# v0lta/PyTorch-Wavelet-Toolbox

Measured on AMD Instinct MI355X. Metric: Msamples/s, higher is better.
Workload: dtype f32; 1 GPU; wavedec2_db4_L3_64x1024x1024_f32; api=ptwt_amd.wavedec2(x, 'db4', mode='reflect', level=3), parallelism=batch-sharded x1, no data-path collective

## Files before the change

### __graft_entry__.py

```python
from __future__ import annotations

import os
import subprocess
import sys
import time
from concurrent.futures import ThreadPoolExecutor

ROOT = os.path.dirname(os.path.abspath(__file__))
PKG = os.path.join(ROOT, "pytorch-wavelet-toolbox_amd")
CSRC = os.path.join(PKG, "csrc")
LIB = os.path.join(PKG, "libmifwt.so")
ARCH = "gfx950"

if ROOT not in sys.path:
    sys.path.insert(0, ROOT)


def _hipcc() -> str:
    for cand in (os.environ.get("HIPCC"), "/opt/rocm/bin/hipcc", "hipcc"):
        if cand and (os.path.isabs(cand) and os.path.exists(cand) or not os.path.isabs(cand)):
            return cand
    return "hipcc"


def _sources():
    return sorted(os.path.join(CSRC, f) for f in os.listdir(CSRC) if f.endswith(".hip"))


STAMP = os.path.join(PKG, "build", "flags.stamp")


def _flag_string() -> str:
    return f"arch={ARCH} cflags={os.environ.get('MIFWT_CFLAGS', '')}"


def _needs_rebuild() -> bool:
    if not os.path.exists(LIB):
        return True
    if os.path.exists(STAMP):
        with open(STAMP) as f:
            if f.read() != _flag_string():
                return True
    elif os.environ.get("MIFWT_CFLAGS"):
        return True
    t = os.path.getmtime(LIB)
    deps = _sources() + [os.path.join(CSRC, f) for f in os.listdir(CSRC) if f.endswith(".h")]
    deps.append(os.path.join(ROOT, "include", "mifwt.h"))
    return any(os.path.getmtime(d) > t for d in deps)


def build_variant(tag: str, cflags: str) -> str:
    objdir = os.path.join(PKG, "build_" + tag)
    os.makedirs(objdir, exist_ok=True)
    lib = os.path.join(PKG, f"libmifwt_{tag}.so")
    flags = [f"--offload-arch={ARCH}", "-O3", "-std=c++17", "-fPIC", "-I" + os.path.join(ROOT, "include"), "-I" + CSRC, *cflags.split()]

    def compile_one(src: str) -> str:
        obj = os.path.join(objdir, os.path.basename(src)[:-4] + ".o")
        subprocess.run([_hipcc(), *flags, "-c", src, "-o", obj], check=True)
        return obj

    with ThreadPoolExecutor(max_workers=8) as pool:
        objs = list(pool.map(compile_one, _sources()))
    subprocess.run([_hipcc(), f"--offload-arch={ARCH}", "-shared", "-fPIC", *objs, "-o", lib], check=True)
    return lib


def build(force: bool = False, verbose: bool = True) -> None:
    if force or _needs_rebuild():
        t0 = time.time()
        objdir = os.path.join(PKG, "build")
        os.makedirs(objdir, exist_ok=True)
        flags = [f"--offload-arch={ARCH}", "-O3", "-std=c++17", "-fPIC", "-I" + os.path.join(ROOT, "include"), "-I" + CSRC]
        flags += os.environ.get("MIFWT_CFLAGS", "").split()

        import re

        def deps_mtime(path: str, seen=None) -> float:
            seen = set() if seen is None else seen
            if path in seen or not os.path.exists(path):
                return 0.0
            seen.add(path)
            t = os.path.getmtime(path)
            with open(path) as f:
                for inc in re.findall(r'^\s*#\s*include\s+"([^"]+)"', f.read(), flags=re.M):
                    for base in (CSRC, os.path.join(ROOT, "include")):
                        t = max(t, deps_mtime(os.path.join(base, inc), seen))
            return t

        stale_flags = not os.path.exists(STAMP) or open(STAMP).read() != _flag_string()

        def compile_one(src: str) -> str:
            obj = os.path.join(objdir, os.path.basename(src)[:-4] + ".o")
            if force or stale_flags or not os.path.exists(obj) or os.path.getmtime(obj) < deps_mtime(src):
                subprocess.run([_hipcc(), *flags, "-c", src, "-o", obj], check=True)
            return obj

        with ThreadPoolExecutor(max_workers=8) as pool:
            objs = list(pool.map(compile_one, _sources()))
        subprocess.run([_hipcc(), f"--offload-arch={ARCH}", "-shared", "-fPIC", *objs, "-o", LIB], check=True)
        with open(STAMP, "w") as f:
            f.write(_flag_string())
        if verbose:
            print(f"[build] libmifwt.so built for {ARCH} in {time.time() - t0:.1f}s ({len(objs)} translation units)")
    import ptwt_amd
    from ptwt_amd import _engine

    lib = _engine.load_library()
    for sym in ("mifwt_dwt_fwd", "mifwt_dwt_inv", "mifwt_dwt_fwd_adjoint", "mifwt_dwt_inv_adjoint", "mifwt_swt_fwd", "mifwt_swt_inv", "mifwt_tap_correlate", "mifwt_tap_correlate_dilated", "mifwt_dwt2_fwd_pair", "mifwt_dwt2_fwd_pair_supported", "mifwt_dwt2_inv_pair", "mifwt_dwt2_inv_pair_supported", "mifwt_dwt2_fwd_pyramid", "mifwt_dwt2_fwd_pyramid_supported", "mifwt_dwt2_fwd_pyramid_schedule", "mifwt_dwt3_fwd_slab_plan", "mifwt_dwt_fwd_dtaps", "mifwt_dwt_inv_dtaps", "mifwt_dwt_fwd_adjoint_dtaps", "mifwt_dwt_inv_adjoint_dtaps", "mifwt_workspace_bytes_dtaps", "mifwt_kernel_id_dtaps", "mifwt_dwt2_inv_pyramid", "mifwt_dwt2_inv_pyramid_supported", "mifwt_dwt1_fwd_long", "mifwt_dwt1_fwd_long_levels", "mifwt_dwt1_inv_long", "mifwt_dwt1_inv_long_supported", "mifwt_dwt1_long_plan", "mifwt_dwt1_fwd_tail", "mifwt_dwt1_fwd_tail_max_n", "mifwt_dwt1_inv_tail", "mifwt_workspace_bytes", "mifwt_kernel_id", "mifwt_set_option",
                "mifwt_launch_count", "mifwt_strerror", "mifwt_abi_version", "mifwt_bwt_fwd", "mifwt_bwt_inv", "mifwt_bwt_supported", "mifwt_bwt_kernel_id",
                "mifwt_bwt_axis_fwd", "mifwt_bwt_axis_inv", "mifwt_bwt3_fwd", "mifwt_bwt3_inv", "mifwt_bwt3_supported", "mifwt_bwt3_kernel_id",
                "mifwt_bwt_tree_levels", "mifwt_bwt_tree_fwd", "mifwt_bwt_tree_inv"):
        getattr(lib, sym)
    if verbose:
        print(f"[build] ptwt_amd imports, libmifwt ABI v{lib.mifwt_abi_version()} exports all symbols of include/mifwt.h")


def smoke() -> None:
    import numpy as np
    import torch

    build(verbose=False)
    import ptwt_amd
    from oracle import fwt_oracle as O

    assert torch.cuda.is_available(), "smoke() needs a GPU"
    dev = torch.device("cuda:0")
    g = torch.Generator().manual_seed(0)
    x = torch.randn(3, 70, 530, generator=g, dtype=torch.float32)
    coeffs = ptwt_amd.wavedec2(x.to(dev), "db4", level=3)
    want = O.wavedec2(x.numpy().astype(np.float64), "db4", level=3)

    def rel(a, b):
        return float(np.linalg.norm(a.cpu().double().numpy() - b) / np.linalg.norm(b))

    errs = [rel(coeffs[0], want[0])]
    for got_t, want_t in zip(coeffs[1:], want[1:]):
        errs += [rel(g_, w_) for g_, w_ in zip(got_t, want_t)]
    rec = ptwt_amd.waverec2(coeffs, "db4")
    rt = float((rec[..., :70, :530].cpu() - x).abs().max())
    torch.cuda.synchronize()
    assert max(errs) < 1e-6, f"HIP wavedec2 deviates from the oracle: {max(errs):.3e}"
    assert rt < 5e-6, f"round trip error {rt:.3e}"
    print(f"[smoke] wavedec2 db4 L3 on {torch.cuda.get_device_name(0)}: max sub-band rel-err vs oracle "
          f"{max(errs):.2e}, round-trip max-abs {rt:.2e}  OK")


if __name__ == "__main__":
    build(force="--force" in sys.argv)
    if "--smoke" in sys.argv:
        smoke()
```

### include/mifwt.h

```cpp
#ifndef MIFWT_H
#define MIFWT_H

#include <stddef.h>
#include <stdint.h>

#ifdef __cplusplus
extern "C" {
#endif

#define MIFWT_ABI_VERSION 3
#define MIFWT_MAX_NDIM 3
#define MIFWT_MAX_FILT 128

enum mifwt_dtype { MIFWT_F32 = 0, MIFWT_F64 = 1, MIFWT_F16 = 2  };

enum mifwt_mode {
  MIFWT_MODE_ZERO = 0,
  MIFWT_MODE_CONSTANT = 1,
  MIFWT_MODE_REFLECT = 2,
  MIFWT_MODE_PERIODIC = 3,
  MIFWT_MODE_SYMMETRIC = 4
};

enum mifwt_status {
  MIFWT_OK = 0,
  MIFWT_ERR_BADARG = -1,
  MIFWT_ERR_UNSUPPORTED = -2,
  MIFWT_ERR_WORKSPACE = -3,
  MIFWT_ERR_LAUNCH = -4
};

typedef struct mifwt_level_desc {
  int32_t ndim;
  int32_t dtype;
  int32_t mode;
  int32_t filt_len;
  int64_t batch;
  int64_t sig_extent[MIFWT_MAX_NDIM];
  int64_t sig_stride[1 + MIFWT_MAX_NDIM];
  int64_t coef_extent[MIFWT_MAX_NDIM];
  int64_t approx_stride[1 + MIFWT_MAX_NDIM];
  int64_t detail_stride[1 + MIFWT_MAX_NDIM];
} mifwt_level_desc;

int mifwt_dwt_fwd(const mifwt_level_desc* desc, const void* x, void* approx, void* const* details,
                  const double* dec_lo, const double* dec_hi, void* workspace, size_t workspace_bytes,
                  void* stream);

int mifwt_dwt_inv(const mifwt_level_desc* desc, const void* approx, const void* const* details, void* y,
                  const double* rec_lo, const double* rec_hi, void* workspace, size_t workspace_bytes,
                  void* stream);

int mifwt_kernel_id_dtaps(const mifwt_level_desc* desc, int direction);
size_t mifwt_workspace_bytes_dtaps(const mifwt_level_desc* desc, int direction);
int mifwt_dwt_fwd_dtaps(const mifwt_level_desc* desc, const void* x, void* approx, void* const* details, const double* d_dec_lo,
                        const double* d_dec_hi, void* workspace, size_t workspace_bytes, void* stream);
int mifwt_dwt_inv_dtaps(const mifwt_level_desc* desc, const void* approx, const void* const* details, void* y, const double* d_rec_lo,
                        const double* d_rec_hi, void* workspace, size_t workspace_bytes, void* stream);
int mifwt_dwt_fwd_adjoint_dtaps(const mifwt_level_desc* desc, const void* g_approx, const void* const* g_details, void* g_x,
                                const double* d_dec_lo, const double* d_dec_hi, void* workspace, size_t workspace_bytes, void* stream);
int mifwt_dwt_inv_adjoint_dtaps(const mifwt_level_desc* desc, const void* g_y, void* g_approx, void* const* g_details,
                                const double* d_rec_lo, const double* d_rec_hi, void* workspace, size_t workspace_bytes, void* stream);

int mifwt_dwt1_fwd_outer(int dtype, int64_t batch, int64_t n, int64_t inner, const void* x, int64_t x_batch_stride, int64_t x_axis_stride, void* lo_out,
                         void* hi_out, int64_t out_batch_stride, int64_t out_axis_stride, int mode, int filt_len, const double* dec_lo,
                         const double* dec_hi, const double* d_dec_lo, const double* d_dec_hi, void* stream);
int mifwt_dwt1_inv_outer(int dtype, int64_t batch, int64_t m, int64_t n_out, int64_t inner, const void* lo_in, int64_t lo_batch_stride,
                         int64_t lo_axis_stride, const void* hi_in, int64_t hi_batch_stride, int64_t hi_axis_stride, void* y, int64_t y_batch_stride,
                         int64_t y_axis_stride, int filt_len, const double* rec_lo, const double* rec_hi, const double* d_rec_lo,
                         const double* d_rec_hi, void* stream);
int mifwt_tap_correlate_planes(int dtype, int along, int64_t batch, int64_t a_rows, int64_t a_cols, int64_t b_rows, int64_t b_cols, const void* a,
                               int64_t a_batch_stride, int64_t a_row_stride, const void* b, int64_t b_batch_stride, int64_t b_row_stride,
                               int filt_len, int c0, int sgn, int mode, double* out, void* stream);

int mifwt_dwt2_fwd_pair_supported(const mifwt_level_desc* d1, const mifwt_level_desc* d2);
int mifwt_dwt2_fwd_pair(const mifwt_level_desc* d1, const mifwt_level_desc* d2, const void* x, void* const* details1,
                        void* approx2, void* const* details2, const double* dec_lo, const double* dec_hi, void* stream);

int mifwt_dwt2_fwd_pyramid_supported(int nlevels, const mifwt_level_desc* const* descs);
int mifwt_dwt2_fwd_pyramid(int nlevels, const mifwt_level_desc* const* descs, const void* x, void* const* const* details, void* approx,
                           const double* dec_lo, const double* dec_hi, void* stream);
int mifwt_dwt2_fwd_pyramid_schedule(int nlevels, const mifwt_level_desc* const* descs, unsigned int* wg_start, int capacity);

int mifwt_dwt3_fwd_slab_plan(const mifwt_level_desc* desc, int* out, int capacity);

int mifwt_dwt2_inv_pyramid_supported(int nlevels, const mifwt_level_desc* const* descs);
int mifwt_dwt2_inv_pyramid(int nlevels, const mifwt_level_desc* const* descs, const void* approx, const void* const* const* details, void* y,
                           const double* rec_lo, const double* rec_hi, void* stream);

int mifwt_dwt2_inv_pair_supported(const mifwt_level_desc* d2, const mifwt_level_desc* d1);
int mifwt_dwt2_inv_pair(const mifwt_level_desc* d2, const mifwt_level_desc* d1, const void* approx2, const void* const* details2,
                        const void* const* details1, void* y, const double* rec_lo, const double* rec_hi, void* stream);

int mifwt_dwt1_fwd_tail_max_n(int dtype);
int mifwt_dwt1_fwd_tail(int dtype, int filt_len, int mode, int64_t rows, int64_t n, int nlevels, const void* x, int64_t x_row_stride,
                        void* approx, int64_t approx_row_stride, void* const* details, const int64_t* detail_row_strides,
                        const double* dec_lo, const double* dec_hi, void* stream);

int mifwt_dwt1_fwd_long_levels(int dtype, int filt_len, int mode, int64_t rows, int64_t n, int want);
int mifwt_dwt1_fwd_long(int dtype, int filt_len, int mode, int64_t rows, int64_t n, int nlevels, const void* x, int64_t x_row_stride,
                        void* approx, int64_t approx_row_stride, void* const* details, const int64_t* detail_row_strides,
                        const double* dec_lo, const double* dec_hi, void* stream);

int mifwt_dwt1_inv_tail(int dtype, int filt_len, int64_t rows, int64_t m, int nlevels, const void* approx, int64_t approx_row_stride,
                        const void* const* details, const int64_t* detail_row_strides, const int32_t* out_len, void* y,
                        int64_t y_row_stride, const double* rec_lo, const double* rec_hi, void* stream);

int mifwt_dwt1_inv_long_supported(int dtype, int filt_len, int64_t rows, int nlevels, const int32_t* m);
int mifwt_dwt1_inv_long(int dtype, int filt_len, int64_t rows, int nlevels, const int32_t* m, const void* approx, int64_t approx_row_stride,
                        const void* const* details, const int64_t* detail_row_strides, void* y, int64_t y_row_stride,
                        const double* rec_lo, const double* rec_hi, void* stream);

int mifwt_dwt1_long_plan(int inverse, int dtype, int filt_len, int mode, int64_t rows, int64_t n, int nlevels, const int32_t* m, int32_t* out6);

int mifwt_dwt_fwd_adjoint(const mifwt_level_desc* desc, const void* g_approx, const void* const* g_details, void* g_x,
                          const double* dec_lo, const double* dec_hi, void* workspace, size_t workspace_bytes,
                          void* stream);
int mifwt_dwt_inv_adjoint(const mifwt_level_desc* desc, const void* g_y, void* g_approx, void* const* g_details,
                          const double* rec_lo, const double* rec_hi, void* workspace, size_t workspace_bytes,
                          void* stream);

int mifwt_swt_fwd(int dtype, int filt_len, int64_t rows, int64_t n, int64_t dilation, const void* x, int64_t x_row_stride,
                  void* lo, void* hi, int64_t lo_row_stride, int64_t hi_row_stride, const double* dec_lo,
                  const double* dec_hi, double scale, void* stream);
int mifwt_swt_inv(int dtype, int filt_len, int64_t rows, int64_t n, int64_t dilation, const void* a, const void* d,
                  int64_t a_row_stride, int64_t d_row_stride, void* y, int64_t y_row_stride, const double* rec_lo,
                  const double* rec_hi, double scale, void* stream);

#define MIFWT_KID_BWT_FWD 26
#define MIFWT_KID_BWT_INV 27
#define MIFWT_KID_BWT_AXIS_FWD 28
#define MIFWT_KID_BWT_AXIS_INV 29
typedef struct mifwt_bwt_tables {
  const double* rows;
  int32_t n_top, n_bot;
} mifwt_bwt_tables;
int mifwt_bwt_supported(const mifwt_level_desc* desc, int direction);
int mifwt_bwt_kernel_id(const mifwt_level_desc* desc, int direction);
int mifwt_bwt_fwd(const mifwt_level_desc* desc, const void* x, void* approx, void* const* details, const double* lo, const double* hi,
                  const mifwt_bwt_tables* tables, void* stream);
int mifwt_bwt_inv(const mifwt_level_desc* desc, const void* approx, const void* const* details, void* y, const double* lo, const double* hi,
                  const mifwt_bwt_tables* tables, void* stream);
int mifwt_bwt_axis_fwd(int dtype, int filt_len, int mode, int64_t outer, int64_t n, int64_t inner, const void* x, const int64_t* x_strides,
                       void* lo_out, const int64_t* lo_strides, void* hi_out, const int64_t* hi_strides, const double* lo, const double* hi,
                       const mifwt_bwt_tables* tables, void* stream);
int mifwt_bwt_axis_inv(int dtype, int filt_len, int64_t outer, int64_t n, int64_t inner, const void* lo_in, const int64_t* lo_strides,
                       const void* hi_in, const int64_t* hi_strides, void* y, const int64_t* y_strides, const double* lo, const double* hi,
                       const mifwt_bwt_tables* tables, void* stream);

#define MIFWT_KID_BWT3_FWD 30
#define MIFWT_KID_BWT3_INV 31
int mifwt_bwt3_supported(const mifwt_level_desc* desc, int direction);
int mifwt_bwt3_kernel_id(const mifwt_level_desc* desc, int direction);
int mifwt_bwt3_fwd(const mifwt_level_desc* desc, const void* x, void* approx, void* const* details, const double* lo, const double* hi,
                   const mifwt_bwt_tables* tables, void* stream);
int mifwt_bwt3_inv(const mifwt_level_desc* desc, const void* approx, const void* const* details, void* y, const double* lo, const double* hi,
                   const mifwt_bwt_tables* tables, void* stream);

#define MIFWT_KID_BWT_TREE_FWD 32
#define MIFWT_KID_BWT_TREE_INV 33
int mifwt_bwt_tree_levels(int dtype, int filt_len, int64_t n, int max_levels);
int mifwt_bwt_tree_fwd(int dtype, int filt_len, int64_t rows, int64_t n, int64_t x_row_stride, int nlevels, const void* x,
                       void* const* levels, const double* lo, const double* hi, const mifwt_bwt_tables* tables, void* stream);
int mifwt_bwt_tree_inv(int dtype, int filt_len, int64_t rows, int64_t n, int nlevels, const void* leaves, void* const* levels,
                       const double* lo, const double* hi, const mifwt_bwt_tables* tables, void* stream);

int mifwt_tap_correlate(int dtype, int64_t rows, int64_t m_len, int64_t n_len, const void* a, int64_t a_row_stride,
                        const void* b, int64_t b_row_stride, int filt_len, int c0, int sgn, int mode, double* out,
                        void* stream);
int mifwt_tap_correlate_dilated(int dtype, int64_t rows, int64_t n, const void* a, int64_t a_row_stride, const void* b,
                                int64_t b_row_stride, int filt_len, int64_t c0, int64_t tstep, double* out, void* stream);

size_t mifwt_workspace_bytes(const mifwt_level_desc* desc, int direction);

int mifwt_kernel_id(const mifwt_level_desc* desc, int direction);

#define MIFWT_OPT_FORCE_GENERIC 0
#define MIFWT_OPT_ROWS_PER_CHUNK 1
#define MIFWT_OPT_PREFETCH_PAIRS 2
#define MIFWT_OPT_RESERVED3 3
#define MIFWT_OPT_NT_STORE 4
#define MIFWT_OPT_TILE_MODE 5
#define MIFWT_OPT_TILE_ROWS 6
#define MIFWT_OPT_MFMA_MODE 7
#define MIFWT_OPT_PAIR_MODE 8
#define MIFWT_OPT_PAIR_ROWS 9
#define MIFWT_OPT_PYRAMID_MODE 12
#define MIFWT_OPT_DEBUG 11
#define MIFWT_OPT_PYR_WGS 13
#define MIFWT_OPT_EXP 15
#define MIFWT_OPT_SYNC_STAGE 10
int mifwt_set_option(int key, int value);

int mifwt_pyr_profile_buffer(void* device_buffer);

#define MIFWT_VARIANT_FWD_MFMA_WALK 0
#define MIFWT_VARIANT_FWD_MFMA_TILE 1
#define MIFWT_VARIANT_FWD_PYR_ST16 2
#define MIFWT_VARIANT_FWD_PYR_ST8 3
unsigned long long mifwt_launch_count(int variant);

const char* mifwt_strerror(int code);
int mifwt_abi_version(void);

#ifdef __cplusplus
}
#endif
#endif
```

### pytorch-wavelet-toolbox_amd/_engine.py

```python
from __future__ import annotations

import ctypes
import os
import threading
import warnings
from typing import List, Optional, Sequence, Tuple

import torch

_PKG_DIR = os.path.dirname(os.path.abspath(__file__))
LIB_PATH = os.path.join(_PKG_DIR, os.environ.get("MIFWT_LIB", "libmifwt.so"))
if "MIFWT_LIB" in os.environ:
    import warnings

    warnings.warn(f"ptwt_amd: MIFWT_LIB is set — running on the experiment build {LIB_PATH}, not on the product library", RuntimeWarning)
ABI_VERSION = 3

MODE_IDS = {"zero": 0, "constant": 1, "reflect": 2, "periodic": 3, "symmetric": 4}
_DTYPE_IDS = {torch.float32: 0, torch.float64: 1, torch.float16: 2}

_i64x3 = ctypes.c_int64 * 3
_i64x4 = ctypes.c_int64 * 4
_array_types: dict = {}


def _arr(base, n: int):
    t = _array_types.get((base, n))
    if t is None:
        t = _array_types[(base, n)] = base * n
    return t


class LevelDesc(ctypes.Structure):

    _fields_ = [
        ("ndim", ctypes.c_int32),
        ("dtype", ctypes.c_int32),
        ("mode", ctypes.c_int32),
        ("filt_len", ctypes.c_int32),
        ("batch", ctypes.c_int64),
        ("sig_extent", _i64x3),
        ("sig_stride", _i64x4),
        ("coef_extent", _i64x3),
        ("approx_stride", _i64x4),
        ("detail_stride", _i64x4),
    ]


_lib: Optional[ctypes.CDLL] = None


def load_library() -> ctypes.CDLL:
    global _lib
    if _lib is not None:
        return _lib
    if not os.path.isfile(LIB_PATH):
        raise RuntimeError(
            f"ptwt_amd: HIP extension {LIB_PATH} is missing — build it with "
            "`python -c \"import __graft_entry__ as g; g.build()\"` (hipcc --offload-arch=gfx950). "
            "There is no CPU/eager fallback."
        )
    lib = ctypes.CDLL(LIB_PATH)
    vp, cp = ctypes.c_void_p, ctypes.c_char_p
    dbl_p = ctypes.POINTER(ctypes.c_double)
    desc_p = ctypes.POINTER(LevelDesc)
    lib.mifwt_abi_version.restype = ctypes.c_int
    lib.mifwt_abi_version.argtypes = []
    mismatch = lib.mifwt_abi_version() != ABI_VERSION
    if mismatch:
        if os.environ.get("MIFWT_ALLOW_ABI_MISMATCH") != "1":
            raise RuntimeError(f"ptwt_amd: {os.path.basename(LIB_PATH)} has ABI version {lib.mifwt_abi_version()}, this package expects "
                               f"{ABI_VERSION}; rebuild the extension (MIFWT_ALLOW_ABI_MISMATCH=1 loads it anyway, at your own risk)")
        warnings.warn("ptwt_amd: ABI version mismatch accepted through MIFWT_ALLOW_ABI_MISMATCH=1")
    lib.mifwt_strerror.restype = cp
    lib.mifwt_strerror.argtypes = [ctypes.c_int]
    lib.mifwt_kernel_id.restype = ctypes.c_int
    lib.mifwt_kernel_id.argtypes = [desc_p, ctypes.c_int]
    lib.mifwt_workspace_bytes.restype = ctypes.c_size_t
    lib.mifwt_workspace_bytes.argtypes = [desc_p, ctypes.c_int]
    lib.mifwt_dwt_fwd.restype = ctypes.c_int
    lib.mifwt_dwt_fwd.argtypes = [desc_p, vp, vp, ctypes.POINTER(vp), dbl_p, dbl_p, vp, ctypes.c_size_t, vp]
    lib.mifwt_dwt_inv.restype = ctypes.c_int
    lib.mifwt_dwt_inv.argtypes = [desc_p, vp, ctypes.POINTER(vp), vp, dbl_p, dbl_p, vp, ctypes.c_size_t, vp]
    lib.mifwt_dwt_fwd_adjoint.restype = ctypes.c_int
    lib.mifwt_dwt_fwd_adjoint.argtypes = [desc_p, vp, ctypes.POINTER(vp), vp, dbl_p, dbl_p, vp, ctypes.c_size_t, vp]
    lib.mifwt_dwt_inv_adjoint.restype = ctypes.c_int
    lib.mifwt_dwt_inv_adjoint.argtypes = [desc_p, vp, vp, ctypes.POINTER(vp), dbl_p, dbl_p, vp, ctypes.c_size_t, vp]
    lib.mifwt_tap_correlate.restype = ctypes.c_int
    lib.mifwt_tap_correlate.argtypes = [ctypes.c_int, ctypes.c_int64, ctypes.c_int64, ctypes.c_int64, vp, ctypes.c_int64, vp,
                                        ctypes.c_int64, ctypes.c_int, ctypes.c_int, ctypes.c_int, ctypes.c_int, vp, vp]
    lib.mifwt_tap_correlate_dilated.restype = ctypes.c_int
    lib.mifwt_tap_correlate_dilated.argtypes = [ctypes.c_int, ctypes.c_int64, ctypes.c_int64, vp, ctypes.c_int64, vp, ctypes.c_int64,
                                                ctypes.c_int, ctypes.c_int64, ctypes.c_int64, vp, vp]
    lib.mifwt_dwt2_fwd_pair_supported.restype = ctypes.c_int
    lib.mifwt_dwt2_fwd_pair_supported.argtypes = [desc_p, desc_p]
    lib.mifwt_dwt2_fwd_pair.restype = ctypes.c_int
    lib.mifwt_dwt2_fwd_pair.argtypes = [desc_p, desc_p, vp, ctypes.POINTER(vp), vp, ctypes.POINTER(vp), dbl_p, dbl_p, vp]
    vpp = ctypes.POINTER(vp)
    lib.mifwt_dwt2_fwd_pyramid_supported.restype = ctypes.c_int
    lib.mifwt_dwt2_fwd_pyramid_supported.argtypes = [ctypes.c_int, ctypes.POINTER(desc_p)]
    lib.mifwt_dwt2_inv_pyramid_supported.restype = ctypes.c_int
    lib.mifwt_dwt2_inv_pyramid_supported.argtypes = [ctypes.c_int, ctypes.POINTER(desc_p)]
    lib.mifwt_dwt2_inv_pyramid.restype = ctypes.c_int
    lib.mifwt_dwt2_inv_pyramid.argtypes = [ctypes.c_int, ctypes.POINTER(desc_p), vp, ctypes.POINTER(vpp), vp, dbl_p, dbl_p, vp]
    lib.mifwt_dwt2_fwd_pyramid.restype = ctypes.c_int
    lib.mifwt_dwt2_fwd_pyramid.argtypes = [ctypes.c_int, ctypes.POINTER(desc_p), vp, ctypes.POINTER(vpp), vp, dbl_p, dbl_p, vp]
    lib.mifwt_dwt2_inv_pair_supported.restype = ctypes.c_int
    lib.mifwt_dwt2_inv_pair_supported.argtypes = [desc_p, desc_p]
    lib.mifwt_dwt2_inv_pair.restype = ctypes.c_int
    lib.mifwt_dwt2_inv_pair.argtypes = [desc_p, desc_p, vp, ctypes.POINTER(vp), ctypes.POINTER(vp), vp, dbl_p, dbl_p, vp]
    lib.mifwt_dwt1_fwd_tail_max_n.restype = ctypes.c_int
    lib.mifwt_dwt1_fwd_tail_max_n.argtypes = [ctypes.c_int]
    lib.mifwt_dwt1_fwd_tail.restype = ctypes.c_int
    lib.mifwt_dwt1_fwd_tail.argtypes = [ctypes.c_int, ctypes.c_int, ctypes.c_int, ctypes.c_int64, ctypes.c_int64, ctypes.c_int, vp,
                                        ctypes.c_int64, vp, ctypes.c_int64, ctypes.POINTER(vp), ctypes.POINTER(ctypes.c_int64), dbl_p, dbl_p, vp]
    lib.mifwt_dwt1_fwd_long.restype = ctypes.c_int
    lib.mifwt_dwt1_fwd_long.argtypes = lib.mifwt_dwt1_fwd_tail.argtypes
    lib.mifwt_dwt1_fwd_long_levels.restype = ctypes.c_int
    lib.mifwt_dwt1_fwd_long_levels.argtypes = [ctypes.c_int, ctypes.c_int, ctypes.c_int, ctypes.c_int64, ctypes.c_int64, ctypes.c_int]
    lib.mifwt_dwt1_inv_long_supported.restype = ctypes.c_int
    lib.mifwt_dwt1_inv_long_supported.argtypes = [ctypes.c_int, ctypes.c_int, ctypes.c_int64, ctypes.c_int, ctypes.POINTER(ctypes.c_int32)]
    lib.mifwt_dwt1_inv_long.restype = ctypes.c_int
    lib.mifwt_dwt1_inv_long.argtypes = [ctypes.c_int, ctypes.c_int, ctypes.c_int64, ctypes.c_int, ctypes.POINTER(ctypes.c_int32), vp, ctypes.c_int64,
                                        ctypes.POINTER(vp), ctypes.POINTER(ctypes.c_int64), vp, ctypes.c_int64, dbl_p, dbl_p, vp]
    lib.mifwt_dwt1_inv_tail.restype = ctypes.c_int
    lib.mifwt_dwt1_inv_tail.argtypes = [ctypes.c_int, ctypes.c_int, ctypes.c_int64, ctypes.c_int64, ctypes.c_int, vp, ctypes.c_int64,
                                        ctypes.POINTER(vp), ctypes.POINTER(ctypes.c_int64), ctypes.POINTER(ctypes.c_int32), vp,
                                        ctypes.c_int64, dbl_p, dbl_p, vp]
    experiment = mismatch
    if not experiment or hasattr(lib, "mifwt_workspace_bytes_dtaps"):
        lib.mifwt_workspace_bytes_dtaps.restype = ctypes.c_size_t
        lib.mifwt_workspace_bytes_dtaps.argtypes = [desc_p, ctypes.c_int]
    if not experiment or hasattr(lib, "mifwt_kernel_id_dtaps"):
        lib.mifwt_kernel_id_dtaps.restype = ctypes.c_int
        lib.mifwt_kernel_id_dtaps.argtypes = [desc_p, ctypes.c_int]
        for name in ("mifwt_dwt_fwd_dtaps", "mifwt_dwt_inv_dtaps", "mifwt_dwt_fwd_adjoint_dtaps", "mifwt_dwt_inv_adjoint_dtaps"):
            getattr(lib, name).restype = ctypes.c_int
        lib.mifwt_dwt_fwd_dtaps.argtypes = [desc_p, vp, vp, vpp, vp, vp, vp, ctypes.c_size_t, vp]
        lib.mifwt_dwt_inv_dtaps.argtypes = [desc_p, vp, vpp, vp, vp, vp, vp, ctypes.c_size_t, vp]
        lib.mifwt_dwt_fwd_adjoint_dtaps.argtypes = [desc_p, vp, vpp, vp, vp, vp, vp, ctypes.c_size_t, vp]
        lib.mifwt_dwt_inv_adjoint_dtaps.argtypes = [desc_p, vp, vp, vpp, vp, vp, vp, ctypes.c_size_t, vp]
    if not experiment or hasattr(lib, "mifwt_launch_count"):
        lib.mifwt_launch_count.restype = ctypes.c_uint64
        lib.mifwt_launch_count.argtypes = [ctypes.c_int]
    if not experiment or hasattr(lib, "mifwt_tap_correlate_planes"):
        lib.mifwt_tap_correlate_planes.restype = ctypes.c_int
        lib.mifwt_tap_correlate_planes.argtypes = [ctypes.c_int, ctypes.c_int] + [ctypes.c_int64] * 5 + [vp, ctypes.c_int64, ctypes.c_int64, vp, ctypes.c_int64,
                                                   ctypes.c_int64, ctypes.c_int, ctypes.c_int, ctypes.c_int, ctypes.c_int, vp, vp]
        lib.mifwt_dwt1_inv_outer.restype = ctypes.c_int
        lib.mifwt_dwt1_inv_outer.argtypes = [ctypes.c_int] + [ctypes.c_int64] * 4 + [vp, ctypes.c_int64, ctypes.c_int64, vp, ctypes.c_int64, ctypes.c_int64, vp,
                                             ctypes.c_int64, ctypes.c_int64, ctypes.c_int, dbl_p, dbl_p, vp, vp, vp]
        lib.mifwt_dwt1_fwd_outer.restype = ctypes.c_int
        lib.mifwt_dwt1_fwd_outer.argtypes = [ctypes.c_int, ctypes.c_int64, ctypes.c_int64, ctypes.c_int64, vp, ctypes.c_int64, ctypes.c_int64, vp, vp, ctypes.c_int64,
                                             ctypes.c_int64, ctypes.c_int, ctypes.c_int, dbl_p, dbl_p, vp, vp, vp]
    lib.mifwt_set_option.restype = ctypes.c_int
    lib.mifwt_set_option.argtypes = [ctypes.c_int, ctypes.c_int]
    _lib = lib
    return lib


def _check(rc: int) -> None:
    if rc != 0:
        msg = load_library().mifwt_strerror(rc).decode()
        raise RuntimeError(f"libmifwt: {msg} (code {rc})")


def _require_gpu(t: torch.Tensor) -> None:
    if not t.is_cuda:
        raise RuntimeError(
            f"ptwt_amd: expected a tensor on a ROCm device, got device '{t.device}'. This engine runs on "
            "MI355X only; there is no CPU path."
        )


level_events: Optional[list] = None

ROW_ALIGN = int(os.environ.get("MIFWT_ROW_ALIGN", "1"))
PYRAMID_ROW_ALIGN = int(os.environ.get("MIFWT_PYRAMID_ROW_ALIGN", "1"))

OPT_FORCE_GENERIC = 0
OPT_ROWS_PER_CHUNK = 1
OPT_PREFETCH_PAIRS = 2
OPT_NT_STORE = 4
OPT_TILE_MODE = 5
OPT_TILE_ROWS = 6
OPT_MFMA_MODE = 7
OPT_PAIR_MODE = 8
OPT_PAIR_ROWS = 9
OPT_DEBUG = 11
OPT_PYRAMID_MODE = 12
OPT_PYR_WGS = 13
OPT_EXP = 15
KID_PAIR = 12
KID_INV_PAIR = 13
KID_TAIL = 14
KID_INV_TAIL = 15
KID_PYRAMID = 16
KID_LONG = 17
KID_INV_LONG = 18
KID_SMALL = 20
KID_INV_SMALL = 21
KID_INV_PYRAMID = 22
MAX_PYRAMID_LEVELS = 8


VARIANT_FWD_MFMA_WALK, VARIANT_FWD_MFMA_TILE, VARIANT_FWD_PYR_ST16, VARIANT_FWD_PYR_ST8 = 0, 1, 2, 3


def launch_count(variant: int) -> int:
    return int(load_library().mifwt_launch_count(variant))


def set_option(key: int, value: int) -> None:
    _check(load_library().mifwt_set_option(key, value))
    _plans.clear()
    for c in _routing_caches:
        c.clear()


_routing_caches: list = []


class _Plan:

    __slots__ = ("desc", "ref", "alloc_shape", "view_last", "nb", "plane_bytes", "ws_bytes", "kid", "empty")


_plans: dict = {}


def _trim_plans() -> None:
    if len(_plans) > 4096:
        for k in list(_plans)[:1024]:
            _plans.pop(k, None)
_tls = threading.local()
_taps_cache: dict = {}


class DevTaps:

    __slots__ = ("t",)

    def __init__(self, t: torch.Tensor):
        t = t.detach().reshape(-1)
        if t.dtype != torch.float64 or not t.is_contiguous():
            t = t.to(torch.float64).contiguous()
        self.t = t

    def __len__(self) -> int:
        return int(self.t.shape[0])

    @property
    def ptr(self) -> int:
        return self.t.data_ptr()


def outer_axis_supported(flen: int, dtype: torch.dtype) -> bool:
    return dtype in (torch.float32, torch.float64) and ((2 <= flen <= 20 and flen % 2 == 0) or flen in (24, 32))


def _is_dev(taps) -> bool:
    return isinstance(taps, DevTaps)


def _taps_array(taps: Sequence[float]):
    key = tuple(taps)
    arr = _taps_cache.get(key)
    if arr is None:
        if len(_taps_cache) > 512:
            _taps_cache.clear()
        arr = _taps_cache[key] = _arr(ctypes.c_double, len(key))(*key)
    return arr


def _band_ptrs(base: int, plane_bytes: int, n: int):
    return _arr(ctypes.c_void_p, n)(*[base + s * plane_bytes for s in range(1, n + 1)])


def _raw_stream(dev_index: int) -> int:
    return torch._C._cuda_getCurrentRawStream(dev_index)


class HipLevelEngine:

    @staticmethod
    def _analysis_plan(x: torch.Tensor, flen: int, mode_id: int, min_align: int = 1) -> _Plan:
        lib = load_library()
        ndim = x.dim() - 1
        batch = x.shape[0]
        sig = [int(n) for n in x.shape[1:]]
        coef = [(n + 2 * ((2 * flen - 3) // 2) + (n % 2) - flen) // 2 + 1 for n in sig]
        nb = 1 << ndim
        esz = x.element_size()
        align = max(ROW_ALIGN, min_align, 1)
        if align <= 1 and ndim == 2 and x.dtype == torch.float16 and 18 <= flen <= 32:
            align = 128
        pitch = -(-coef[-1] * esz // align) * align // esz if align > esz and ndim >= 2 else coef[-1]
        if min_align < 0 and ndim >= 2:
            pitch = coef[-1] - min_align
        p = _Plan()
        p.alloc_shape = (batch, nb, *coef[:-1], pitch)
        p.view_last = coef[-1] if pitch != coef[-1] else None
        p.nb = nb
        p.empty = batch == 0 or min(coef) == 0
        d = LevelDesc()
        d.ndim, d.dtype, d.mode, d.filt_len, d.batch = ndim, _DTYPE_IDS[x.dtype], mode_id, flen, batch
        bstride = [1] * (ndim + 2)
        for i in range(ndim, -1, -1):
            bstride[i] = bstride[i + 1] * p.alloc_shape[i + 1]
        for a in range(ndim):
            d.sig_extent[a] = sig[a]
            d.coef_extent[a] = coef[a]
            d.sig_stride[1 + a] = x.stride(1 + a)
            d.approx_stride[1 + a] = d.detail_stride[1 + a] = bstride[2 + a]
        d.sig_stride[0] = x.stride(0)
        d.approx_stride[0] = d.detail_stride[0] = bstride[0]
        p.desc = d
        p.ref = ctypes.byref(d)
        p.plane_bytes = bstride[1] * esz
        p.ws_bytes = 0 if p.empty else lib.mifwt_workspace_bytes(p.ref, 0)
        p.kid = lib.mifwt_kernel_id(p.ref, 0)
        return p

    @staticmethod
    def _details_only(pl: _Plan) -> _Plan:
        q = _Plan()
        d = LevelDesc()
        ctypes.memmove(ctypes.addressof(d), ctypes.addressof(pl.desc), ctypes.sizeof(LevelDesc))
        plane = pl.desc.detail_stride[0] // pl.nb
        d.detail_stride[0] = d.approx_stride[0] = plane * (pl.nb - 1)
        q.desc, q.ref = d, ctypes.byref(d)
        q.alloc_shape = (pl.alloc_shape[0], pl.nb - 1, *pl.alloc_shape[2:])
        q.view_last, q.nb, q.plane_bytes, q.ws_bytes, q.kid, q.empty = pl.view_last, pl.nb - 1, pl.plane_bytes, pl.ws_bytes, pl.kid, pl.empty
        return q

    def analysis(self, x: torch.Tensor, dec_lo: Sequence[float], dec_hi: Sequence[float], mode_id: int) -> torch.Tensor:
        _require_gpu(x)
        flen = len(dec_lo)
        key = (x.shape, x.stride(), x.dtype, mode_id, flen, ROW_ALIGN)
        p = _plans.get(key)
        if p is None:
            _trim_plans()
            p = _plans[key] = self._analysis_plan(x, flen, mode_id)
        buf = torch.empty(p.alloc_shape, dtype=x.dtype, device=x.device)
        if p.view_last is not None:
            buf = buf[..., : p.view_last]
        if p.empty:
            return buf
        base = buf.data_ptr()
        ptrs = _band_ptrs(base, p.plane_bytes, p.nb - 1)
        lib = _lib
        xp = x.data_ptr()
        if _is_dev(dec_lo):
            dl, dh = dec_lo.ptr, dec_hi.ptr
            self._run(p, 0, x, lambda ws, wsb, stream: lib.mifwt_dwt_fwd_dtaps(p.ref, xp, base, ptrs, dl, dh, ws, wsb, stream), kid=0, dtaps=True)
            return buf
        lo, hi = _taps_array(dec_lo), _taps_array(dec_hi)
        self._run(p, 0, x, lambda ws, wsb, stream: lib.mifwt_dwt_fwd(p.ref, xp, base, ptrs, lo, hi, ws, wsb, stream))
        return buf

    def analysis_pair(self, x: torch.Tensor, dec_lo: Sequence[float], dec_hi: Sequence[float], mode_id: int):
        _require_gpu(x)
        if x.dim() != 3:
            return None
        flen = len(dec_lo)
        key = ("pair", x.shape, x.stride(), x.dtype, mode_id, flen, ROW_ALIGN)
        plan = _plans.get(key)
        if plan is None:
            _trim_plans()
            lib = load_library()
            p1 = self._analysis_plan(x, flen, mode_id)
            ok = False
            p2 = None
            if not p1.empty:
                lvl1 = torch.empty(p1.alloc_shape, dtype=x.dtype, device="meta")
                if p1.view_last is not None:
                    lvl1 = lvl1[..., : p1.view_last]
                p2 = self._analysis_plan(lvl1[:, 0], flen, mode_id)
                ok = (not p2.empty) and bool(lib.mifwt_dwt2_fwd_pair_supported(p1.ref, p2.ref))
                if ok:
                    lean = self._details_only(p1)
                    if lib.mifwt_dwt2_fwd_pair_supported(lean.ref, p2.ref):
                        p1 = lean
            plan = _plans[key] = (p1, p2, ok)
        p1, p2, ok = plan
        if not ok:
            return None
        buf1 = torch.empty(p1.alloc_shape, dtype=x.dtype, device=x.device)
        buf2 = torch.empty(p2.alloc_shape, dtype=x.dtype, device=x.device)
        if p1.view_last is not None:
            buf1 = buf1[..., : p1.view_last]
        if p2.view_last is not None:
            buf2 = buf2[..., : p2.view_last]
        b1, b2 = buf1.data_ptr(), buf2.data_ptr()
        ptrs1 = _band_ptrs(b1 - (4 - p1.nb) * p1.plane_bytes, p1.plane_bytes, 3)
        ptrs2 = _band_ptrs(b2, p2.plane_bytes, 3)
        lo, hi = _taps_array(dec_lo), _taps_array(dec_hi)
        lib = _lib
        xp = x.data_ptr()
        self._run(p1, 0, x, lambda ws, wsb, stream: lib.mifwt_dwt2_fwd_pair(p1.ref, p2.ref, xp, ptrs1, b2, ptrs2, lo, hi, stream),
                  kid=KID_PAIR)
        return buf1, buf2

    def analysis_pyramid(self, x: torch.Tensor, dec_lo: Sequence[float], dec_hi: Sequence[float], mode_id: int, nlevels: int):
        _require_gpu(x)
        if x.dim() != 3 or x.dtype != torch.float32:
            return None
        flen = len(dec_lo)
        key, plan = self._pyramid_plan(x, flen, mode_id, nlevels)
        plans, n_ok, refs, kid = plan
        if n_ok == 0:
            return None
        bufs = []
        for pl in plans:
            b = torch.empty(pl.alloc_shape, dtype=x.dtype, device=x.device)
            bufs.append(b if pl.view_last is None else b[..., : pl.view_last])
        skey = (key, n_ok)
        slot = _tls.__dict__.setdefault("pyr", {}).get(skey)
        if slot is None:
            rows = [_arr(ctypes.c_void_p, 3)() for _ in plans]
            det = _arr(ctypes.POINTER(ctypes.c_void_p), n_ok)(*[ctypes.cast(r, ctypes.POINTER(ctypes.c_void_p)) for r in rows])
            slot = _tls.pyr[skey] = (rows, det)
            if len(_tls.pyr) > 256:
                _tls.pyr.clear()
                _tls.pyr[skey] = slot
        rows, det = slot
        for r, b, pl in zip(rows, bufs, plans):
            pb = pl.plane_bytes
            base = b.data_ptr() + (pl.nb - 3) * pb
            r[0], r[1], r[2] = base, base + pb, base + 2 * pb
        lo, hi = _taps_array(dec_lo), _taps_array(dec_hi)
        lib = _lib
        xp, ap = x.data_ptr(), bufs[-1].data_ptr()
        self._run(plans[0], 0, x, lambda ws, wsb, stream: lib.mifwt_dwt2_fwd_pyramid(n_ok, refs, xp, det, ap, lo, hi, stream), kid=kid)
        return bufs

    def pyramid_levels(self, x: torch.Tensor, flen: int, mode_id: int, nlevels: int) -> int:
        if x.dim() != 3 or x.dtype != torch.float32 or not x.is_cuda:
            return 0
        return self._pyramid_plan(x, flen, mode_id, nlevels)[1][1]

    def _pyramid_plan(self, x: torch.Tensor, flen: int, mode_id: int, nlevels: int):
        key = ("pyr", x.shape, x.stride(), mode_id, flen, min(nlevels, MAX_PYRAMID_LEVELS), ROW_ALIGN, PYRAMID_ROW_ALIGN)
        plan = _plans.get(key)
        if plan is None:
            _trim_plans()
            lib = load_library()

            def chain(min_align):
                plans = [self._analysis_plan(x, flen, mode_id, min_align)]
                while len(plans) < min(nlevels, MAX_PYRAMID_LEVELS) and not plans[-1].empty:
                    pl = plans[-1]
                    lvl = torch.empty(pl.alloc_shape, dtype=x.dtype, device="meta")
                    if pl.view_last is not None:
                        lvl = lvl[..., : pl.view_last]
                    plans.append(self._analysis_plan(lvl[:, 0], flen, mode_id, min_align))
                n_ok, route = 0, 0
                if not any(pl.empty for pl in plans):
                    for n in range(len(plans), 0, -1):
                        refs = (ctypes.POINTER(LevelDesc) * n)(*[ctypes.pointer(pl.desc) for pl in plans[:n]])
                        route = lib.mifwt_dwt2_fwd_pyramid_supported(n, refs)
                        if route:
                            n_ok = n
                            break
                return plans, n_ok, route

            plans, n_ok, route = chain(1)
            if n_ok and route == 1 and (PYRAMID_ROW_ALIGN > 1 or PYRAMID_ROW_ALIGN < 0):
                plans_a, n_a, route_a = chain(PYRAMID_ROW_ALIGN)
                if n_a == n_ok and route_a == route:
                    plans = plans_a
            keep = plans[:n_ok]
            refs = (ctypes.POINTER(LevelDesc) * n_ok)(*[ctypes.pointer(pl.desc) for pl in keep]) if n_ok else None
            if n_ok > 1:
                lean = [self._details_only(pl) for pl in keep[:-1]] + [keep[-1]]
                lrefs = (ctypes.POINTER(LevelDesc) * n_ok)(*[ctypes.pointer(pl.desc) for pl in lean])
                if lib.mifwt_dwt2_fwd_pyramid_supported(n_ok, lrefs) == route:
                    keep, refs = lean, lrefs
            if n_ok:
                keep[0].ws_bytes = 0
            plan = _plans[key] = (keep, n_ok, refs, KID_SMALL if route == 2 else KID_PYRAMID)
        return key, plan

    def analysis_tail(self, x: torch.Tensor, dec_lo: Sequence[float], dec_hi: Sequence[float], mode_id: int, nlevels: int):
        _require_gpu(x)
        if x.dim() != 2 or x.dtype not in (torch.float32, torch.float64) or x.stride(1) != 1 or nlevels < 2 or nlevels > 24:
            return None
        lib = load_library()
        flen = len(dec_lo)
        rows, n0 = x.shape
        if rows == 0 or n0 == 0 or flen > 32:
            return None
        k_long = lib.mifwt_dwt1_fwd_long_levels(_DTYPE_IDS[x.dtype], flen, mode_id, rows, n0, nlevels) if x.dtype == torch.float32 else 0
        long_rows = k_long >= 2
        if long_rows:
            nlevels = k_long
        elif n0 > lib.mifwt_dwt1_fwd_tail_max_n(_DTYPE_IDS[x.dtype]):
            return None
        sizes, n = [], n0
        for _ in range(nlevels):
            n = (n + flen - 1) // 2
            sizes.append(n)
        last = nlevels - 1
        bufs = [torch.empty((rows, 2 if i == last else 1, m), dtype=x.dtype, device=x.device) for i, m in enumerate(sizes)]
        esz = x.element_size()
        det = _arr(ctypes.c_void_p, nlevels)(*[b.data_ptr() + (sizes[i] * esz if i == last else 0) for i, b in enumerate(bufs)])
        det_rs = _arr(ctypes.c_int64, nlevels)(*[(2 if i == last else 1) * m for i, m in enumerate(sizes)])
        lo, hi = _taps_array(dec_lo), _taps_array(dec_hi)
        p = _Plan()
        p.ws_bytes, p.kid = 0, (KID_LONG if long_rows else KID_TAIL)
        d = LevelDesc()
        d.ndim = 1
        d.sig_extent[0] = n0
# ... 529 lines not shown
```

### pytorch-wavelet-toolbox_amd/csrc/mifwt_api.hip

```cpp
#include <string.h>

#include "mifwt_common.h"

using namespace mifwt;

namespace {

inline int64_t elem_size(int dtype) { return dtype == MIFWT_F64 ? 8 : (dtype == MIFWT_F16 ? 2 : 4); }

int validate(const mifwt_level_desc* d, int direction) {
  if (!d) return MIFWT_ERR_BADARG;
  if (d->ndim < 1 || d->ndim > MIFWT_MAX_NDIM) return MIFWT_ERR_BADARG;
  if (d->dtype != MIFWT_F32 && d->dtype != MIFWT_F64 && d->dtype != MIFWT_F16) return MIFWT_ERR_BADARG;
  if (d->filt_len < 2 || d->filt_len > MIFWT_MAX_FILT) return MIFWT_ERR_BADARG;
  if (d->batch < 0) return MIFWT_ERR_BADARG;
  if (direction == 0 && (d->mode < MIFWT_MODE_ZERO || d->mode > MIFWT_MODE_SYMMETRIC)) return MIFWT_ERR_BADARG;
  for (int a = 0; a < d->ndim; ++a) {
    const int64_t n = d->sig_extent[a], m = d->coef_extent[a], L = d->filt_len;
    if (n < 1 || m < 1 || n > INT32_MAX / 4 || m > INT32_MAX / 4) return MIFWT_ERR_BADARG;
    if (direction == 0) {
      const int64_t pad = 2 * ((2 * L - 3) / 2) + (n % 2);
      if (m != (n + pad - L) / 2 + 1) return MIFWT_ERR_BADARG;
    } else {
      const int64_t full = 2 * m - L + 2;
// ... 310 lines not shown

static size_t level_ws(const mifwt_level_desc* desc, int direction, bool dev) {
  if (validate_call(desc, direction) != MIFWT_OK) return 0;
  return route_ws(desc, direction == 0 || direction == 3 ? 0 : 1, route(desc, direction, dev));
}

int mifwt_kernel_id(const mifwt_level_desc* desc, int direction) {
  const int rc = validate_call(desc, direction);
  return rc != MIFWT_OK ? rc : route(desc, direction, false);
}

size_t mifwt_workspace_bytes(const mifwt_level_desc* desc, int direction) { return level_ws(desc, direction, false); }

int mifwt_kernel_id_dtaps(const mifwt_level_desc* desc, int direction) {
  if (direction < 0 || direction > 3) return MIFWT_ERR_BADARG;
  const int rc = validate_call(desc, direction);
  return rc != MIFWT_OK ? rc : route(desc, direction, true);
}

size_t mifwt_workspace_bytes_dtaps(const mifwt_level_desc* desc, int direction) {
  return direction < 0 || direction > 3 ? 0 : level_ws(desc, direction, true);
}

static LevelTaps reversed(LevelTaps t, int L, double (&buf)[2][MIFWT_MAX_FILT]) {
  if (t.dev) return {t.lo, t.hi, true, t.rev ^ 1};
  for (int j = 0; j < L; ++j) {
    buf[0][j] = t.tap_lo(L - 1 - j);
    buf[1][j] = t.tap_hi(L - 1 - j);
  }
  return {buf[0], buf[1], false, 0};
}

static int level_fwd(const mifwt_level_desc* desc, const void* x, void* approx, void* const* details, LevelTaps dec, void* workspace,
                     size_t workspace_bytes, void* stream) {
  int rc = validate(desc, 0);
  if (rc != MIFWT_OK) return rc;
  if (!x || !approx || !details || !dec.lo || !dec.hi) return MIFWT_ERR_BADARG;
  for (int s = 1; s < (1 << desc->ndim); ++s)
    if (!details[s - 1]) return MIFWT_ERR_BADARG;
  if (desc->batch == 0) return MIFWT_OK;
  hipStream_t st = static_cast<hipStream_t>(stream);
  const int kid = route(desc, 0, dec.dev);
  const size_t need = route_ws(desc, 0, kid);
  if (need > 0 && (!workspace || workspace_bytes < need)) return MIFWT_ERR_WORKSPACE;
  switch (kid) {
    case kGeneric: return generic_fwd(desc, x, approx, details, dec, workspace, st);
    case kDwt2FwdTile: return dwt2_fwd_tile(desc, x, approx, details, dec, st);
    case kDwt2FwdPyr: return dwt2_fwd_fused(desc, x, approx, details, dec, st);
    case kDwt1FwdRow: return rows_fwd(desc, x, approx, details, dec, workspace, st);
    default: break;
  }
  const double *lo, *hi;
  if ((rc = dec.host(&lo, &hi)) != MIFWT_OK) return rc;
  switch (kid) {
    case kDwt2FwdStream: return dwt2_fwd_stream(desc, x, approx, details, lo, hi, st);
    case kDwt2FwdMfma: return dwt2_fwd_mfma(desc, x, approx, details, lo, hi, st);
    case kDwt3FwdTile: return dwt3_fwd_tile(desc, x, approx, details, lo, hi, st);
    case kDwt3FwdWalk: return dwt3_fwd_walk(desc, x, approx, details, lo, hi, st);
    case kDwt3FwdStream: return plane3_fwd(desc, x, approx, details, lo, hi, workspace, st);
    default: return MIFWT_ERR_UNSUPPORTED;
  }
}

static int level_inv(const mifwt_level_desc* desc, const void* approx, const void* const* details, void* y, LevelTaps rec, void* workspace,
                     size_t workspace_bytes, void* stream) {
  int rc = validate(desc, 1);
  if (rc != MIFWT_OK) return rc;
  if (!y || !approx || !details || !rec.lo || !rec.hi) return MIFWT_ERR_BADARG;
  for (int s = 1; s < (1 << desc->ndim); ++s)
    if (!details[s - 1]) return MIFWT_ERR_BADARG;
  if (desc->batch == 0) return MIFWT_OK;
  hipStream_t st = static_cast<hipStream_t>(stream);
  const int kid = route(desc, 1, rec.dev);
  const size_t need = route_ws(desc, 1, kid);
  if (need > 0 && (!workspace || workspace_bytes < need)) return MIFWT_ERR_WORKSPACE;
  switch (kid) {
    case kGeneric: return generic_inv(desc, approx, details, y, rec, workspace, st);
    case kDwt2InvTile: return dwt2_inv_tile(desc, approx, details, y, rec, st);
    case kDwt2InvPyr: return dwt2_inv_fused(desc, approx, details, y, rec, st);
    case kDwt1InvRow: return rows_inv(desc, approx, details, y, rec, workspace, st);
    default: break;
  }
  const double *lo, *hi;
  if ((rc = rec.host(&lo, &hi)) != MIFWT_OK) return rc;
  switch (kid) {
    case kDwt2InvStream: return dwt2_inv_stream(desc, approx, details, y, lo, hi, st);
    case kDwt2InvMfma: return dwt2_inv_mfma(desc, approx, details, y, lo, hi, st);
    case kDwt3InvTile: return dwt3_inv_tile(desc, approx, details, y, lo, hi, st);
    case kDwt3InvWalk: return dwt3_inv_walk(desc, approx, details, y, lo, hi, st);
    case kDwt3InvStream: return plane3_inv(desc, approx, details, y, lo, hi, workspace, st);
    default: return MIFWT_ERR_UNSUPPORTED;
  }
}

static int level_fwd_adjoint(const mifwt_level_desc* desc, const void* g_approx, const void* const* g_details, void* g_x, LevelTaps dec,
                             void* workspace, size_t workspace_bytes, void* stream) {
  int rc = validate(desc, 0);
  if (rc != MIFWT_OK) return rc;
  if (!g_x || !g_approx || !g_details || !dec.lo || !dec.hi) return MIFWT_ERR_BADARG;
  for (int s = 1; s < (1 << desc->ndim); ++s)
    if (!g_details[s - 1]) return MIFWT_ERR_BADARG;
  if (desc->batch == 0) return MIFWT_OK;
  hipStream_t st = static_cast<hipStream_t>(stream);
  const bool synth = dec.dev ? route(desc, 2, true) != kGeneric
                             : adjoint_is_synthesis(desc) && (desc->mode == MIFWT_MODE_ZERO || adjoint_border_supported(desc));
  if (!synth) {
    const size_t need = generic_ws(desc, 1);
    if (need > 0 && (!workspace || workspace_bytes < need)) return MIFWT_ERR_WORKSPACE;
    return generic_inv(desc, g_approx, g_details, g_x, dec, workspace, st, true);
  }
  double buf[2][MIFWT_MAX_FILT];
  const mifwt_level_desc z = as_zero_mode(desc);
  rc = level_inv(&z, g_approx, g_details, g_x, reversed(dec, desc->filt_len, buf), workspace, workspace_bytes, stream);
  if (rc != MIFWT_OK || desc->mode == MIFWT_MODE_ZERO) return rc;
  return adjoint_border(desc, g_approx, g_details, g_x, dec, st);
}

static int level_inv_adjoint(const mifwt_level_desc* desc, const void* g_y, void* g_approx, void* const* g_details, LevelTaps rec,
                             void* workspace, size_t workspace_bytes, void* stream) {
  const int rc = validate(desc, 1);
  if (rc != MIFWT_OK) return rc;
  if (!rec.lo || !rec.hi) return MIFWT_ERR_BADARG;
  double buf[2][MIFWT_MAX_FILT];
  const mifwt_level_desc z = as_zero_mode(desc);
  return level_fwd(&z, g_y, g_approx, g_details, reversed(rec, desc->filt_len, buf), workspace, workspace_bytes, stream);
}

int mifwt_dwt_fwd(const mifwt_level_desc* desc, const void* x, void* approx, void* const* details,
                  const double* dec_lo, const double* dec_hi, void* workspace, size_t workspace_bytes,
                  void* stream) {
  return level_fwd(desc, x, approx, details, {dec_lo, dec_hi, false, 0}, workspace, workspace_bytes, stream);
}

int mifwt_dwt_inv(const mifwt_level_desc* desc, const void* approx, const void* const* details, void* y,
                  const double* rec_lo, const double* rec_hi, void* workspace, size_t workspace_bytes,
                  void* stream) {
  return level_inv(desc, approx, details, y, {rec_lo, rec_hi, false, 0}, workspace, workspace_bytes, stream);
}

int mifwt_dwt_fwd_adjoint(const mifwt_level_desc* desc, const void* g_approx, const void* const* g_details, void* g_x,
                          const double* dec_lo, const double* dec_hi, void* workspace, size_t workspace_bytes,
                          void* stream) {
  return level_fwd_adjoint(desc, g_approx, g_details, g_x, {dec_lo, dec_hi, false, 0}, workspace, workspace_bytes, stream);
}

int mifwt_dwt_inv_adjoint(const mifwt_level_desc* desc, const void* g_y, void* g_approx, void* const* g_details,
                          const double* rec_lo, const double* rec_hi, void* workspace, size_t workspace_bytes,
                          void* stream) {
  return level_inv_adjoint(desc, g_y, g_approx, g_details, {rec_lo, rec_hi, false, 0}, workspace, workspace_bytes, stream);
}

int mifwt_dwt_fwd_dtaps(const mifwt_level_desc* desc, const void* x, void* approx, void* const* details, const double* d_dec_lo,
                        const double* d_dec_hi, void* workspace, size_t workspace_bytes, void* stream) {
  return level_fwd(desc, x, approx, details, {d_dec_lo, d_dec_hi, true, 0}, workspace, workspace_bytes, stream);
}

int mifwt_dwt_inv_dtaps(const mifwt_level_desc* desc, const void* approx, const void* const* details, void* y, const double* d_rec_lo,
                        const double* d_rec_hi, void* workspace, size_t workspace_bytes, void* stream) {
  return level_inv(desc, approx, details, y, {d_rec_lo, d_rec_hi, true, 0}, workspace, workspace_bytes, stream);
}

int mifwt_dwt_fwd_adjoint_dtaps(const mifwt_level_desc* desc, const void* g_approx, const void* const* g_details, void* g_x,
                                const double* d_dec_lo, const double* d_dec_hi, void* workspace, size_t workspace_bytes, void* stream) {
  return level_fwd_adjoint(desc, g_approx, g_details, g_x, {d_dec_lo, d_dec_hi, true, 0}, workspace, workspace_bytes, stream);
}

int mifwt_dwt_inv_adjoint_dtaps(const mifwt_level_desc* desc, const void* g_y, void* g_approx, void* const* g_details,
                                const double* d_rec_lo, const double* d_rec_hi, void* workspace, size_t workspace_bytes, void* stream) {
  return level_inv_adjoint(desc, g_y, g_approx, g_details, {d_rec_lo, d_rec_hi, true, 0}, workspace, workspace_bytes, stream);
}

static LevelTaps host_or_device(const double* lo, const double* hi, const double* d_lo, const double* d_hi) {
  return d_lo && d_hi ? LevelTaps{d_lo, d_hi, true, 0} : LevelTaps{lo, hi, false, 0};
}

int mifwt_dwt1_fwd_outer(int dtype, int64_t batch, int64_t n, int64_t inner, const void* x, int64_t x_batch_stride, int64_t x_axis_stride, void* lo_out,
                         void* hi_out, int64_t out_batch_stride, int64_t out_axis_stride, int mode, int filt_len, const double* dec_lo,
                         const double* dec_hi, const double* d_dec_lo, const double* d_dec_hi, void* stream) {
  const LevelTaps taps = host_or_device(dec_lo, dec_hi, d_dec_lo, d_dec_hi);
  if (!x || !lo_out || !hi_out || !taps.lo || !taps.hi || batch < 0 || n < 1 || inner < 1) return MIFWT_ERR_BADARG;
  if (mode < MIFWT_MODE_ZERO || mode > MIFWT_MODE_SYMMETRIC) return MIFWT_ERR_BADARG;
  if ((dtype != MIFWT_F32 && dtype != MIFWT_F64) || !stream_filter_supported(filt_len)) return MIFWT_ERR_UNSUPPORTED;
  if (batch == 0) return MIFWT_OK;
  StreamJob jb;
  memset(&jb, 0, sizeof(jb));
  jb.in0 = x;
  jb.out0 = lo_out;
  jb.out1 = hi_out;
  jb.in0_s[0] = x_batch_stride, jb.in0_s[1] = x_axis_stride;
  jb.out0_s[0] = jb.out1_s[0] = out_batch_stride, jb.out0_s[1] = jb.out1_s[1] = out_axis_stride;
  StreamCall c;
  memset(&c, 0, sizeof(c));
  c.filt_len = filt_len;
  c.mode = mode;
  c.jobs = &jb;
  c.njobs = 1;
  c.batch = batch;
  c.inner = inner;
  c.n_in = n;
  c.n_out = (n + filt_len - 1) / 2;
  c.taps = taps;
  c.stream = static_cast<hipStream_t>(stream);
  return stream_call(dtype, kOuterFwd, c);
}

int mifwt_dwt1_inv_outer(int dtype, int64_t batch, int64_t m, int64_t n_out, int64_t inner, const void* lo_in, int64_t lo_batch_stride,
                         int64_t lo_axis_stride, const void* hi_in, int64_t hi_batch_stride, int64_t hi_axis_stride, void* y, int64_t y_batch_stride,
                         int64_t y_axis_stride, int filt_len, const double* rec_lo, const double* rec_hi, const double* d_rec_lo,
                         const double* d_rec_hi, void* stream) {
  const LevelTaps taps = host_or_device(rec_lo, rec_hi, d_rec_lo, d_rec_hi);
  if (!lo_in || !hi_in || !y || !taps.lo || !taps.hi || batch < 0 || m < 1 || inner < 1 || n_out < 1) return MIFWT_ERR_BADARG;
  if (n_out > 2 * m - filt_len + 2 || n_out < 2 * m - filt_len + 1) return MIFWT_ERR_BADARG;
  if ((dtype != MIFWT_F32 && dtype != MIFWT_F64) || !stream_filter_supported(filt_len)) return MIFWT_ERR_UNSUPPORTED;
  if (batch == 0) return MIFWT_OK;
  StreamJob jb;
  memset(&jb, 0, sizeof(jb));
  jb.in0 = lo_in;
  jb.in1 = hi_in;
  jb.out0 = y;
  jb.in0_s[0] = lo_batch_stride, jb.in0_s[1] = lo_axis_stride;
  jb.in1_s[0] = hi_batch_stride, jb.in1_s[1] = hi_axis_stride;
  jb.out0_s[0] = y_batch_stride, jb.out0_s[1] = y_axis_stride;
  StreamCall c;
  memset(&c, 0, sizeof(c));
  c.filt_len = filt_len;
  c.jobs = &jb;
  c.njobs = 1;
  c.batch = batch;
  c.inner = inner;
  c.n_in = m;
  c.n_out = n_out;
  c.taps = taps;
  c.stream = static_cast<hipStream_t>(stream);
  return stream_call(dtype, kOuterInv, c);
}

int mifwt_dwt2_fwd_pair_supported(const mifwt_level_desc* d1, const mifwt_level_desc* d2) {
  if (!d1 || !d2 || validate(d1, 0) != MIFWT_OK || validate(d2, 0) != MIFWT_OK) return 0;
  return dwt2_fwd_pair_supported(d1, d2) ? 1 : 0;
}

int mifwt_dwt2_fwd_pair(const mifwt_level_desc* d1, const mifwt_level_desc* d2, const void* x, void* const* details1,
                        void* approx2, void* const* details2, const double* dec_lo, const double* dec_hi, void* stream) {
  if (!d1 || !d2) return MIFWT_ERR_BADARG;
  int rc = validate(d1, 0);
  if (rc == MIFWT_OK) rc = validate(d2, 0);
  if (rc != MIFWT_OK) return rc;
  if (!x || !details1 || !approx2 || !details2 || !dec_lo || !dec_hi) return MIFWT_ERR_BADARG;
  for (int s = 0; s < 3; ++s)
    if (!details1[s] || !details2[s]) return MIFWT_ERR_BADARG;
  if (!dwt2_fwd_pair_supported(d1, d2)) return MIFWT_ERR_UNSUPPORTED;
  if (d1->batch == 0) return MIFWT_OK;
  hipStream_t st = static_cast<hipStream_t>(stream);
  const int pm = g_options[MIFWT_OPT_PAIR_MODE];
  if (pm != 1 && (pm == 3 || d1->filt_len >= 8) && dwt2_fwd_roll_supported(d1, d2))
    return dwt2_fwd_roll(d1, d2, x, details1, approx2, details2, dec_lo, dec_hi, st);
  return dwt2_fwd_pair(d1, d2, x, details1, approx2, details2, dec_lo, dec_hi, st);
}
static int pyramid_route(int nlevels, const mifwt_level_desc* const* descs) {
  const bool pyr = nlevels <= 3 && dwt2_fwd_pyr_supported(nlevels, descs);
  if (pyr && g_options[MIFWT_OPT_PYRAMID_MODE] == 1) return 1;
  const bool lone = nlevels == 1 && descs[0]->batch < 1024 && g_options[MIFWT_OPT_PYRAMID_MODE] != 3;
  if (!lone && dwt2_fwd_small_supported(nlevels, descs)) return 2;
  return pyr ? 1 : 0;
}

int mifwt_dwt2_fwd_pyramid_supported(int nlevels, const mifwt_level_desc* const* descs) {
  if (!descs || nlevels < 1 || nlevels > 8) return 0;
  for (int l = 0; l < nlevels; ++l)
    if (!descs[l] || validate(descs[l], 0) != MIFWT_OK) return 0;
  return pyramid_route(nlevels, descs);
}

int mifwt_dwt2_fwd_pyramid(int nlevels, const mifwt_level_desc* const* descs, const void* x, void* const* const* details, void* approx,
                           const double* dec_lo, const double* dec_hi, void* stream) {
  if (!descs || nlevels < 1 || nlevels > 8) return MIFWT_ERR_BADARG;
  for (int l = 0; l < nlevels; ++l) {
    if (!descs[l]) return MIFWT_ERR_BADARG;
    const int rc = validate(descs[l], 0);
    if (rc != MIFWT_OK) return rc;
  }
  if (!x || !details || !approx || !dec_lo || !dec_hi) return MIFWT_ERR_BADARG;
  for (int l = 0; l < nlevels; ++l) {
    if (!details[l]) return MIFWT_ERR_BADARG;
    for (int s = 0; s < 3; ++s)
      if (!details[l][s]) return MIFWT_ERR_BADARG;
  }
  const int route = pyramid_route(nlevels, descs);
  if (route == 0) return MIFWT_ERR_UNSUPPORTED;
  if (descs[0]->batch == 0) return MIFWT_OK;
  if (route == 2) return dwt2_fwd_small(nlevels, descs, x, details, approx, dec_lo, dec_hi, static_cast<hipStream_t>(stream));
  return dwt2_fwd_pyr(nlevels, descs, x, details, approx, {dec_lo, dec_hi, false, 0}, static_cast<hipStream_t>(stream));
}
int mifwt_dwt2_fwd_pyramid_schedule(int nlevels, const mifwt_level_desc* const* descs, unsigned int* wg_start, int capacity) {
  if (!descs || !wg_start || nlevels < 1 || nlevels > 3) return MIFWT_ERR_BADARG;
  for (int l = 0; l < nlevels; ++l) {
    if (!descs[l]) return MIFWT_ERR_BADARG;
    const int rc = validate(descs[l], 0);
    if (rc != MIFWT_OK) return rc;
  }
  if (pyramid_route(nlevels, descs) != 1) return MIFWT_ERR_UNSUPPORTED;
  return dwt2_fwd_pyr_schedule(nlevels, descs, wg_start, capacity);
}
int mifwt_dwt3_fwd_slab_plan(const mifwt_level_desc* desc, int* out, int capacity) {
  if (!desc || !out) return MIFWT_ERR_BADARG;
  const int rc = validate(desc, 0);
  if (rc != MIFWT_OK) return rc;
  return dwt3_fwd_slab_plan_query(desc, out, capacity);
}
int mifwt_dwt2_inv_pyramid_supported(int nlevels, const mifwt_level_desc* const* descs) {
  if (!descs || nlevels < 1 || nlevels > 8) return 0;
  for (int l = 0; l < nlevels; ++l)
    if (!descs[l] || validate(descs[l], 1) != MIFWT_OK) return 0;
  if (dwt2_inv_small_supported(nlevels, descs)) return 1;
  return nlevels <= 3 && dwt2_inv_pyr_supported(nlevels, descs) ? 2 : 0;
}

int mifwt_dwt2_inv_pyramid(int nlevels, const mifwt_level_desc* const* descs, const void* approx, const void* const* const* details, void* y,
                           const double* rec_lo, const double* rec_hi, void* stream) {
  if (!descs || nlevels < 1 || nlevels > 8) return MIFWT_ERR_BADARG;
  for (int l = 0; l < nlevels; ++l) {
    if (!descs[l]) return MIFWT_ERR_BADARG;
    const int rc = validate(descs[l], 1);
    if (rc != MIFWT_OK) return rc;
  }
  if (!approx || !details || !y || !rec_lo || !rec_hi) return MIFWT_ERR_BADARG;
  for (int l = 0; l < nlevels; ++l) {
    if (!details[l]) return MIFWT_ERR_BADARG;
    for (int s = 0; s < 3; ++s)
      if (!details[l][s]) return MIFWT_ERR_BADARG;
  }
  if (dwt2_inv_small_supported(nlevels, descs)) {
    if (descs[0]->batch == 0) return MIFWT_OK;
    return dwt2_inv_small(nlevels, descs, approx, details, y, rec_lo, rec_hi, static_cast<hipStream_t>(stream));
  }
  if (nlevels > 3 || !dwt2_inv_pyr_supported(nlevels, descs)) return MIFWT_ERR_UNSUPPORTED;
  return dwt2_inv_pyr(nlevels, descs, approx, details, y, {rec_lo, rec_hi, false, 0}, static_cast<hipStream_t>(stream));
}
int mifwt_dwt2_inv_pair_supported(const mifwt_level_desc* d2, const mifwt_level_desc* d1) {
  if (!d1 || !d2 || validate(d1, 1) != MIFWT_OK || validate(d2, 1) != MIFWT_OK) return 0;
  return dwt2_inv_pair_supported(d2, d1) ? 1 : 0;
}

int mifwt_dwt2_inv_pair(const mifwt_level_desc* d2, const mifwt_level_desc* d1, const void* approx2, const void* const* details2,
                        const void* const* details1, void* y, const double* rec_lo, const double* rec_hi, void* stream) {
  if (!d1 || !d2) return MIFWT_ERR_BADARG;
  int rc = validate(d2, 1);
  if (rc == MIFWT_OK) rc = validate(d1, 1);
  if (rc != MIFWT_OK) return rc;
  if (!approx2 || !details2 || !details1 || !y || !rec_lo || !rec_hi) return MIFWT_ERR_BADARG;
  for (int s = 0; s < 3; ++s)
    if (!details1[s] || !details2[s]) return MIFWT_ERR_BADARG;
  if (!dwt2_inv_pair_supported(d2, d1)) return MIFWT_ERR_UNSUPPORTED;
  if (d1->batch == 0) return MIFWT_OK;
  return dwt2_inv_pair(d2, d1, approx2, details2, details1, y, rec_lo, rec_hi, static_cast<hipStream_t>(stream));
}
int mifwt_dwt1_fwd_tail_max_n(int dtype) { return dwt1_tail_max_n(dtype); }

int mifwt_dwt1_fwd_tail(int dtype, int filt_len, int mode, int64_t rows, int64_t n, int nlevels, const void* x, int64_t x_row_stride,
                        void* approx, int64_t approx_row_stride, void* const* details, const int64_t* detail_row_strides,
                        const double* dec_lo, const double* dec_hi, void* stream) {
  if (!x || !approx || !details || !detail_row_strides || !dec_lo || !dec_hi) return MIFWT_ERR_BADARG;
  if (!dwt1_tail_supported(dtype, filt_len, mode, rows, n, nlevels)) return MIFWT_ERR_UNSUPPORTED;
  for (int l = 0; l < nlevels; ++l)
    if (!details[l]) return MIFWT_ERR_BADARG;
  return dwt1_tail(dtype, filt_len, mode, rows, n, nlevels, x, x_row_stride, approx, approx_row_stride, details, detail_row_strides,
                   dec_lo, dec_hi, static_cast<hipStream_t>(stream));
}
int mifwt_dwt1_fwd_long_levels(int dtype, int filt_len, int mode, int64_t rows, int64_t n, int want) {
  return dwt1_long_levels(dtype, filt_len, mode, rows, n, want);
}

int mifwt_dwt1_fwd_long(int dtype, int filt_len, int mode, int64_t rows, int64_t n, int nlevels, const void* x, int64_t x_row_stride,
                        void* approx, int64_t approx_row_stride, void* const* details, const int64_t* detail_row_strides,
                        const double* dec_lo, const double* dec_hi, void* stream) {
  if (!x || !approx || !details || !detail_row_strides || !dec_lo || !dec_hi) return MIFWT_ERR_BADARG;
  if (nlevels < 1 || dwt1_long_levels(dtype, filt_len, mode, rows, n, nlevels) != nlevels) return MIFWT_ERR_UNSUPPORTED;
  for (int l = 0; l < nlevels; ++l)
    if (!details[l]) return MIFWT_ERR_BADARG;
  return dwt1_long(dtype, filt_len, mode, rows, n, nlevels, x, x_row_stride, approx, approx_row_stride, details, detail_row_strides,
                   dec_lo, dec_hi, static_cast<hipStream_t>(stream));
}
int mifwt_dwt1_inv_long_supported(int dtype, int filt_len, int64_t rows, int nlevels, const int32_t* m) {
  return idwt1_long_supported(dtype, filt_len, rows, nlevels, m);
}

int mifwt_dwt1_inv_long(int dtype, int filt_len, int64_t rows, int nlevels, const int32_t* m, const void* approx, int64_t approx_row_stride,
                        const void* const* details, const int64_t* detail_row_strides, void* y, int64_t y_row_stride,
                        const double* rec_lo, const double* rec_hi, void* stream) {
  if (!m || !approx || !details || !detail_row_strides || !y || !rec_lo || !rec_hi) return MIFWT_ERR_BADARG;
  if (!idwt1_long_supported(dtype, filt_len, rows, nlevels, m)) return MIFWT_ERR_UNSUPPORTED;
  for (int l = 0; l < nlevels; ++l)
    if (!details[l]) return MIFWT_ERR_BADARG;
  return idwt1_long(dtype, filt_len, rows, nlevels, m, approx, approx_row_stride, details, detail_row_strides, y, y_row_stride, rec_lo,
                    rec_hi, static_cast<hipStream_t>(stream));
}
int mifwt_dwt1_long_plan(int inverse, int dtype, int filt_len, int mode, int64_t rows, int64_t n, int nlevels, const int32_t* m, int32_t* out6) {
  if (!out6) return 0;
  return inverse ? idwt1_long_plan_query(dtype, filt_len, rows, nlevels, m, out6) : dwt1_long_plan_query(dtype, filt_len, mode, rows, n, nlevels, out6);
}
int mifwt_dwt1_inv_tail(int dtype, int filt_len, int64_t rows, int64_t m, int nlevels, const void* approx, int64_t approx_row_stride,
                        const void* const* details, const int64_t* detail_row_strides, const int32_t* out_len, void* y,
                        int64_t y_row_stride, const double* rec_lo, const double* rec_hi, void* stream) {
  if (!approx || !details || !detail_row_strides || !out_len || !y || !rec_lo || !rec_hi) return MIFWT_ERR_BADARG;
  if (!idwt1_tail_supported(dtype, filt_len, rows, m, nlevels, out_len)) return MIFWT_ERR_UNSUPPORTED;
  for (int l = 0; l < nlevels; ++l)
    if (!details[l]) return MIFWT_ERR_BADARG;
  return idwt1_tail(dtype, filt_len, rows, m, nlevels, approx, approx_row_stride, details, detail_row_strides, out_len, y, y_row_stride,
                    rec_lo, rec_hi, static_cast<hipStream_t>(stream));
}
}
```

### pytorch-wavelet-toolbox_amd/csrc/mifwt_common.h

```cpp
#pragma once
#include <hip/hip_runtime.h>
#include <stdint.h>

#include <atomic>

#include "mifwt.h"

namespace mifwt {

constexpr int kMaxFilt = MIFWT_MAX_FILT;
extern int g_options[16];

#ifdef MIFWT_DIAG
constexpr bool kDiag = true;
#define MIFWT_DBG(a) ((a).dbg)
#define MIFWT_EXPW(a) ((a).exp)
#define MIFWT_PROFP(a) ((a).prof)
#else
constexpr bool kDiag = false;
#define MIFWT_DBG(a) 0
#define MIFWT_EXPW(a) 0
#define MIFWT_PROFP(a) (static_cast<unsigned long long*>(nullptr))
#endif
constexpr int kRouteBits = 8 | 64 | 512 | 1024 | 4096 | 8192 | 524288 | 1048576 | 2097152;
inline int exp_word() { return kDiag ? g_options[MIFWT_OPT_EXP] : 0; }
extern unsigned long long g_launch_counts[16];
inline void count_launch(int variant) { __atomic_fetch_add(&g_launch_counts[variant], 1ull, __ATOMIC_RELAXED); }

struct BatchSplit {
  int64_t inner, outer_stride;
};

struct DynLdsOnce {
  std::atomic<uint64_t> done{0};
  bool ensure(const void* fn, int bytes) {
    int dev = 0;
    if (hipGetDevice(&dev) != hipSuccess) return false;
    const uint64_t bit = uint64_t(1) << (dev & 63);
    if (done.load(std::memory_order_acquire) & bit) return true;
    if (hipFuncSetAttribute(fn, hipFuncAttributeMaxDynamicSharedMemorySize, bytes) != hipSuccess) return false;
    done.fetch_or(bit, std::memory_order_release);
    return true;
  }
};

__host__ __device__ __forceinline__ int ext_index(int i, int n, int mode) {
  if ((unsigned)i < (unsigned)n) return i;
  switch (mode) {
    case MIFWT_MODE_ZERO:
      return -1;
    case MIFWT_MODE_CONSTANT:
      return i < 0 ? 0 : n - 1;
    case MIFWT_MODE_PERIODIC: {
      int p = i % n;
      return p < 0 ? p + n : p;
    }
    case MIFWT_MODE_SYMMETRIC: {
      const int t = 2 * n;
      int p = i % t;
      if (p < 0) p += t;
      return p < n ? p : t - 1 - p;
    }
    default: {
      if (n == 1) return 0;
      const int t = 2 * (n - 1);
      int p = i % t;
      if (p < 0) p += t;
      return p < n ? p : t - p;
    }
  }
}

__host__ __device__ __forceinline__ int ext_index_near(int i, int n, int mode) {
  if ((unsigned)i < (unsigned)n) return i;
  int j;
  switch (mode) {
    case MIFWT_MODE_ZERO:
      return -1;
    case MIFWT_MODE_CONSTANT:
      return i < 0 ? 0 : n - 1;
    case MIFWT_MODE_PERIODIC:
      j = i < 0 ? i + n : i - n;
      break;
    case MIFWT_MODE_SYMMETRIC:
      j = i < 0 ? -i - 1 : 2 * n - 1 - i;
      break;
    default:
      j = i < 0 ? -i : 2 * (n - 1) - i;
      break;
  }
  return (unsigned)j < (unsigned)n ? j : ext_index(i, n, mode);
}

struct AxisJob {
  const void* in0;
  const void* in1;
  void* out0;
  void* out1;
  int64_t in0_stride[4], in1_stride[4], out0_stride[4], out1_stride[4];
};

struct DeviceTaps {
  const double* lo;
  const double* hi;
  int rev;
};
struct DevTapArg {
  const double* lo;
  const double* hi;
  int rev, len;
};
struct LevelTaps {
  const double* lo;
  const double* hi;
  bool dev;
  int rev;
  double tap_lo(int m) const { return dev ? 0.0 : lo[m]; }
  double tap_hi(int m) const { return dev ? 0.0 : hi[m]; }
  DeviceTaps dev_taps() const { return dev ? DeviceTaps{lo, hi, rev} : DeviceTaps{nullptr, nullptr, 0}; }
  DevTapArg dev_arg(int filt_len) const { return dev ? DevTapArg{lo, hi, rev, filt_len} : DevTapArg{nullptr, nullptr, 0, filt_len}; }
  int host(const double** lo_out, const double** hi_out) const {
    if (dev) return MIFWT_ERR_UNSUPPORTED;
    *lo_out = lo;
    *hi_out = hi;
    return MIFWT_OK;
  }
};
#ifdef __HIPCC__
__device__ __forceinline__ int dtap_rfl(int v) {
  int r;
  asm volatile("s_nop 0\n\tv_readfirstlane_b32 %0, %1\n\ts_nop 1" : "=s"(r) : "v"(v));
  return r;
}
__device__ __forceinline__ float dtap_uniform(float v) { return __builtin_bit_cast(float, dtap_rfl(__builtin_bit_cast(int, v))); }
__device__ __forceinline__ double dtap_uniform(double v) { return v; }
template <typename S>
__device__ __forceinline__ S dtap_lo(const DevTapArg& dt, int m) { return dtap_uniform((S)dt.lo[dt.rev ? dt.len - 1 - m : m]); }
template <typename S>
__device__ __forceinline__ S dtap_hi(const DevTapArg& dt, int m) { return dtap_uniform((S)dt.hi[dt.rev ? dt.len - 1 - m : m]); }
#endif
int launch_axis_fwd(int dtype, const AxisJob* jobs, int njobs, const int64_t out_ext[4], int taxis, int64_t n_in,
                    int mode, int filt_len, LevelTaps taps, hipStream_t stream);
int launch_axis_inv(int dtype, const AxisJob* jobs, int njobs, const int64_t out_ext[4], int taxis, int64_t m_in,
                    int filt_len, LevelTaps taps, hipStream_t stream);

int launch_axis_adj(int dtype, const AxisJob* jobs, int njobs, const int64_t out_ext[4], int taxis, int64_t m_in,
                    int64_t n_sig, int mode, int filt_len, LevelTaps taps, hipStream_t stream);

struct StreamJob {
  const void* in0;
  const void* in1;
  void* out0;
  void* out1;
  int64_t in0_s[3], in1_s[3], out0_s[3], out1_s[3];
};

struct StreamCall {
  int filt_len, mode;
  const StreamJob* jobs;
  int njobs;
  int64_t batch;
  int64_t rows[3];
  int64_t n_in, n_out;
  int64_t inner;
  LevelTaps taps;
  hipStream_t stream;
};

enum StreamKind { kOuterFwd = 0, kOuterInv = 1, kInnerFwd = 2, kInnerInv = 3 };
bool stream_filter_supported(int filt_len);
int stream_call(int dtype, int kind, const StreamCall& c);

enum KernelId { kGeneric = 0, kDwt2FwdStream = 1, kDwt2InvStream = 2, kDwt1FwdRow = 3, kDwt1InvRow = 4, kDwt3FwdStream = 5, kDwt3InvStream = 6, kDwt2FwdTile = 7, kDwt2InvTile = 8, kDwt3FwdTile = 9, kDwt3InvTile = 10, kDwt2FwdMfma = 11, kDwt2FwdPair = 12, kDwt2InvPair = 13, kDwt1FwdTail = 14, kDwt1InvTail = 15, kDwt2FwdPyr = 16,
  kDwt1FwdLong = 17, kDwt1InvLong = 18, kDwt2FwdSmall = 20, kDwt2InvSmall = 21, kDwt2InvPyr = 22, kDwt2InvMfma = 23, kDwt3FwdWalk = 24, kDwt3InvWalk = 25 };

bool dwt2_fwd_stream_supported(const mifwt_level_desc* d);
int dwt2_fwd_stream(const mifwt_level_desc* d, const void* x, void* approx, void* const* details,
                    const double* dec_lo, const double* dec_hi, hipStream_t stream);

bool dwt2_fwd_tile_supported(const mifwt_level_desc* d);
int dwt2_fwd_tile(const mifwt_level_desc* d, const void* x, void* approx, void* const* details, LevelTaps dec, hipStream_t stream,
                  BatchSplit split = {0, 0});

bool dwt2_fwd_mfma_supported(const mifwt_level_desc* d);
bool dwt2_inv_mfma_supported(const mifwt_level_desc* d);
int dwt2_inv_mfma(const mifwt_level_desc* d, const void* approx, const void* const* details, void* y, const double* lo,
                  const double* hi, hipStream_t stream);
int dwt2_fwd_mfma(const mifwt_level_desc* d, const void* x, void* approx, void* const* details,
                  const double* dec_lo, const double* dec_hi, hipStream_t stream);

bool dwt2_fwd_pair_supported(const mifwt_level_desc* d1, const mifwt_level_desc* d2);
int dwt2_fwd_pair(const mifwt_level_desc* d1, const mifwt_level_desc* d2, const void* x, void* const* details1,
                  void* approx2, void* const* details2, const double* dec_lo, const double* dec_hi, hipStream_t stream);

bool dwt2_fwd_roll_supported(const mifwt_level_desc* d1, const mifwt_level_desc* d2);

bool adjoint_border_supported(const mifwt_level_desc* d);
int adjoint_border(const mifwt_level_desc* d, const void* g_approx, const void* const* g_details, void* g_x, LevelTaps dec,
                   hipStream_t stream);
int dwt2_fwd_roll(const mifwt_level_desc* d1, const mifwt_level_desc* d2, const void* x, void* const* details1,
                  void* approx2, void* const* details2, const double* dec_lo, const double* dec_hi, hipStream_t stream);

bool dwt2_fwd_small_supported(int nlevels, const mifwt_level_desc* const* d);
int dwt2_fwd_small(int nlevels, const mifwt_level_desc* const* d, const void* x, void* const* const* details, void* approx, const double* lo,
                   const double* hi, hipStream_t stream);
bool dwt2_inv_small_supported(int nlevels, const mifwt_level_desc* const* d);
int dwt2_inv_small(int nlevels, const mifwt_level_desc* const* d, const void* approx, const void* const* const* details, void* y,
                   const double* lo, const double* hi, hipStream_t stream);
bool dwt2_inv_pyr_supported(int nlev, const mifwt_level_desc* const* d);
int dwt2_inv_pyr(int nlev, const mifwt_level_desc* const* d, const void* approx, const void* const* const* details, void* y,
                 LevelTaps rec, hipStream_t stream);
bool dwt2_fwd_pyr_supported(int nlev, const mifwt_level_desc* const* d);
int dwt2_fwd_pyr(int nlev, const mifwt_level_desc* const* d, const void* x, void* const* const* details, void* approx,
                 LevelTaps dec, hipStream_t stream);
int dwt2_fwd_pyr_schedule(int nlev, const mifwt_level_desc* const* d, uint32_t* wg_start, int capacity);

bool dwt2_inv_pair_supported(const mifwt_level_desc* d2, const mifwt_level_desc* d1);
int dwt2_inv_pair(const mifwt_level_desc* d2, const mifwt_level_desc* d1, const void* approx2, const void* const* details2,
                  const void* const* details1, void* y, const double* rec_lo, const double* rec_hi, hipStream_t stream);

int dwt1_tail_max_n(int dtype);
bool dwt1_tail_supported(int dtype, int filt_len, int mode, int64_t rows, int64_t n0, int nlevels);
int dwt1_tail(int dtype, int filt_len, int mode, int64_t rows, int64_t n0, int nlevels, const void* x, int64_t x_row_stride,
              void* approx, int64_t approx_row_stride, void* const* details, const int64_t* detail_row_strides, const double* lo,
              const double* hi, hipStream_t stream);

int dwt1_long_levels(int dtype, int filt_len, int mode, int64_t rows, int64_t n0, int want);
int dwt1_long(int dtype, int filt_len, int mode, int64_t rows, int64_t n0, int nlevels, const void* x, int64_t x_row_stride,
              void* approx, int64_t approx_row_stride, void* const* details, const int64_t* detail_row_strides, const double* lo,
              const double* hi, hipStream_t stream);
int idwt1_long_supported(int dtype, int filt_len, int64_t rows, int nlevels, const int* m);
int dwt1_long_plan_query(int dtype, int filt_len, int mode, int64_t rows, int64_t n0, int want, int* out);
int idwt1_long_plan_query(int dtype, int filt_len, int64_t rows, int nlevels, const int* m, int* out);
int idwt1_long(int dtype, int filt_len, int64_t rows, int nlevels, const int* m, const void* approx, int64_t approx_row_stride,
               const void* const* details, const int64_t* detail_row_strides, void* y, int64_t y_row_stride, const double* lo,
               const double* hi, hipStream_t stream);
bool idwt1_tail_supported(int dtype, int filt_len, int64_t rows, int64_t m0, int nlevels, const int* out_len);
int idwt1_tail(int dtype, int filt_len, int64_t rows, int64_t m0, int nlevels, const void* approx, int64_t approx_row_stride,
               const void* const* details, const int64_t* detail_row_strides, const int* out_len, void* y, int64_t y_row_stride,
               const double* lo, const double* hi, hipStream_t stream);

int dwt2_fwd_choice(const mifwt_level_desc* d);
int dwt2_fwd_fused(const mifwt_level_desc* d, const void* x, void* approx, void* const* details, LevelTaps dec,
                   hipStream_t stream);

bool dwt2_inv_tile_supported(const mifwt_level_desc* d);
int dwt2_inv_tile(const mifwt_level_desc* d, const void* approx, const void* const* details, void* y, LevelTaps rec,
                  hipStream_t stream);
int dwt2_inv_choice(const mifwt_level_desc* d);
int dwt2_inv_fused(const mifwt_level_desc* d, const void* approx, const void* const* details, void* y, LevelTaps rec,
                   hipStream_t stream);

bool dwt2_inv_stream_supported(const mifwt_level_desc* d);
int dwt2_inv_stream(const mifwt_level_desc* d, const void* approx, const void* const* details, void* y,
                    const double* rec_lo, const double* rec_hi, hipStream_t stream);

bool dwt3_fwd_tile_supported(const mifwt_level_desc* d);
int dwt3_fwd_tile(const mifwt_level_desc* d, const void* x, void* approx, void* const* details,
                  const double* dec_lo, const double* dec_hi, hipStream_t stream);
bool dwt3_fwd_walk_supported(const mifwt_level_desc* d);
bool dwt3_fwd_slab_supported(const mifwt_level_desc* d);
int dwt3_fwd_slab_plan_query(const mifwt_level_desc* d, int* out, int capacity);
bool dwt3_fwd_slab_pays(const mifwt_level_desc* d);
int dwt3_fwd_slab(const mifwt_level_desc* d, const void* x, void* approx, void* const* details, const double* lo, const double* hi,
                  hipStream_t stream);
int dwt3_fwd_walk(const mifwt_level_desc* d, const void* x, void* approx, void* const* details, const double* lo, const double* hi,
                  hipStream_t stream);
bool dwt3_inv_walk_supported(const mifwt_level_desc* d);
int dwt3_inv_walk(const mifwt_level_desc* d, const void* approx, const void* const* details, void* y, const double* lo, const double* hi,
                  hipStream_t stream);
bool dwt3_inv_tile_supported(const mifwt_level_desc* d);
int dwt3_inv_tile(const mifwt_level_desc* d, const void* approx, const void* const* details, void* y, const double* lo,
                  const double* hi, hipStream_t stream);

bool plane3_route_ok(const mifwt_level_desc* d, int direction);
bool rows_route_ok(const mifwt_level_desc* d, int direction);
size_t plane3_ws_bytes(const mifwt_level_desc* d, int direction);
size_t rows_ws_bytes(const mifwt_level_desc* d, int direction);
int plane3_fwd(const mifwt_level_desc* d, const void* x, void* approx, void* const* details, const double* lo,
               const double* hi, void* ws, hipStream_t stream);
int plane3_inv(const mifwt_level_desc* d, const void* approx, const void* const* details, void* y, const double* lo,
               const double* hi, void* ws, hipStream_t stream);
int rows_fwd(const mifwt_level_desc* d, const void* x, void* approx, void* const* details, LevelTaps taps, void* ws,
             hipStream_t stream);
int rows_inv(const mifwt_level_desc* d, const void* approx, const void* const* details, void* y, LevelTaps taps, void* ws,
             hipStream_t stream);

}
```

### pytorch-wavelet-toolbox_amd/csrc/mifwt_dwt2_fwd_pyr.hip

```cpp
#include <atomic>
#include <cstring>
#include <mutex>

#include "mifwt_pyr.h"

namespace mifwt {

unsigned long long* g_pyr_prof = nullptr;

constexpr int kPyrSub = 4;
constexpr int kPyrPad = 8;
constexpr int kPyrRing = 16;
constexpr int kPyrCtl = 64;
constexpr int kPyrWaves = 16;
constexpr int kPyrMaxChunks = 5;
constexpr int kPyrMaxWG = 320;
constexpr int kPyrTailCols = 8;
constexpr int kPyrTailRows = kPyrRing + 8;
constexpr int kPyrTailBytes = kPyrTailRows * kPyrTailCols * 8;

template <int L, int NLEV>
struct PyrArgs {
  const float* x;
  float* det[NLEV];
  uint32_t doff[NLEV][3];
  uint32_t dspan[NLEV];
  float* approx;
  int64_t xs_b, ds_b[NLEV], as_b;
  int xs_h, ds_h[NLEV], as_h;
  int H[NLEV + 1], W[NLEV + 1];
  int ngroups;
  int cpg0, cpg;
  int nchunks, nbuf;
  int pitch0, pitch1, pitch2;
  int nl1, nl2, nl3;
  int nt[3], tc0[3];
  int twave;
  int mode;
  int exp;
  int l2split;
  unsigned long long* prof;
  int dbg;
  DevTapArg dt;
  FastDiv hn_div;
  uint32_t wg_start[kPyrMaxWG + 1];
  f2 tap[L];
};

template <int L>
__device__ __forceinline__ void pyr_load_win2(const unsigned char* row, f2 (&w)[L / 2 + 1]) {
  constexpr int HP = L / 2;
  if constexpr (((L - 2) & 3) == 2) {
    w[0] = *reinterpret_cast<const f2*>(row);
#pragma unroll
    for (int j = 0; j < HP / 2; ++j) {
      const f4 v = *reinterpret_cast<const f4*>(row + 8 + 16 * j);
      w[1 + 2 * j] = (f2){v.x, v.y};
      w[2 + 2 * j] = (f2){v.z, v.w};
    }
  } else {
#pragma unroll
    for (int j = 0; j < (HP + 1) / 2; ++j) {
      const f4 v = *reinterpret_cast<const f4*>(row + 16 * j);
      w[2 * j] = (f2){v.x, v.y};
      w[2 * j + 1] = (f2){v.z, v.w};
    }
  }
}

template <int NW>
__device__ __forceinline__ void pyr_role(int wave, int nl1, int nchunks, int twave, int& role, int& idx) {
  role = -1;
  idx = 0;
  if constexpr (NW == 12) {
    if (wave == twave) role = kRoleTail;
    else if (wave < 4) role = kRoleL1, idx = wave;
    else if (wave < 6) role = kRoleL2, idx = wave - 4;
    else if (wave < 8) role = kRoleL3, idx = wave - 6;
    else if (wave == 11 || (wave == 10 && nchunks >= 2)) role = kRoleLoad, idx = 11 - wave;
    return;
  }
  if (wave == twave) {
    role = kRoleTail;
  } else if (wave < 5) {
    role = kRoleL1;
    idx = nl1 < 5 ? wave : (wave == 0 ? 1 : (wave == 1 ? 0 : (wave == 2 ? 3 : (wave == 3 ? 4 : 2))));
  } else if (wave == 13) {
    role = kRoleL1;
    idx = 5;
  } else if (wave >= 5 && wave <= 7) {
    role = kRoleL2;
    idx = wave - 5;
  } else if (wave >= 9 && wave <= 11) {
    role = kRoleL3;
    idx = wave - 9;
  } else if (wave == 15 || (wave == 14 && nchunks >= 2)) {
    role = kRoleLoad;
    idx = 15 - wave;
  }
}

template <int L, int NLEV, bool PROF, int NW, bool DT = false>
__global__ void __launch_bounds__(64 * NW) dwt2_fwd_pyr_kernel(const PyrArgs<L, NLEV> a) {
  constexpr int HL = L - 2, HP = L / 2;
  constexpr int NC1 = 2;
  constexpr int NP = 2 * HL + 1;
  extern __shared__ __attribute__((aligned(16))) unsigned char smem[];

  const int lane = threadIdx.x & 63;
  const int wave = __builtin_amdgcn_readfirstlane(threadIdx.x >> 6);
  int role, widx;
  pyr_role<NW>(wave, a.nl1, a.nchunks, a.twave, role, widx);
  if (role < 0 || (role == kRoleL1 && widx >= a.nl1) || (role == kRoleL2 && (NLEV < 2 || widx >= a.nl2)) ||
      (role == kRoleL3 && (NLEV < 3 || widx >= a.nl3)))
    return;

  const int grp = blockIdx.x % a.ngroups;
  int chunk = blockIdx.x / a.ngroups;
  if (MIFWT_EXPW(a) >> 16) chunk = (chunk + ((MIFWT_EXPW(a) >> 16) & 15)) % (int)(gridDim.x / a.ngroups);
  const uint32_t g_lo = a.wg_start[chunk], g_hi = a.wg_start[chunk + 1];
  if (g_lo >= g_hi) return;
  const bool zero_mode = a.mode == MIFWT_MODE_ZERO;
  Fold1 fold;
  fold.set(a.mode);

  int cA[NLEV + 1], cB[NLEV + 1], pA[NLEV + 1], pB[NLEV + 1];
  pA[NLEV] = cA[NLEV] = grp == 0 ? 0 : a.cpg0 + (grp - 1) * a.cpg;
  pB[NLEV] = cB[NLEV] = grp == a.ngroups - 1 ? a.W[NLEV] : min(a.W[NLEV], a.cpg0 + grp * a.cpg);
#pragma unroll
  for (int l = NLEV - 1; l >= 1; --l) {
    pA[l] = 2 * pA[l + 1];
    pB[l] = pB[l + 1] == a.W[l + 1] ? a.W[l] : min(a.W[l], 2 * pB[l + 1]);
    cA[l] = max(0, 2 * cA[l + 1] - HL);
    cB[l] = min(a.W[l], 2 * cB[l + 1]);
  }
  const int o1 = pA[1] - NC1 * ((pA[1] - cA[1] + NC1 - 1) / NC1);
  const int g0 = max(0, 2 * o1 - HL) & ~3;

  int sh1 = 0;
  if constexpr (NLEV >= 2) sh1 = (2 * cA[2] - cA[1]) & 2;
  unsigned char* const stage = smem + kPyrCtl;
  unsigned char* const ring1 = stage + a.nbuf * kPyrSub * a.pitch0;
  unsigned char* const ring2 = ring1 + (kPyrRing + 1) * a.pitch1;
  unsigned char* const tailimg = ring2 + (kPyrRing + 1) * a.pitch2;

  unsigned long long waited = 0;
  const unsigned long long t_start = PROF ? __builtin_readcyclecounter() : 0;
  const unsigned long long w_start = PROF ? __builtin_amdgcn_s_memrealtime() : 0;

  f2 tap[L];
  if (role != kRoleLoad) {
    if constexpr (DT) {
#pragma unroll
      for (int m = 0; m < L; ++m) tap[m] = (f2){dtap_lo<float>(a.dt, m), dtap_hi<float>(a.dt, m)};
    } else {
#pragma unroll
      for (int m = 0; m < L; ++m) tap[m] = a.tap[m];
    }
    const int nst = a.nbuf * kPyrSub * a.pitch0 / 16, nrg = ((kPyrRing + 1) * (a.pitch1 + a.pitch2)) / 16;
    if (role == kRoleL1)
      for (int i = widx * 64 + lane; i < nst; i += 64 * a.nl1) reinterpret_cast<f4*>(stage)[i] = (f4){0.f, 0.f, 0.f, 0.f};
    if (NLEV >= 2 && role == kRoleL2)
      for (int i = widx * 64 + lane; i < nrg; i += 64 * a.nl2) reinterpret_cast<f4*>(ring1)[i] = (f4){0.f, 0.f, 0.f, 0.f};
  } else {
    if (!(MIFWT_DBG(a) & 16)) __builtin_amdgcn_s_setprio(3);
  }
  __syncthreads();

  auto run_units = [&](auto role_tag) {
  constexpr int role = decltype(role_tag)::value;
#pragma unroll 1
  for (uint32_t g = g_lo; g < g_hi;) {
    const int img = (int)a.hn_div.div(g);
    const int u_lo = (int)(g - (uint32_t)img * (uint32_t)a.H[NLEV]);
    const int u_rows = min(a.H[NLEV] - u_lo, (int)(g_hi - g));
    g += (uint32_t)u_rows;

    int rA[NLEV + 1], rB[NLEV + 1], oA[NLEV + 1], oB[NLEV + 1];
    oA[NLEV] = rA[NLEV] = u_lo;
    oB[NLEV] = rB[NLEV] = u_lo + u_rows;
#pragma unroll
    for (int l = NLEV - 1; l >= 1; --l) {
      oA[l] = 2 * oA[l + 1];
      oB[l] = oB[l + 1] == a.H[l + 1] ? a.H[l] : min(a.H[l], 2 * oB[l + 1]);
      rA[l] = max(0, 2 * rA[l + 1] - HL);
      rB[l] = min(a.H[l], 2 * rB[l + 1]);
    }
    const bool top = u_lo == 0;
    const int D2 = top ? pyr_lag2(L) : pyr_lag2_inner(L);
    const int D3 = top ? pyr_lag3(L) : pyr_lag3_inner(L);
    const int E0 = 2 * rA[1] - HL, e0_end = 2 * rB[1];
    const int npair1 = rB[1] - rA[1] + HP - 1;
    const int nsteps1 = (npair1 + 3) / 4;
    int nsteps = nsteps1, npair2 = 0, npair3 = 0;
    if constexpr (NLEV >= 2) {
      npair2 = rB[2] - rA[2] + HP - 1;
      nsteps = max(nsteps, D2 + (npair2 + 1) / 2);
    }
    if constexpr (NLEV >= 3) {
      npair3 = rB[3] - rA[3] + HP - 1;
      nsteps = max(nsteps, D3 + npair3);
    }
    const int nsub = 2 * nsteps, nsub1 = 2 * nsteps1;

    if (role == kRoleLoad) {
      const uint32_t img_bytes = ((uint32_t)(a.H[0] - 1) * (uint32_t)a.xs_h + (uint32_t)a.W[0]) * 4u;
      const rsrc_t xr = pyr_rsrc(a.x + (int64_t)img * a.xs_b, img_bytes);
      const rsrc_t xr_dead = pyr_rsrc(a.x + (int64_t)img * a.xs_b, 0);
      const uint32_t row_bytes = (uint32_t)a.xs_h * 4u;
      const int mych = (a.nchunks - widx + 1) / 2;
      uint32_t voff[3];
#pragma unroll
      for (int j = 0; j < 3; ++j) {
        const int c = g0 + 256 * (widx + 2 * j) + 4 * lane;
        voff[j] = (j < mych && c < a.W[0]) ? 4u * (uint32_t)c : kPyrOob;
      }
      auto run = [&](auto nch_tag) {
        constexpr int NCH = decltype(nch_tag)::value;
        constexpr int PER = kPyrSub * NCH;
        int ib = 0;
        auto issue = [&](int t) {
          const uint32_t buf = (uint32_t)ib * (uint32_t)(kPyrSub * a.pitch0) + (uint32_t)kPyrCtl + kPyrPad * 4u + 1024u * (uint32_t)widx;
          ib = ib + 1 == a.nbuf ? 0 : ib + 1;
          if (MIFWT_DBG(a) & 2) return;
#pragma unroll
          for (int kk = 0; kk < kPyrSub; ++kk) {
            const int e = E0 + kPyrSub * t + kk;
            const bool dead = e >= e0_end || (zero_mode && (unsigned)e >= (unsigned)a.H[0]);
            const uint32_t soff = dead ? 0u : (uint32_t)fold(e, a.H[0]) * row_bytes;
            pyr_dma_row<NCH, 0x800>(voff, dead ? xr_dead : xr, soff, buf + (uint32_t)(kk * a.pitch0));
          }
        };
        const int ahead = a.nbuf - 1;
        for (int t = 0; t < ahead; ++t)
          if (t < nsub1) issue(t);
#pragma unroll 1
        for (int t = 0; t < nsub; ++t) {
          const int later = min(ahead - 1, nsub1 - 1 - t);
          if (later >= 6) pyr_wait_vm<(6 * PER > 63 ? 63 : 6 * PER)>();
          else if (later == 5) pyr_wait_vm<(5 * PER > 63 ? 63 : 5 * PER)>();
          else if (later == 4) pyr_wait_vm<(4 * PER > 63 ? 63 : 4 * PER)>();
          else if (later == 3) pyr_wait_vm<(3 * PER > 63 ? 63 : 3 * PER)>();
          else if (later == 2) pyr_wait_vm<(2 * PER > 63 ? 63 : 2 * PER)>();
          else if (later == 1) pyr_wait_vm<PER>();
          else pyr_wait_vm<0>();
          __syncthreads();
          if (t + ahead < nsub1) issue(t + ahead);
        }
      };
      pyr_dispatch<3>(mych - 1, [&](auto k) { run(std::integral_constant<int, decltype(k)::value + 1>{}); });
    } else if (role == kRoleL1) {
      const int gmax = (cB[1] - o1 + NC1 - 1) / NC1 - 1;
      const int glane = 64 * widx + lane;
      const int G = min(glane, gmax);
      const bool real = glane <= gmax;
      const int c0 = o1 + NC1 * G;
      const uint32_t win = 4u * (uint32_t)(kPyrPad - HL + 2 * o1 - g0 + 2 * NC1 * G);
      const bool full = real && c0 >= pA[1] && c0 + 1 < pB[1];
      const bool rag1 = real && c0 >= pA[1] && c0 + 1 == pB[1];
      const uint32_t sv2 = full ? 4u * (uint32_t)c0 : kPyrOob, sv1 = rag1 ? 4u * (uint32_t)c0 : kPyrOob;
      const bool rag = __builtin_amdgcn_readfirstlane(__builtin_amdgcn_ballot_w64(rag1) != 0);
      uint32_t rw[NC1];
#pragma unroll
      for (int k = 0; k < NC1; ++k) rw[k] = (real && c0 + k >= cA[1] && c0 + k < cB[1]) ? 4u * (uint32_t)(kPyrPad + sh1 + c0 + k - cA[1]) : 0u;
      constexpr int NFP = (kPyrSub * NP + 63) / 64;
      uint32_t f_src[NFP], f_dst[NFP];
      bool f_on[NFP];
      bool f_some = false;
#pragma unroll
      for (int ps = 0; ps < NFP; ++ps) {
        f_src[ps] = f_dst[ps] = 0;
        f_on[ps] = false;
        const int wlo = 2 * (o1 + NC1 * min(64 * widx, gmax)) - HL, whi = 2 * (o1 + NC1 * min(64 * widx + 63, gmax) + NC1 - 1) + 1;
        const int fl = lane + 64 * ps;
        const int kk = fl / NP, p = fl - kk * NP;
        const bool left = p < HL;
        const int e = left ? p - HL : a.W[0] + (p - HL);
        const bool zfix = zero_mode && !left && (a.W[0] & 3) != 0;
        if (kk < kPyrSub && (!zero_mode || zfix) && (left ? wlo < 0 : whi >= a.W[0])) {
          f_on[ps] = true;
          f_some = true;
          f_src[ps] = (uint32_t)(kk * a.pitch0) + 4u * (uint32_t)(kPyrPad + (zero_mode ? 0 : fold(e, a.W[0])) - g0);
          f_dst[ps] = (uint32_t)(kk * a.pitch0) + 4u * (uint32_t)(kPyrPad + e - g0);
        }
      }
      const bool f_any = __builtin_amdgcn_readfirstlane(__builtin_amdgcn_ballot_w64(f_some) != 0) && !(MIFWT_DBG(a) & 16384);
      const uint32_t dbytes = (MIFWT_DBG(a) & 1) ? 0u : a.dspan[0] + ((uint32_t)(a.H[1] - 1) * (uint32_t)a.ds_h[0] + (uint32_t)a.W[1]) * 4u;
      const uint32_t abytes = (MIFWT_DBG(a) & 1) ? 0u : ((uint32_t)(a.H[NLEV] - 1) * (uint32_t)a.as_h + (uint32_t)a.W[NLEV]) * 4u;
      const rsrc_t rd = pyr_rsrc(a.det[0] + (int64_t)img * a.ds_b[0], dbytes);
      const rsrc_t ra = pyr_rsrc(a.approx + (int64_t)img * a.as_b, NLEV == 1 ? abytes : 0u);
      const uint32_t o0 = a.doff[0][0], o1b = a.doff[0][1], o2 = a.doff[0][2];

      PyrAcc<L, NC1> acc;
      acc.clear();
      int bi = 0;
      constexpr int NW2 = HP + 1;
      auto load_win = [&](const unsigned char* row, f2 (&w)[NW2]) { pyr_load_win2<L>(row, w); };
      auto h_pair = [&](const f2 (&wa)[NW2], const f2 (&wb)[NW2], f2 (&ha)[NC1], f2 (&hb)[NC1]) {
#pragma unroll
        for (int k = 0; k < HP; ++k) {
#pragma unroll
          for (int c = 0; c < NC1; ++c) {
            if (k == 0) {
              ha[c] = vmul_lo(tap[L - 1], wa[c]);
              hb[c] = vmul_lo(tap[L - 1], wb[c]);
            } else {
              vfma_lo(ha[c], tap[L - 1 - 2 * k], wa[c + k]);
              vfma_lo(hb[c], tap[L - 1 - 2 * k], wb[c + k]);
            }
          }
#pragma unroll
          for (int c = 0; c < NC1; ++c) {
            vfma_hi(ha[c], tap[L - 2 - 2 * k], wa[c + k]);
            vfma_hi(hb[c], tap[L - 2 - 2 * k], wb[c + k]);
          }
        }
      };

      auto step1 = [&](auto sm_tag, int s) {
        constexpr int SM = decltype(sm_tag)::value;
        pyr_static_for<2>([&](auto half_tag) {
          constexpr int half = decltype(half_tag)::value;
          pyr_barrier<PROF>(waited);
          if (s < nsteps1) {
            unsigned char* sb = stage + bi * (kPyrSub * a.pitch0);
            bi = bi + 1 == a.nbuf ? 0 : bi + 1;
            if (f_any) {
              float v[NFP];
#pragma unroll
              for (int ps = 0; ps < NFP; ++ps) v[ps] = zero_mode ? 0.f : *reinterpret_cast<const float*>(sb + f_src[ps]);
              wave_lds_fence();
#pragma unroll
              for (int ps = 0; ps < NFP; ++ps)
                if (f_on[ps]) *reinterpret_cast<float*>(sb + f_dst[ps]) = v[ps];
              wave_lds_fence();
            }
            f2 w[kPyrSub][NW2];
#pragma unroll
            for (int kk = 0; kk < kPyrSub; ++kk) load_win(sb + kk * a.pitch0 + win, w[kk]);
            pyr_static_for<kPyrSub / 2>([&](auto jj_tag) {
              constexpr int jj = decltype(jj_tag)::value;
              constexpr int j = 2 * half + jj;
              constexpr int R = (4 * SM + j) % HP;
              f2 ha[NC1], hb[NC1];
              h_pair(w[2 * jj], w[2 * jj + 1], ha, hb);
              acc.template feed<0, R>(tap, ha);
              acc.template feed<1, R>(tap, hb);
              const int i = rA[1] + 4 * s + j - (HP - 1);
              const f2 (&lo)[NC1] = acc.lo[PyrAcc<L, NC1>::done(R)];
              const f2 (&hi)[NC1] = acc.hi[PyrAcc<L, NC1>::done(R)];
              if constexpr (NLEV >= 2) {
                unsigned char* rr = ring1 + ((4 * s + j) & (kPyrRing - 1)) * a.pitch1;
#pragma unroll
                for (int k = 0; k < NC1; ++k) *reinterpret_cast<float*>(rr + (i < rB[1] ? rw[k] : 0u)) = lo[k].x;
              }
              const bool own = i >= oA[1] && i < oB[1];
              const uint32_t v2 = own ? sv2 : kPyrOob;
              const uint32_t so = own ? (uint32_t)i * (uint32_t)a.ds_h[0] * 4u : 0u;
              __builtin_amdgcn_raw_buffer_store_b64((f2){hi[0].x, hi[1].x}, rd, v2, so + o0, MIFWT_ST_AUX);
              __builtin_amdgcn_raw_buffer_store_b64((f2){lo[0].y, lo[1].y}, rd, v2, so + o1b, MIFWT_ST_AUX);
              __builtin_amdgcn_raw_buffer_store_b64((f2){hi[0].y, hi[1].y}, rd, v2, so + o2, MIFWT_ST_AUX);
              if (rag) {
                const uint32_t v1 = own ? sv1 : kPyrOob;
                pyr_store1(hi[0].x, rd, v1, so + o0);
                pyr_store1(lo[0].y, rd, v1, so + o1b);
                pyr_store1(hi[0].y, rd, v1, so + o2);
              }
              if constexpr (NLEV == 1) {
                const uint32_t sa = own ? (uint32_t)i * (uint32_t)a.as_h * 4u : 0u;
                __builtin_amdgcn_raw_buffer_store_b64((f2){lo[0].x, lo[1].x}, ra, v2, sa, MIFWT_ST_AUX);
                if (rag) pyr_store1(lo[0].x, ra, own ? sv1 : kPyrOob, sa);
              }
            });
          }
        });
      };
      int sm = 0;
#pragma unroll 1
      for (int s = 0; s < nsteps; ++s) {
        if constexpr (HP == 3 || HP == 5) {
          pyr_dispatch<HP>(sm, [&](auto t) { step1(t, s); });
          sm = sm == HP - 1 ? 0 : sm + 1;
        } else {
          step1(std::integral_constant<int, 0>{}, s);
        }
      }
    } else if (NLEV >= 2 && role == kRoleL2) {
      if constexpr (NLEV >= 2) {
        const int gmax = (cB[2] - cA[2] + 1) / 2 - 1;
        const int glane = 64 * widx + lane;
        const int G = min(glane, gmax);
        const bool real = glane <= gmax;
        const int c0 = cA[2] + 2 * G;
        const uint32_t win = 4u * (uint32_t)(kPyrPad + sh1 - HL + 2 * c0 - cA[1]);
        const bool full = real && c0 >= pA[2] && c0 + 1 < pB[2];
        const bool rag1 = real && c0 >= pA[2] && c0 + 1 == pB[2];
        const uint32_t sv2 = full ? 4u * (uint32_t)c0 : kPyrOob, sv1 = rag1 ? 4u * (uint32_t)c0 : kPyrOob;
        const bool rag = __builtin_amdgcn_readfirstlane(__builtin_amdgcn_ballot_w64(rag1) != 0);
        uint32_t rw[2];
#pragma unroll
        for (int k = 0; k < 2; ++k) rw[k] = (real && c0 + k < cB[2]) ? 4u * (uint32_t)(kPyrPad + c0 + k - cA[2]) : 0u;
        uint32_t f_src = 0, f_dst = 0;
        bool f_on = false;
        const int f_r = lane / NP;
        {
          const int wlo = 2 * (cA[2] + 2 * min(64 * widx, gmax)) - HL, whi = 2 * (cA[2] + 2 * min(64 * widx + 63, gmax) + 1) + 1;
          const int p = lane - f_r * NP;
          const bool left = p < HL;
          const int e = left ? p - HL : a.W[1] + (p - HL);
          if (f_r < 4 && !zero_mode && (left ? wlo < 0 : whi >= a.W[1])) {
            f_on = true;
            f_src = 4u * (uint32_t)(kPyrPad + sh1 + fold(e, a.W[1]) - cA[1]);
            f_dst = 4u * (uint32_t)(kPyrPad + sh1 + e - cA[1]);
          }
        }
        const bool f_any = __builtin_amdgcn_readfirstlane(__builtin_amdgcn_ballot_w64(f_on) != 0) && !(MIFWT_DBG(a) & 32768);
        const uint32_t dbytes = (MIFWT_DBG(a) & 1) ? 0u : a.dspan[1] + ((uint32_t)(a.H[2] - 1) * (uint32_t)a.ds_h[1] + (uint32_t)a.W[2]) * 4u;
        const uint32_t abytes = (MIFWT_DBG(a) & 1) ? 0u : ((uint32_t)(a.H[NLEV] - 1) * (uint32_t)a.as_h + (uint32_t)a.W[NLEV]) * 4u;
        const rsrc_t rd = pyr_rsrc(a.det[1] + (int64_t)img * a.ds_b[1], dbytes);
        const rsrc_t ra = pyr_rsrc(a.approx + (int64_t)img * a.as_b, NLEV == 2 ? abytes : 0u);
        const uint32_t o0 = a.doff[1][0], o1b = a.doff[1][1], o2 = a.doff[1][2];
        const int ro1 = HP - 1 - rA[1];
        const int E1 = 2 * rA[2] - HL;
        PyrAcc<L, 2> acc;
        acc.clear();
        constexpr int NW2 = HP + 1;
        auto load_win = [&](const unsigned char* row, f2 (&w)[NW2]) { pyr_load_win2<L>(row, w); };
        auto h_pair = [&](const f2 (&wa)[NW2], const f2 (&wb)[NW2], f2 (&ha)[2], f2 (&hb)[2]) {
#pragma unroll
          for (int k = 0; k < HP; ++k) {
#pragma unroll
            for (int c = 0; c < 2; ++c) {
              if (k == 0) {
                ha[c] = vmul_lo(tap[L - 1], wa[c]);
                hb[c] = vmul_lo(tap[L - 1], wb[c]);
              } else {
                vfma_lo(ha[c], tap[L - 1 - 2 * k], wa[c + k]);
                vfma_lo(hb[c], tap[L - 1 - 2 * k], wb[c + k]);
              }
            }
#pragma unroll
            for (int c = 0; c < 2; ++c) {
              vfma_hi(ha[c], tap[L - 2 - 2 * k], wa[c + k]);
              vfma_hi(hb[c], tap[L - 2 - 2 * k], wb[c + k]);
            }
          }
        };
        if ((MIFWT_EXPW(a) & 3) == 1) __builtin_amdgcn_s_setprio(1);
        if ((MIFWT_EXPW(a) & 3) == 2) __builtin_amdgcn_s_setprio(2);
        if ((MIFWT_EXPW(a) & 3) == 3) __builtin_amdgcn_s_setprio(3);
        unsigned long long tsec[4] = {0, 0, 0, 0};
        auto do_pair = [&](auto r_tag, auto jj_tag, int s, const uint32_t (&so_r)[4]) {
          constexpr int R = decltype(r_tag)::value, jj = decltype(jj_tag)::value;
          unsigned long long t0 = 0;
          if constexpr (PROF) t0 = __builtin_readcyclecounter();
          f2 wa[NW2], wb[NW2];
          load_win(ring1 + so_r[2 * jj] + win, wa);
          load_win(ring1 + so_r[2 * jj + 1] + win, wb);
          if constexpr (PROF) {
            asm volatile("s_waitcnt lgkmcnt(0)" ::: "memory");
            const unsigned long long t1 = __builtin_readcyclecounter();
            tsec[0] += t1 - t0;
            t0 = t1;
          }
          f2 ha[2], hb[2];
          h_pair(wa, wb, ha, hb);
          acc.template feed<0, R>(tap, ha);
          acc.template feed<1, R>(tap, hb);
          if constexpr (PROF) {
            asm volatile("" ::: "memory");
            const unsigned long long t1 = __builtin_readcyclecounter();
            tsec[1] += t1 - t0;
            t0 = t1;
          }
          const int p = 2 * (s - D2) + jj;
          const int i = rA[2] + p - (HP - 1);
          const f2 (&lo)[2] = acc.lo[PyrAcc<L, 2>::done(R)];
          const f2 (&hi)[2] = acc.hi[PyrAcc<L, 2>::done(R)];
          if constexpr (NLEV >= 3) {
            unsigned char* rr = ring2 + (p & (kPyrRing - 1)) * a.pitch2;
            const bool mine = i < rB[2];
            *reinterpret_cast<float*>(rr + (mine ? rw[0] : 0u)) = lo[0].x;
            *reinterpret_cast<float*>(rr + (mine ? rw[1] : 0u)) = lo[1].x;
          }
          const bool own = i >= oA[2] && i < oB[2];
          const uint32_t v2 = own ? sv2 : kPyrOob;
          const uint32_t so = own ? (uint32_t)i * (uint32_t)a.ds_h[1] * 4u : 0u;
          __builtin_amdgcn_raw_buffer_store_b64((f2){hi[0].x, hi[1].x}, rd, v2, so + o0, MIFWT_ST_AUX);
          __builtin_amdgcn_raw_buffer_store_b64((f2){lo[0].y, lo[1].y}, rd, v2, so + o1b, MIFWT_ST_AUX);
          __builtin_amdgcn_raw_buffer_store_b64((f2){hi[0].y, hi[1].y}, rd, v2, so + o2, MIFWT_ST_AUX);
          if (rag) {
            const uint32_t v1 = own ? sv1 : kPyrOob;
            pyr_store1(hi[0].x, rd, v1, so + o0);
            pyr_store1(lo[0].y, rd, v1, so + o1b);
            pyr_store1(hi[0].y, rd, v1, so + o2);
          }
          if constexpr (NLEV == 2) {
            const uint32_t sa = own ? (uint32_t)i * (uint32_t)a.as_h * 4u : 0u;
            __builtin_amdgcn_raw_buffer_store_b64((f2){lo[0].x, lo[1].x}, ra, v2, sa, MIFWT_ST_AUX);
            if (rag) pyr_store1(lo[0].x, ra, own ? sv1 : kPyrOob, sa);
          }
          if constexpr (PROF) {
            asm volatile("" ::: "memory");
            tsec[2] += __builtin_readcyclecounter() - t0;
          }
        };
        auto half = [&](auto r_tag, auto jj_tag, int s, const uint32_t (&so_r)[4]) {
          constexpr int jj = decltype(jj_tag)::value;
          unsigned long long tp = 0;
          if constexpr (PROF) tp = __builtin_readcyclecounter();
          if (f_any) {
            const uint32_t fo = f_r == 0 ? so_r[0] : (f_r == 1 ? so_r[1] : (f_r == 2 ? so_r[2] : so_r[3]));
            const float v = *reinterpret_cast<const float*>(ring1 + fo + f_src);
            wave_lds_fence();
            if (f_on && (f_r >> 1) == jj) *reinterpret_cast<float*>(ring1 + fo + f_dst) = v;
            wave_lds_fence();
          }
          if constexpr (PROF) tsec[3] += __builtin_readcyclecounter() - tp;
          do_pair(r_tag, jj_tag, s, so_r);
        };
        auto step2 = [&](auto r0_tag, int s) {
          constexpr int R0 = decltype(r0_tag)::value;
          using RA = std::integral_constant<int, R0 % HP>;
          using RB = std::integral_constant<int, (R0 + 1) % HP>;
          pyr_barrier<PROF>(waited);
          const bool act = 2 * (s - D2) < npair2 && !(MIFWT_DBG(a) & 4);
          uint32_t so_r[4] = {0u, 0u, 0u, 0u};
          bool early = false;
          if (act) {
            int qmax0 = 0;
            const int e0 = E1 + 4 * (s - D2);
            if (e0 >= 0 && e0 + 3 < a.H[1]) {
              const int q0 = e0 + ro1;
#pragma unroll
              for (int r = 0; r < 4; ++r) so_r[r] = (uint32_t)(((q0 + r) & (kPyrRing - 1)) * a.pitch1);
              qmax0 = q0 + 1;
            } else {
#pragma unroll
              for (int r = 0; r < 4; ++r) {
                const int e = e0 + r;
                const bool dead = zero_mode && (unsigned)e >= (unsigned)a.H[1];
                const int q = fold(e, a.H[1]) + ro1;
                so_r[r] = (uint32_t)((dead ? kPyrRing : (q & (kPyrRing - 1))) * a.pitch1);
                if (r < 2 && !dead) qmax0 = max(qmax0, q);
              }
            }
            if (NW == 12 && widx == 0 && a.twave >= 0 && lane == 0) *reinterpret_cast<u4*>(smem) = (u4){so_r[0], so_r[1], so_r[2], so_r[3]};
            early = a.l2split && qmax0 <= 4 * s - 1;
            if (early) half(RA{}, std::integral_constant<int, 0>{}, s, so_r);
          }
          pyr_barrier<PROF>(waited);
          if (act) {
            if (!early) half(RA{}, std::integral_constant<int, 0>{}, s, so_r);
            half(RB{}, std::integral_constant<int, 1>{}, s, so_r);
          }
        };
        {
          int s = 0;
#pragma unroll 1
          for (; s < D2 && s < nsteps; ++s) {
            pyr_barrier<PROF>(waited);
            pyr_barrier<PROF>(waited);
          }
          constexpr int PERIOD = (HP % 2 == 0) ? (HP / 2 > 0 ? HP / 2 : 1) : HP;
#pragma unroll 1
          for (; s < nsteps; s += PERIOD) {
            pyr_static_for<PERIOD>([&](auto k_tag) {
              constexpr int k = decltype(k_tag)::value;
              if (k == 0 || s + k < nsteps) step2(std::integral_constant<int, (2 * k) % HP>{}, s + k);
            });
          }
        }
        if (PROF && widx == 0 && lane == 0) {
          unsigned long long* o = MIFWT_PROFP(a) + ((size_t)blockIdx.x * kPyrWaves + 14) * 2;
          o[0] += tsec[0], o[1] += tsec[1], o[2] += tsec[2], o[3] += tsec[3];
        }
      }
    } else if (NLEV >= 3 && role == kRoleL3) {
      if constexpr (NLEV >= 3) {
        const int gmax = cB[3] - cA[3] - 1;
        const int G = min(64 * widx + lane, gmax);
        const bool real = 64 * widx + lane <= gmax;
        const int c = cA[3] + G;
        const uint32_t win = 4u * (uint32_t)(kPyrPad - HL + 2 * c - cA[2]);
        const uint32_t sv = real && c >= pA[3] && c < pB[3] ? 4u * (uint32_t)c : kPyrOob;
        uint32_t f_src = 0, f_dst = 0;
        bool f_on = false;
        const int f_r = lane / NP;
        {
          const int wlo = 2 * (cA[3] + min(64 * widx, gmax)) - HL, whi = 2 * (cA[3] + min(64 * widx + 63, gmax)) + 1;
          const int p = lane - f_r * NP;
          const bool left = p < HL;
          const int e = left ? p - HL : a.W[2] + (p - HL);
          if (f_r < 2 && !zero_mode && (left ? wlo < 0 : whi >= a.W[2])) {
            f_on = true;
            f_src = 4u * (uint32_t)(kPyrPad + fold(e, a.W[2]) - cA[2]);
            f_dst = 4u * (uint32_t)(kPyrPad + e - cA[2]);
          }
        }
        const bool f_any = __builtin_amdgcn_readfirstlane(__builtin_amdgcn_ballot_w64(f_on) != 0) && !(MIFWT_DBG(a) & 32768);
        const uint32_t dbytes = (MIFWT_DBG(a) & 1) ? 0u : a.dspan[2] + ((uint32_t)(a.H[3] - 1) * (uint32_t)a.ds_h[2] + (uint32_t)a.W[3]) * 4u;
        const uint32_t abytes = (MIFWT_DBG(a) & 1) ? 0u : ((uint32_t)(a.H[3] - 1) * (uint32_t)a.as_h + (uint32_t)a.W[3]) * 4u;
        const rsrc_t rd = pyr_rsrc(a.det[2] + (int64_t)img * a.ds_b[2], dbytes);
        const rsrc_t ra = pyr_rsrc(a.approx + (int64_t)img * a.as_b, abytes);
        const uint32_t o0 = a.doff[2][0], o1b = a.doff[2][1], o2 = a.doff[2][2];
        const int ro2 = HP - 1 - rA[2];
        const int E2 = 2 * rA[3] - HL;
        PyrAcc<L, 1> acc;
        acc.clear();
        auto load_win = [&](const unsigned char* row, f2 (&w)[HP]) {
#pragma unroll
          for (int k = 0; k < HP; ++k) w[k] = *reinterpret_cast<const f2*>(row + 8 * k);
        };
        auto h_pair = [&](const f2 (&wa)[HP], const f2 (&wb)[HP], f2 (&ha)[1], f2 (&hb)[1]) {
#pragma unroll
          for (int k = 0; k < HP; ++k) {
            if (k == 0) {
              ha[0] = vmul_lo(tap[L - 1], wa[0]);
              hb[0] = vmul_lo(tap[L - 1], wb[0]);
            } else {
              vfma_lo(ha[0], tap[L - 1 - 2 * k], wa[k]);
              vfma_lo(hb[0], tap[L - 1 - 2 * k], wb[k]);
            }
            vfma_hi(ha[0], tap[L - 2 - 2 * k], wa[k]);
            vfma_hi(hb[0], tap[L - 2 - 2 * k], wb[k]);
          }
        };
        auto step3 = [&](auto r_tag, int s) {
          constexpr int R = decltype(r_tag)::value;
          pyr_barrier<PROF>(waited);
          if (s - D3 < npair3 && !(MIFWT_DBG(a) & 4)) {
            uint32_t so_r[2];
            const int e0 = E2 + 2 * (s - D3);
            if (e0 >= 0 && e0 + 1 < a.H[2]) {
              so_r[0] = (uint32_t)(((e0 + ro2) & (kPyrRing - 1)) * a.pitch2);
              so_r[1] = (uint32_t)(((e0 + 1 + ro2) & (kPyrRing - 1)) * a.pitch2);
            } else {
#pragma unroll
              for (int r = 0; r < 2; ++r) {
                const int e = e0 + r;
                const bool dead = zero_mode && (unsigned)e >= (unsigned)a.H[2];
                so_r[r] = (uint32_t)((dead ? kPyrRing : ((fold(e, a.H[2]) + ro2) & (kPyrRing - 1))) * a.pitch2);
              }
            }
            if (NW == 12 && widx == 0 && a.twave >= 0 && lane == 0) *reinterpret_cast<u2*>(smem + 16) = (u2){so_r[0], so_r[1]};
            if (f_any) {
              const uint32_t fo = f_r == 0 ? so_r[0] : so_r[1];
              const float v = *reinterpret_cast<const float*>(ring2 + fo + f_src);
              wave_lds_fence();
              if (f_on) *reinterpret_cast<float*>(ring2 + fo + f_dst) = v;
              wave_lds_fence();
            }
            f2 w[2][HP];
            load_win(ring2 + so_r[0] + win, w[0]);
            load_win(ring2 + so_r[1] + win, w[1]);
            f2 ha[1], hb[1];
            h_pair(w[0], w[1], ha, hb);
            acc.template feed<0, R>(tap, ha);
            acc.template feed<1, R>(tap, hb);
            const int i = rA[3] + (s - D3) - (HP - 1);
            const f2 lo = acc.lo[PyrAcc<L, 1>::done(R)][0], hi = acc.hi[PyrAcc<L, 1>::done(R)][0];
            const bool own = i >= oA[3] && i < oB[3];
            const uint32_t v = own ? sv : kPyrOob;
            const uint32_t so = own ? (uint32_t)i * (uint32_t)a.ds_h[2] * 4u : 0u;
            pyr_store1(hi.x, rd, v, so + o0);
            pyr_store1(lo.y, rd, v, so + o1b);
            pyr_store1(hi.y, rd, v, so + o2);
            pyr_store1(lo.x, ra, v, own ? (uint32_t)i * (uint32_t)a.as_h * 4u : 0u);
          }
          pyr_barrier<PROF>(waited);
        };
        {
          int s = 0;
#pragma unroll 1
          for (; s < D3 && s < nsteps; ++s) {
            pyr_barrier<PROF>(waited);
            pyr_barrier<PROF>(waited);
          }
#pragma unroll 1
          for (; s < nsteps; s += HP) {
            pyr_static_for<HP>([&](auto k_tag) {
              constexpr int k = decltype(k_tag)::value;
              if (k == 0 || s + k < nsteps) step3(k_tag, s + k);
            });
          }
        }
      }
    }
    else if (NW == 12 && role == kRoleTail) {
      if constexpr (NW == 12) {
      const int nt1 = a.nt[0], nt2 = NLEV >= 2 ? a.nt[1] : 0, nt3 = NLEV >= 3 ? a.nt[2] : 0;
      int j_lvl = 0, j_r = 0, j_c = 0;
      {
        int idx = lane;
        if (idx < 4 * nt1) {
          j_lvl = 1, j_r = idx / max(nt1, 1), j_c = idx - j_r * nt1;
        } else {
          idx -= 4 * nt1;
          if (idx < 4 * nt2) {
            j_lvl = 2, j_r = idx / max(nt2, 1), j_c = idx - j_r * nt2;
          } else {
            idx -= 4 * nt2;
            if (idx < 2 * nt3) j_lvl = 3, j_r = idx / max(nt3, 1), j_c = idx - j_r * nt3;
          }
        }
      }
      uint32_t soff[L];
      {
        const int Wp = j_lvl <= 1 ? a.W[0] : (j_lvl == 2 ? a.W[NLEV >= 2 ? 1 : 0] : a.W[NLEV >= 3 ? 2 : 0]);
        const int tc = j_lvl <= 1 ? a.tc0[0] : (j_lvl == 2 ? a.tc0[1] : a.tc0[2]);
        const int body0 = j_lvl <= 1 ? kPyrPad - g0 : (j_lvl == 2 ? kPyrPad + sh1 - cA[1] : kPyrPad - cA[NLEV >= 2 ? 2 : 1]);
#pragma unroll
        for (int k = 0; k < L; ++k) {
          const int x = 2 * (tc + j_c) - HL + k;
          const bool oob = (unsigned)x >= (unsigned)Wp;
          soff[k] = (oob && zero_mode) ? 4u : 4u * (uint32_t)(body0 + (zero_mode ? x : fold(x, Wp)));
        }
      }
      const uint32_t m_l1 = j_lvl == 1 ? ~0u : 0u, m_l2 = j_lvl == 2 ? ~0u : 0u, m_l3 = j_lvl == 3 ? ~0u : 0u;
      const uint32_t m_r0 = j_r == 0 ? ~0u : 0u, m_r1 = j_r == 1 ? ~0u : 0u, m_r2 = j_r == 2 ? ~0u : 0u, m_r3 = j_r == 3 ? ~0u : 0u;
      const uint32_t j_rp0 = (uint32_t)j_r * (uint32_t)a.pitch0, r1off = (uint32_t)(ring1 - smem), r2off = (uint32_t)(ring2 - smem);
      const uint32_t img1 = (uint32_t)(tailimg - smem) + (uint32_t)(max(j_lvl, 1) - 1) * (uint32_t)kPyrTailBytes + 8u * (uint32_t)j_c;
      int k_lvl = 0, k_o = 0, k_c = 0;
      {
        int idx = lane;
        if (idx < 2 * nt1) {
          k_lvl = 1, k_o = idx / max(nt1, 1), k_c = idx - k_o * nt1;
        } else {
          idx -= 2 * nt1;
          if (idx < 2 * nt2) {
            k_lvl = 2, k_o = idx / max(nt2, 1), k_c = idx - k_o * nt2;
          } else {
            idx -= 2 * nt2;
            if (idx < nt3) k_lvl = 3, k_c = idx;
          }
        }
      }
      constexpr int I2 = NLEV >= 2 ? 1 : 0, I3 = NLEV >= 3 ? 2 : 0;
      const int kC = (k_lvl <= 1 ? a.tc0[0] : (k_lvl == 2 ? a.tc0[1] : a.tc0[2])) + k_c;
      const int k_rA = k_lvl <= 1 ? rA[1] : (k_lvl == 2 ? rA[I2 + 1] : rA[I3 + 1]);
      const int k_rB = k_lvl <= 1 ? rB[1] : (k_lvl == 2 ? rB[I2 + 1] : rB[I3 + 1]);
      const int k_oA = k_lvl <= 1 ? oA[1] : (k_lvl == 2 ? oA[I2 + 1] : oA[I3 + 1]);
      const int k_oB = k_lvl <= 1 ? oB[1] : (k_lvl == 2 ? oB[I2 + 1] : oB[I3 + 1]);
      const bool k_last = k_lvl == NLEV;
      const int kl = max(k_lvl, 1) - 1;
      unsigned char* const k_dptr = reinterpret_cast<unsigned char*>((kl == 0 ? a.det[0] : (kl == 1 ? a.det[I2] : a.det[I3])) +
                                                                      (int64_t)img * (kl == 0 ? a.ds_b[0] : (kl == 1 ? a.ds_b[I2] : a.ds_b[I3])) + kC);
      const uint32_t k_dpitch = 4u * (uint32_t)(kl == 0 ? a.ds_h[0] : (kl == 1 ? a.ds_h[I2] : a.ds_h[I3]));
      const uint32_t k_o0 = kl == 0 ? a.doff[0][0] : (kl == 1 ? a.doff[I2][0] : a.doff[I3][0]);
      const uint32_t k_o1 = kl == 0 ? a.doff[0][1] : (kl == 1 ? a.doff[I2][1] : a.doff[I3][1]);
      const uint32_t k_o2 = kl == 0 ? a.doff[0][2] : (kl == 1 ? a.doff[I2][2] : a.doff[I3][2]);
      unsigned char* const k_aptr = reinterpret_cast<unsigned char*>(a.approx + (int64_t)img * a.as_b + kC);
      const uint32_t k_apitch = 4u * (uint32_t)a.as_h;
      const uint32_t k_ring = k_lvl <= 1 ? (uint32_t)(ring1 - smem) + 4u * (uint32_t)(kPyrPad + sh1 + kC - cA[1])
                                         : (uint32_t)(ring2 - smem) + 4u * (uint32_t)(kPyrPad + kC - cA[I2 + 1]);
      const uint32_t k_rpitch = k_lvl <= 1 ? (uint32_t)a.pitch1 : (uint32_t)a.pitch2;
      const uint32_t img2 = (uint32_t)(tailimg - smem) + (uint32_t)kl * (uint32_t)kPyrTailBytes + 8u * (uint32_t)k_c;
      const uint32_t n_l1 = k_lvl == 1 ? ~0u : 0u, n_l2 = k_lvl == 2 ? ~0u : 0u, n_l3 = k_lvl == 3 ? ~0u : 0u;
      const bool nostore = MIFWT_DBG(a) & 1;
      int bi = 0;
      if (((MIFWT_EXPW(a) >> 4) & 3) == 0) __builtin_amdgcn_s_setprio(2);
      if (((MIFWT_EXPW(a) >> 4) & 3) == 1) __builtin_amdgcn_s_setprio(1);
      if (((MIFWT_EXPW(a) >> 4) & 3) == 3) __builtin_amdgcn_s_setprio(3);

      auto run_half = [&](int s, int half, bool act1, bool act2, bool act3, uint32_t rb1, const u4 v2, const u2 v3) {
        const bool on1 = (j_lvl == 1 && act1) || (j_lvl == 2 && act2) || (j_lvl == 3 && act3);
        if (on1) {
          const uint32_t rowb = (m_l1 & (rb1 + j_rp0)) | (m_l2 & (r1off + ((m_r0 & v2.x) | (m_r1 & v2.y) | (m_r2 & v2.z) | (m_r3 & v2.w)))) |
                                (m_l3 & (r2off + ((m_r0 & v3.x) | (m_r1 & v3.y))));
          const int seq = j_r + (int)((m_l1 & (uint32_t)(8 * s + 4 * half)) | (m_l2 & (uint32_t)(4 * (s - D2))) | (m_l3 & (uint32_t)(2 * (s - D3))));
          float xs[L];
#pragma unroll
          for (int k = 0; k < L; ++k) xs[k] = *reinterpret_cast<const float*>(smem + rowb + soff[k]);
          f2 h;
#pragma unroll
          for (int k = 0; k < HP; ++k) {
            const f2 pr = (f2){xs[2 * k], xs[2 * k + 1]};
            if (k == 0) h = vmul_lo(tap[L - 1], pr);
            else vfma_lo(h, tap[L - 1 - 2 * k], pr);
            vfma_hi(h, tap[L - 2 - 2 * k], pr);
          }
          const uint32_t slot = (uint32_t)seq & (kPyrRing - 1);
          *reinterpret_cast<f2*>(smem + img1 + slot * (8u * kPyrTailCols)) = h;
          *reinterpret_cast<f2*>(smem + img1 + (slot < 8u ? slot + kPyrRing : slot) * (8u * kPyrTailCols)) = h;
        }
        wave_lds_fence();
        const int P = k_o + (int)((n_l1 & (uint32_t)(4 * s + 2 * half)) | (n_l2 & (uint32_t)(2 * (s - D2))) | (n_l3 & (uint32_t)(s - D3)));
        const bool on2 = ((k_lvl == 1 && act1) || (k_lvl == 2 && act2) || (k_lvl == 3 && act3)) && P >= HP - 1;
        if (on2) {
          const uint32_t b = (uint32_t)(2 * P + 2 - L) & (kPyrRing - 1);
          const unsigned char* hp = smem + img2 + b * (8u * kPyrTailCols);
          f2 hv[L];
#pragma unroll
          for (int n = 0; n < L; ++n) hv[n] = *reinterpret_cast<const f2*>(hp + n * (8 * kPyrTailCols));
          f2 lo = vmul_lo(tap[L - 1], hv[0]), hi = vmul_hi(tap[L - 1], hv[0]);
#pragma unroll
          for (int n = 1; n < L; ++n) {
            vfma_lo(lo, tap[L - 1 - n], hv[n]);
            vfma_hi(hi, tap[L - 1 - n], hv[n]);
          }
          const int i = k_rA + P - (HP - 1);
          if (!k_last && i < k_rB) *reinterpret_cast<float*>(smem + k_ring + ((uint32_t)P & (kPyrRing - 1)) * k_rpitch) = lo.x;
          if (i >= k_oA && i < k_oB && !nostore) {
            unsigned char* drow = k_dptr + (size_t)i * k_dpitch;
            *reinterpret_cast<float*>(drow + k_o0) = hi.x;
            *reinterpret_cast<float*>(drow + k_o1) = lo.y;
            *reinterpret_cast<float*>(drow + k_o2) = hi.y;
            if (k_last) *reinterpret_cast<float*>(k_aptr + (size_t)i * k_apitch) = lo.x;
          }
        }
      };
#pragma unroll 1
      for (int s = 0; s < nsteps; ++s) {
        const bool act1 = s < nsteps1;
        const bool act2 = NLEV >= 2 && s >= D2 && 2 * (s - D2) < npair2 && !(MIFWT_DBG(a) & 4);
        const bool act3 = NLEV >= 3 && s >= D3 && s - D3 < npair3 && !(MIFWT_DBG(a) & 4);
        pyr_barrier<PROF>(waited);
        uint32_t rb1 = (uint32_t)(stage - smem) + (uint32_t)bi * (uint32_t)(kPyrSub * a.pitch0);
        if (act1) bi = bi + 1 == a.nbuf ? 0 : bi + 1;
        run_half(s, 0, act1, false, false, rb1, (u4){0u, 0u, 0u, 0u}, (u2){0u, 0u});
        pyr_barrier<PROF>(waited);
        const u4 v2 = *reinterpret_cast<const u4*>(smem);
        const u2 v3 = *reinterpret_cast<const u2*>(smem + 16);
        rb1 = (uint32_t)(stage - smem) + (uint32_t)bi * (uint32_t)(kPyrSub * a.pitch0);
        if (act1) bi = bi + 1 == a.nbuf ? 0 : bi + 1;
        run_half(s, 1, act1, act2, act3, rb1, v2, v3);
      }
      }
    }
    __syncthreads();
  }
  };
  if (role == kRoleLoad) run_units(std::integral_constant<int, kRoleLoad>{});
  else if (role == kRoleL1) run_units(std::integral_constant<int, kRoleL1>{});
  else if (role == kRoleL2) run_units(std::integral_constant<int, kRoleL2>{});
  else if (role == kRoleL3) run_units(std::integral_constant<int, kRoleL3>{});
  else run_units(std::integral_constant<int, kRoleTail>{});

  if (PROF && lane == 0 && role != kRoleLoad) {
    unsigned long long* o = MIFWT_PROFP(a) + ((size_t)blockIdx.x * kPyrWaves + wave) * 2;
    o[0] = __builtin_readcyclecounter() - t_start;
    o[1] = waited;
    if (wave == 0) {
      unsigned long long* w = MIFWT_PROFP(a) + ((size_t)blockIdx.x * kPyrWaves + 8) * 2;
      w[0] = w_start;
      w[1] = __builtin_amdgcn_s_memrealtime();
      w[8] = __builtin_amdgcn_s_getreg((31 << 11) | 4);
      w[9] = __builtin_amdgcn_s_getreg((31 << 11) | 20);
      w[10] = g_lo;
      w[11] = g_hi;
    }
  }
}

struct PyrPlan {
  int ngroups, cpg0, cpg, nchunks, nbuf, pitch0, pitch1, pitch2, nl1, nl2, nl3, lds;
  int nt[3], tc0[3], twave;
  int nwaves;
  int nwg;
  uint32_t wg_start[kPyrMaxWG + 1];
};

static int pyr_group_cols_search(int L, int nlev, bool first);
static int pyr_group_cols(int L, int nlev, bool first) {
  static std::atomic<int> memo[6][4][2];
  const int li = L / 2;
  if (li < 0 || li > 5 || nlev < 0 || nlev > 3) return pyr_group_cols_search(L, nlev, first);
  std::atomic<int>& m = memo[li][nlev][first ? 1 : 0];
  int v = m.load(std::memory_order_relaxed);
  if (v == 0) {
    v = pyr_group_cols_search(L, nlev, first) + 1;
    m.store(v, std::memory_order_relaxed);
  }
  return v - 1;
}
static int pyr_group_cols_search(int L, int nlev, bool first) {
  const int nc1 = 2;
  const int HL = first ? 0 : L - 2;
  int best = 0;
  for (int n = 1; n <= 4 * 192; ++n) {
    int m = n;
    bool ok = true;
    for (int l = nlev; l >= 1 && ok; --l) {
      const int cap = l == 1 ? 6 * 128 - nc1 : (l == 2 ? 3 * 128 : 3 * 64);
      ok = m <= cap;
      if (l > 1) m = 2 * m + HL;
    }
    if (ok && 2 * m + HL + 3 <= kPyrMaxChunks * 256) best = n;
  }
  return best;
}

struct PyrGeom {
  int L, nlev, H[4];
  int parity;
};
constexpr double kUnitStart = 1.0;
static double pyr_unit_time(const PyrGeom& gm, int u_lo, int u_hi) {
  const int ex = exp_word();
  const double kDrainStep = ((ex >> 8) & 15) ? 0.25 + 0.05 * ((ex >> 8) & 15) : 0.45;
  const double kTopBonus = ((ex >> 12) & 15) ? 0.1 * ((ex >> 12) & 15) : 1.0;
  const int L = gm.L, HL = L - 2, HP = L / 2, nlev = gm.nlev;
  int rA[4], rB[4];
  rA[nlev] = u_lo;
  rB[nlev] = u_hi;
  for (int l = nlev - 1; l >= 1; --l) {
    rA[l] = std::max(0, 2 * rA[l + 1] - HL);
    rB[l] = std::min(gm.H[l], 2 * rB[l + 1]);
  }
  const bool top = u_lo == 0;
  const int D2 = top ? pyr_lag2(L) : pyr_lag2_inner(L), D3 = top ? pyr_lag3(L) : pyr_lag3_inner(L);
  const int nsteps1 = (rB[1] - rA[1] + HP - 1 + 3) / 4;
  int nsteps = nsteps1;
  if (nlev >= 2) nsteps = std::max(nsteps, D2 + (rB[2] - rA[2] + HP - 1 + 1) / 2);
  if (nlev >= 3) nsteps = std::max(nsteps, D3 + rB[3] - rA[3] + HP - 1);
  return nsteps1 + kDrainStep * (nsteps - nsteps1) + kUnitStart - (top ? kTopBonus : 0.0);
}

constexpr int kMinRows = 8;
static int pyr_cut(const PyrGeom& gm, int64_t B, double budget, int gmax, uint32_t* cut) {
  const int HN = gm.H[gm.nlev];
  int64_t img = 0;
  int row = 0, n = 0;
  if (cut) cut[0] = 0;
  while (img < B) {
    if (n == gmax) return gmax + 1;
    double used = 0;
    bool first = true;
    while (img < B) {
      const double rest = pyr_unit_time(gm, row, HN);
      if (used + rest <= budget) {
        used += rest;
        ++img;
        row = 0;
        first = false;
        continue;
      }
      int lo = 0, hi = HN - row - kMinRows;
      if (hi >= kMinRows) {
        while (lo < hi) {
          const int mid = (lo + hi + 1) / 2;
          if (used + pyr_unit_time(gm, row, row + mid) <= budget) lo = mid;
          else hi = mid - 1;
        }
      } else {
        lo = 0;
      }
      if (lo >= kMinRows) {
        row += lo;
        first = false;
      } else if (first) {
        return gmax + 1;
      }
      break;
    }
    ++n;
    if (cut) cut[n] = (uint32_t)(img * HN + row);
  }
  return n;
}

static void pyr_schedule(const PyrGeom& gm, int64_t B, int gwant, PyrPlan* p) {
  const int HN = gm.H[gm.nlev];
  struct Entry {
    int L, nlev, H[4], gwant, ex, n, parity;
    int64_t B;
    uint32_t cut[kPyrMaxWG + 1];
  };
  constexpr int kEntries = 16;
  static std::mutex mu;
  static Entry cache[kEntries];
  static int used = 0, next = 0;
  const int ex = exp_word();
  auto same = [&](const Entry& e) {
    return e.L == gm.L && e.nlev == gm.nlev && e.H[1] == gm.H[1] && e.H[2] == gm.H[2] && e.H[3] == gm.H[3] && e.gwant == gwant && e.ex == ex && e.parity == gm.parity && e.B == B;
  };
  {
    std::lock_guard<std::mutex> lk(mu);
    for (int i = 0; i < used; ++i)
      if (same(cache[i])) {
        p->nwg = cache[i].n;
        std::copy(cache[i].cut, cache[i].cut + cache[i].n + 1, p->wg_start);
        return;
      }
  }
  const int g = std::max(1, std::min(gwant, kPyrMaxWG));
  double lo = 0, hi = pyr_unit_time(gm, 0, HN);
  hi = hi * (double)((B + g - 1) / g) + hi;
  for (int it = 0; it < 40 && hi - lo > 0.02; ++it) {
    const double mid = 0.5 * (lo + hi);
    if (pyr_cut(gm, B, mid, g, nullptr) <= g) hi = mid;
    else lo = mid;
  }
  p->nwg = pyr_cut(gm, B, hi, g, p->wg_start);
  {
    std::lock_guard<std::mutex> lk(mu);
    Entry& e = cache[next];
    next = (next + 1) % kEntries;
    used = std::min(used + 1, kEntries);
    e.L = gm.L, e.nlev = gm.nlev, e.gwant = gwant, e.ex = ex, e.B = B, e.n = p->nwg, e.parity = gm.parity;
    for (int l = 0; l < 4; ++l) e.H[l] = gm.H[l];
    std::copy(p->wg_start, p->wg_start + p->nwg + 1, e.cut);
  }
}

static bool pyr_plan_compute(int nlev, const mifwt_level_desc* const* d, PyrPlan* p) {
  const int nc1 = 2;
  const int L = d[0]->filt_len, HL = L - 2;
  const int WN = (int)d[nlev - 1]->coef_extent[1], HN = (int)d[nlev - 1]->coef_extent[0];
  const int min_cols = HL + 2;
  if (WN < min_cols || HN < 2 * (HL + 2)) return false;
  if (d[0]->batch * (int64_t)HN >= (int64_t(1) << 31)) return false;
  p->cpg0 = pyr_group_cols(L, nlev, true);
  p->cpg = pyr_group_cols(L, nlev, false);
  if (nlev == 1) {
    p->cpg0 &= ~1;
    p->cpg &= ~1;
  }
  if (p->cpg < min_cols) return false;
  if (WN <= p->cpg0) {
    p->ngroups = 1;
  } else {
    p->ngroups = 1 + (WN - p->cpg0 + p->cpg - 1) / p->cpg;
    int base = (WN + p->ngroups - 1) / p->ngroups;
    if (nlev == 1) base = (base + 1) & ~1;
    if (base < p->cpg) {
      p->cpg0 = base;
      p->cpg = base;
    }
    const int last = WN - p->cpg0 - (p->ngroups - 2) * p->cpg;
    if (last < min_cols) p->cpg0 -= min_cols - last;
  }
  int n[4] = {0, 0, 0, 0}, body = 0;
  const int W0 = (int)d[0]->sig_extent[1];
  for (int g = 0; g < p->ngroups; ++g) {
    int cA = g == 0 ? 0 : p->cpg0 + (g - 1) * p->cpg, cB = g == p->ngroups - 1 ? WN : std::min(WN, p->cpg0 + g * p->cpg);
    int pA = cA;
    for (int l = nlev; l >= 1; --l) {
      n[l] = std::max(n[l], cB - cA + (l == 1 ? 2 : 0));
      if (l > 1) {
        const int Wl = (int)d[l - 2]->coef_extent[1];
        pA = 2 * pA;
        cA = std::max(0, 2 * cA - HL);
        cB = std::min(Wl, 2 * cB);
      }
    }
    const int o1 = pA - nc1 * ((pA - cA + nc1 - 1) / nc1);
    if (o1 < 0) return false;
    const int g0 = std::max(0, 2 * o1 - HL) & ~3;
    body = std::max(body, std::min(W0, 2 * cB) - g0);
  }
  p->nl1 = (n[1] + 64 * nc1 - 1) / (64 * nc1);
  p->nl2 = nlev >= 2 ? (n[2] + 127) / 128 : 0;
  p->nl3 = nlev >= 3 ? (n[3] + 63) / 64 : 0;
  if (p->nl1 > 6 || p->nl2 > 3 || p->nl3 > 3) return false;
  p->twave = -1;
  for (int l = 0; l < 3; ++l) p->nt[l] = p->tc0[l] = 0;
  if (p->ngroups == 1 && !(g_options[MIFWT_OPT_DEBUG] & 524288)) {
    const int cap[3] = {64 * nc1, 128, 64}, ntmax[3] = {4, 6, 6};
    int* nl[3] = {&p->nl1, &p->nl2, &p->nl3};
    bool any = false;
    for (int l = 0; l < nlev; ++l) {
      const int cols = (int)d[l]->coef_extent[1], full = cols / cap[l], rem = cols - full * cap[l];
      if (full >= 1 && rem >= 1 && rem <= ntmax[l]) {
        p->nt[l] = rem;
        p->tc0[l] = full * cap[l];
        *nl[l] = full;
        any = true;
      }
    }
    const bool fits12 = p->nl1 <= 4 && p->nl2 <= 2 && p->nl3 <= 2 && !(g_options[MIFWT_OPT_DEBUG] & 1048576);
    if (any && fits12) {
      p->twave = 9;
    } else if (any) {
      for (int l = 0; l < 3; ++l) p->nt[l] = p->tc0[l] = 0;
      p->nl1 = (n[1] + 64 * nc1 - 1) / (64 * nc1);
      p->nl2 = nlev >= 2 ? (n[2] + 127) / 128 : 0;
      p->nl3 = nlev >= 3 ? (n[3] + 63) / 64 : 0;
    }
  }
  p->nwaves = (p->nl1 <= 4 && p->nl2 <= 2 && p->nl3 <= 2 && !(g_options[MIFWT_OPT_DEBUG] & 1048576)) ? 12 : 16;
  p->nchunks = (body + 255) / 256;
  if (p->nchunks < 1 || p->nchunks > kPyrMaxChunks) return false;
  p->pitch0 = (kPyrPad + 256 * p->nchunks + 8) * 4;
  p->pitch1 = nlev >= 2 ? ((kPyrPad + n[1] + HL + 8 + 3) & ~3) * 4 : 0;
  p->pitch2 = nlev >= 3 ? ((kPyrPad + n[2] + HL + 8 + 3) & ~3) * 4 : 0;
  const int rings = (kPyrRing + 1) * (p->pitch1 + p->pitch2) + (p->twave >= 0 ? 3 * kPyrTailBytes : 0);
  p->nbuf = g_options[MIFWT_OPT_PREFETCH_PAIRS] > 1 ? std::min(8, g_options[MIFWT_OPT_PREFETCH_PAIRS]) : 4;
  const int lds_cap = 160 * 1024, per_loader = (p->nchunks + 1) / 2;
  while (p->nbuf > 2 && (kPyrCtl + p->nbuf * kPyrSub * p->pitch0 + rings > lds_cap || (p->nbuf - 1) * kPyrSub * per_loader > 63)) --p->nbuf;
  p->lds = kPyrCtl + p->nbuf * kPyrSub * p->pitch0 + rings;
  if (p->lds > lds_cap) return false;
  if (p->lds < 82 * 1024) p->lds = 82 * 1024;
  int dev = 0, ncu = 256;
  if (hipGetDevice(&dev) == hipSuccess) {
    static std::atomic<int> ncu_of[64];
    int v = ncu_of[dev & 63].load(std::memory_order_relaxed);
    if (v == 0 && hipDeviceGetAttribute(&v, hipDeviceAttributeMultiprocessorCount, dev) == hipSuccess && v > 0) ncu_of[dev & 63].store(v, std::memory_order_relaxed);
    if (v > 0) ncu = v;
  }
  PyrGeom gm;
  gm.L = L;
  gm.nlev = nlev;
  gm.parity = p->ngroups == 1 ? 1 : 0;
  gm.H[0] = (int)d[0]->sig_extent[0];
  for (int l = 1; l <= 3; ++l) gm.H[l] = l <= nlev ? (int)d[l - 1]->coef_extent[0] : 0;
  const int64_t rows = d[0]->batch * (int64_t)HN;
  int64_t gwant = std::max(1, ncu / p->ngroups);
  if (g_options[MIFWT_OPT_PAIR_ROWS] > 0) gwant = (rows + g_options[MIFWT_OPT_PAIR_ROWS] - 1) / g_options[MIFWT_OPT_PAIR_ROWS];
  if (g_options[MIFWT_OPT_PYR_WGS] > 0) gwant = g_options[MIFWT_OPT_PYR_WGS];
  gwant = std::min<int64_t>(gwant, std::max<int64_t>(1, rows / kMinRows));
  pyr_schedule(gm, d[0]->batch, (int)std::min<int64_t>(gwant, kPyrMaxWG), p);
  return p->nwg >= 1 && p->nwg <= kPyrMaxWG && p->wg_start[p->nwg] == (uint32_t)rows;
}

static bool pyr_plan(int nlev, const mifwt_level_desc* const* d, PyrPlan* p) {
  struct Memo {
    bool valid = false, ok = false;
    int nlev = 0, dev = -1;
    int opts[6] = {0, 0, 0, 0, 0, 0};
    mifwt_level_desc desc[3];
    PyrPlan plan;
  };
  static thread_local Memo m;
  const int opts[6] = {g_options[MIFWT_OPT_DEBUG], g_options[MIFWT_OPT_PREFETCH_PAIRS], g_options[MIFWT_OPT_PAIR_ROWS], g_options[MIFWT_OPT_PYR_WGS],
                       exp_word(), 0};
  int dev = 0;
  (void)hipGetDevice(&dev);
  if (nlev >= 1 && nlev <= 3 && m.valid && m.nlev == nlev && m.dev == dev && memcmp(m.opts, opts, sizeof(opts)) == 0) {
    bool same = true;
    for (int l = 0; l < nlev && same; ++l) same = memcmp(&m.desc[l], d[l], sizeof(mifwt_level_desc)) == 0;
    if (same) {
      if (m.ok) *p = m.plan;
      return m.ok;
    }
  }
  const bool ok = pyr_plan_compute(nlev, d, p);
  if (nlev >= 1 && nlev <= 3) {
    m.nlev = nlev;
    m.dev = dev;
    memcpy(m.opts, opts, sizeof(opts));
    for (int l = 0; l < nlev; ++l) m.desc[l] = *d[l];
    m.ok = ok;
    if (ok) m.plan = *p;
    m.valid = true;
  }
  return ok;
}

bool dwt2_fwd_pyr_supported(int nlev, const mifwt_level_desc* const* d) {
  if (nlev < 1 || nlev > 3 || g_options[MIFWT_OPT_PAIR_MODE] == 2 || g_options[MIFWT_OPT_PYRAMID_MODE] == 2) return false;
  const mifwt_level_desc* d0 = d[0];
  const int L = d0->filt_len;
  if (d0->ndim != 2 || d0->dtype != MIFWT_F32 || L < 2 || L > 10 || (L & 1)) return false;
  if ((L == 10 || d0->mode == MIFWT_MODE_PERIODIC) && nlev != 1) return false;
  if (d0->mode < 0 || d0->mode > MIFWT_MODE_SYMMETRIC) return false;
  if (d0->batch < 1 || d0->sig_stride[2] != 1) return false;
  const int64_t lim = int64_t(1) << 29;
  if (d0->sig_extent[0] * d0->sig_stride[1] >= lim) return false;
  for (int l = 0; l < nlev; ++l) {
    const mifwt_level_desc* dl = d[l];
    if (dl->ndim != 2 || dl->dtype != MIFWT_F32 || dl->filt_len != L || dl->mode != d0->mode || dl->batch != d0->batch) return false;
    if (dl->detail_stride[2] != 1 || dl->coef_extent[0] * dl->detail_stride[1] >= lim) return false;
    for (int ax = 0; ax < 2; ++ax) {
      const int64_t n = l == 0 ? d0->sig_extent[ax] : d[l - 1]->coef_extent[ax];
      if (dl->sig_extent[ax] != n || dl->coef_extent[ax] != (n + L - 1) / 2) return false;
      if (n < 2 * L) return false;
    }
  }
  const mifwt_level_desc* dn = d[nlev - 1];
  if (dn->approx_stride[2] != 1 || dn->coef_extent[0] * dn->approx_stride[1] >= lim) return false;
  PyrPlan p;
  if (!pyr_plan(nlev, d, &p)) return false;
  if (L == 10 && p.nwaves != 12) return false;
  if (g_options[MIFWT_OPT_PYRAMID_MODE] != 1 && (p.ngroups > 2 || d0->sig_extent[1] < 448)) return false;
  if (g_options[MIFWT_OPT_PYRAMID_MODE] != 1 && nlev == 1 && (d0->sig_extent[1] < 896 || d0->sig_extent[1] > 1280 || d0->sig_extent[0] < 256)) return false;
  return true;
}

int dwt2_fwd_pyr_schedule(int nlev, const mifwt_level_desc* const* d, uint32_t* wg_start, int capacity) {
  if (!dwt2_fwd_pyr_supported(nlev, d)) return MIFWT_ERR_UNSUPPORTED;
  PyrPlan p;
  if (!pyr_plan(nlev, d, &p)) return MIFWT_ERR_UNSUPPORTED;
  if (capacity < p.nwg + 1) return MIFWT_ERR_BADARG;
  std::copy(p.wg_start, p.wg_start + p.nwg + 1, wg_start);
  return p.nwg;
}

template <int L, int NLEV>
static int launch_pyr(const mifwt_level_desc* const* d, const void* x, void* const* const* details, void* approx, LevelTaps t,
                      hipStream_t stream) {
  PyrPlan p;
  if (!pyr_plan(NLEV, d, &p)) return MIFWT_ERR_UNSUPPORTED;
  PyrArgs<L, NLEV> a;
  a.x = static_cast<const float*>(x);
  a.xs_b = d[0]->sig_stride[0];
  a.xs_h = (int)d[0]->sig_stride[1];
  a.H[0] = (int)d[0]->sig_extent[0];
  a.W[0] = (int)d[0]->sig_extent[1];
  for (int l = 0; l < NLEV; ++l) {
    uintptr_t lo_p = reinterpret_cast<uintptr_t>(details[l][0]);
    for (int b = 1; b < 3; ++b) lo_p = std::min(lo_p, reinterpret_cast<uintptr_t>(details[l][b]));
    a.det[l] = reinterpret_cast<float*>(lo_p);
    a.dspan[l] = 0;
    for (int b = 0; b < 3; ++b) {
      const uintptr_t off = reinterpret_cast<uintptr_t>(details[l][b]) - lo_p;
      if (off >= (uintptr_t(1) << 30) || (off & 3)) return MIFWT_ERR_UNSUPPORTED;
      a.doff[l][b] = (uint32_t)off;
      a.dspan[l] = std::max(a.dspan[l], (uint32_t)off);
    }
    a.ds_b[l] = d[l]->detail_stride[0];
    a.ds_h[l] = (int)d[l]->detail_stride[1];
    a.H[l + 1] = (int)d[l]->coef_extent[0];
    a.W[l + 1] = (int)d[l]->coef_extent[1];
  }
  a.approx = static_cast<float*>(approx);
  a.as_b = d[NLEV - 1]->approx_stride[0];
  a.as_h = (int)d[NLEV - 1]->approx_stride[1];
  a.ngroups = p.ngroups;
  a.cpg0 = p.cpg0;
  a.cpg = p.cpg;
  a.nchunks = p.nchunks;
  a.nbuf = p.nbuf;
  a.pitch0 = p.pitch0;
  a.pitch1 = p.pitch1;
  a.pitch2 = p.pitch2;
  a.nl1 = p.nl1;
  a.nl2 = p.nl2;
  a.nl3 = p.nl3;
  for (int l = 0; l < 3; ++l) a.nt[l] = p.nt[l], a.tc0[l] = p.tc0[l];
  a.twave = p.twave;
  a.mode = d[0]->mode;
  a.dbg = g_options[MIFWT_OPT_DEBUG];
  if ((MIFWT_DBG(a) & 65536) && a.nl1 > 1) --a.nl1;
  if ((MIFWT_DBG(a) & 131072) && a.nl2 > 1) --a.nl2;
  if ((MIFWT_DBG(a) & 262144) && a.nl3 > 1) --a.nl3;
  a.prof = g_pyr_prof;
  a.l2split = (g_options[MIFWT_OPT_DEBUG] & 8192) ? 0 : 1;
  a.exp = exp_word();
  a.hn_div = make_fastdiv((uint32_t)a.H[NLEV]);
  std::copy(p.wg_start, p.wg_start + p.nwg + 1, a.wg_start);
  for (int k = p.nwg + 1; k <= kPyrMaxWG; ++k) a.wg_start[k] = a.wg_start[p.nwg];
  for (int m = 0; m < L; ++m) a.tap[m] = (f2){(float)t.tap_lo(m), (float)t.tap_hi(m)};
  a.dt = t.dev_arg(L);
  const int64_t nwg = (int64_t)p.nwg * p.ngroups;
  constexpr bool kCanProf = kDiag && L == 8 && NLEV == 3;
  constexpr bool kHas16 = L <= 8;
  static DynLdsOnce lds_once12, lds_once16, lds_once_prof12, lds_once_prof16;
  if (!lds_once12.ensure(reinterpret_cast<const void*>(&dwt2_fwd_pyr_kernel<L, NLEV, false, 12>), 160 * 1024)) return MIFWT_ERR_LAUNCH;
  if (kCanProf && !lds_once_prof12.ensure(reinterpret_cast<const void*>(&dwt2_fwd_pyr_kernel<L, NLEV, kCanProf, 12>), 160 * 1024)) return MIFWT_ERR_LAUNCH;
  count_launch(MIFWT_VARIANT_FWD_PYR_ST8);
  const dim3 grid((unsigned)nwg), block(64 * p.nwaves);
  if (a.dt.lo) {
    if constexpr (NLEV == 1) {
      static DynLdsOnce lds_dt12, lds_dt16;
      if (p.nwaves == 12) {
        if (!lds_dt12.ensure(reinterpret_cast<const void*>(&dwt2_fwd_pyr_kernel<L, 1, false, 12, true>), 160 * 1024)) return MIFWT_ERR_LAUNCH;
        hipLaunchKernelGGL((dwt2_fwd_pyr_kernel<L, 1, false, 12, true>), grid, block, p.lds, stream, a);
      } else if constexpr (kHas16) {
        if (!lds_dt16.ensure(reinterpret_cast<const void*>(&dwt2_fwd_pyr_kernel<L, 1, false, 16, true>), 160 * 1024)) return MIFWT_ERR_LAUNCH;
        hipLaunchKernelGGL((dwt2_fwd_pyr_kernel<L, 1, false, 16, true>), grid, block, p.lds, stream, a);
      } else {
        return MIFWT_ERR_UNSUPPORTED;
      }
      return hipGetLastError() == hipSuccess ? MIFWT_OK : MIFWT_ERR_LAUNCH;
    }
    return MIFWT_ERR_UNSUPPORTED;
  }
  if (p.nwaves == 12) {
    if (kCanProf && MIFWT_PROFP(a)) hipLaunchKernelGGL((dwt2_fwd_pyr_kernel<L, NLEV, kCanProf, 12>), grid, block, p.lds, stream, a);
    else hipLaunchKernelGGL((dwt2_fwd_pyr_kernel<L, NLEV, false, 12>), grid, block, p.lds, stream, a);
  } else if constexpr (kHas16) {
    if (!lds_once16.ensure(reinterpret_cast<const void*>(&dwt2_fwd_pyr_kernel<L, NLEV, false, 16>), 160 * 1024)) return MIFWT_ERR_LAUNCH;
    if (kCanProf && !lds_once_prof16.ensure(reinterpret_cast<const void*>(&dwt2_fwd_pyr_kernel<L, NLEV, kCanProf, 16>), 160 * 1024)) return MIFWT_ERR_LAUNCH;
    if (kCanProf && MIFWT_PROFP(a)) hipLaunchKernelGGL((dwt2_fwd_pyr_kernel<L, NLEV, kCanProf, 16>), grid, block, p.lds, stream, a);
    else hipLaunchKernelGGL((dwt2_fwd_pyr_kernel<L, NLEV, false, 16>), grid, block, p.lds, stream, a);
  } else {
    return MIFWT_ERR_UNSUPPORTED;
  }
  return hipGetLastError() == hipSuccess ? MIFWT_OK : MIFWT_ERR_LAUNCH;
}

template <int L>
static int launch_pyr_l(int nlev, const mifwt_level_desc* const* d, const void* x, void* const* const* details, void* approx,
                        LevelTaps t, hipStream_t stream) {
  switch (nlev) {
    case 1: return launch_pyr<L, 1>(d, x, details, approx, t, stream);
    case 2: return launch_pyr<L, 2>(d, x, details, approx, t, stream);
    case 3: return launch_pyr<L, 3>(d, x, details, approx, t, stream);
    default: return MIFWT_ERR_UNSUPPORTED;
  }
}

int dwt2_fwd_pyr(int nlev, const mifwt_level_desc* const* d, const void* x, void* const* const* details, void* approx, LevelTaps t,
                 hipStream_t stream) {
  if (!dwt2_fwd_pyr_supported(nlev, d)) return MIFWT_ERR_UNSUPPORTED;
  switch (d[0]->filt_len) {
    case 2: return launch_pyr_l<2>(nlev, d, x, details, approx, t, stream);
    case 4: return launch_pyr_l<4>(nlev, d, x, details, approx, t, stream);
    case 6: return launch_pyr_l<6>(nlev, d, x, details, approx, t, stream);
    case 8: return launch_pyr_l<8>(nlev, d, x, details, approx, t, stream);
    case 10: return nlev == 1 ? launch_pyr<10, 1>(d, x, details, approx, t, stream) : MIFWT_ERR_UNSUPPORTED;
    default: return MIFWT_ERR_UNSUPPORTED;
  }
}

}
```

### pytorch-wavelet-toolbox_amd/csrc/mifwt_pyr.h

```cpp
#pragma once
#include <type_traits>

#include "mifwt_stream.h"

namespace mifwt {

extern unsigned long long* g_pyr_prof;

enum PyrRole { kRoleL1 = 0, kRoleL2 = 1, kRoleL3 = 2, kRoleLoad = 3, kRoleTail = 4 };

constexpr uint32_t kPyrOob = 0x80000000u;

constexpr int pyr_cdiv(int a, int b) { return a <= 0 ? 0 : (a + b - 1) / b; }
constexpr int pyr_lag2_inner(int L) { return (L / 2) / 4 + 1; }
constexpr int pyr_lag2(int L) { const int b = pyr_cdiv(L - 2 + L / 2 - 2, 4); return b > pyr_lag2_inner(L) ? b : pyr_lag2_inner(L); }
constexpr int pyr_lag3_inner(int L) { return pyr_lag2_inner(L) + 1 + pyr_cdiv(L / 2 - 1, 2); }
constexpr int pyr_lag3(int L) { const int a = L / 2 - 1, b = L - 2 + L / 2 - 2; return pyr_lag2(L) + 1 + pyr_cdiv(a > b ? a : b, 2); }

#ifndef MIFWT_ST_AUX
#define MIFWT_ST_AUX 0
#endif
typedef __amdgpu_buffer_rsrc_t rsrc_t;
__device__ __forceinline__ rsrc_t pyr_rsrc(const void* p, uint32_t bytes) {
  return __builtin_amdgcn_make_buffer_rsrc(const_cast<void*>(p), 0, (int)bytes, 0x00020000);
}
__device__ __forceinline__ void pyr_store1(float v, rsrc_t rsrc, uint32_t voff, uint32_t soff) {
  __builtin_amdgcn_raw_buffer_store_b32(__builtin_bit_cast(uint32_t, v), rsrc, voff, soff, MIFWT_ST_AUX);
}
#ifndef MIFWT_PYR_ST16_POLICY
#define MIFWT_PYR_ST16_POLICY "nt"
#endif
__device__ __forceinline__ void pyr_store4(const f4 data, rsrc_t rsrc, uint32_t voff, uint32_t soff) {
  asm volatile("buffer_store_dwordx4 %0, %1, %2, %3 offen " MIFWT_PYR_ST16_POLICY "\n\ts_nop 1" ::"v"(data), "v"(voff), "s"(rsrc), "s"(soff) : "memory");
}
__device__ __forceinline__ void pyr_permlane32_swap(float& x, float& y) {
  asm volatile("s_nop 1\n\tv_permlane32_swap_b32 %0, %1\n\ts_nop 0" : "+v"(x), "+v"(y));
}
__device__ __forceinline__ f4 pyr_swap_rows(float a0, float a1, float b0, float b1) {
  pyr_permlane32_swap(a0, b0);
  pyr_permlane32_swap(a1, b1);
  return (f4){a0, a1, b0, b1};
}
struct PyrSt16 {
  uint32_t v16;
  int cq0, wend;
  bool rag;
  __device__ __forceinline__ void set(int lane, int cq0_, int wend_) {
    cq0 = cq0_;
    wend = wend_;
    const int cq = cq0 + 4 * (lane & 31), nin = wend - cq;
    v16 = nin >= 4 ? 4u * (uint32_t)cq : kPyrOob;
    rag = __builtin_amdgcn_readfirstlane(__builtin_amdgcn_ballot_w64(nin > 0 && nin < 4) != 0);
  }
  __device__ __forceinline__ void rows(int lane, int i0, int oA, int oB, uint32_t pitch_bytes, uint32_t& v4, uint32_t& dx, bool& mine, uint32_t& so) const {
    const bool own0 = i0 >= oA && i0 < oB, own1 = i0 + 1 >= oA && i0 + 1 < oB, upper = lane >= 32;
    so = (own0 || own1) ? (uint32_t)(own0 ? i0 : i0 + 1) * pitch_bytes : 0u;
    mine = upper ? own1 : own0;
    dx = (upper && own0) ? pitch_bytes : 0u;
    v4 = mine ? v16 + dx : kPyrOob;
  }
  __device__ __forceinline__ void band(int lane, uint32_t v4, uint32_t dx, bool mine, float a0, float a1, float b0, float b1, rsrc_t r, uint32_t soff) const {
    const f4 t = pyr_swap_rows(a0, a1, b0, b1);
    pyr_store4(t, r, v4, soff);
    if (rag) {
      const int cq = cq0 + 4 * (lane & 31), nin = wend - cq;
      const uint32_t vrl = (mine && nin > 0 && nin < 4) ? 4u * (uint32_t)cq + dx : kPyrOob;
      pyr_store1(t.x, r, vrl, soff);
      pyr_store1(t.y, r, nin >= 2 ? vrl : kPyrOob, soff + 4u);
      pyr_store1(t.z, r, nin >= 3 ? vrl : kPyrOob, soff + 8u);
    }
  }
};

#ifndef MIFWT_PYR_DMA_POLICY
#define MIFWT_PYR_DMA_POLICY "nt"
#endif
template <int NCH, int STR>
__device__ __forceinline__ void pyr_dma_row(const uint32_t (&voff)[3], rsrc_t rsrc, uint32_t soff, uint32_t lds0) {
  uint32_t keep;
  if constexpr (NCH == 1) {
    asm volatile("s_mov_b32 %0, m0\n\ts_mov_b32 m0, %4\n\ts_nop 0\n\tbuffer_load_dwordx4 %1, %2, %3 offen " MIFWT_PYR_DMA_POLICY " lds\n\ts_mov_b32 m0, %0"
                 : "=&s"(keep) : "v"(voff[0]), "s"(rsrc), "s"(soff), "s"(lds0) : "memory");
  } else if constexpr (NCH == 2) {
    asm volatile("s_mov_b32 %0, m0\n\ts_mov_b32 m0, %5\n\ts_nop 0\n\tbuffer_load_dwordx4 %1, %3, %4 offen " MIFWT_PYR_DMA_POLICY " lds\n\t"
                 "s_add_u32 m0, m0, %6\n\ts_nop 0\n\tbuffer_load_dwordx4 %2, %3, %4 offen " MIFWT_PYR_DMA_POLICY " lds\n\ts_mov_b32 m0, %0"
                 : "=&s"(keep) : "v"(voff[0]), "v"(voff[1]), "s"(rsrc), "s"(soff), "s"(lds0), "n"(STR) : "memory", "scc");
  } else {
    static_assert(NCH == 3, "at most three requests per row and loader");
    asm volatile("s_mov_b32 %0, m0\n\ts_mov_b32 m0, %6\n\ts_nop 0\n\tbuffer_load_dwordx4 %1, %4, %5 offen " MIFWT_PYR_DMA_POLICY " lds\n\t"
                 "s_add_u32 m0, m0, %7\n\ts_nop 0\n\tbuffer_load_dwordx4 %2, %4, %5 offen " MIFWT_PYR_DMA_POLICY " lds\n\t"
                 "s_add_u32 m0, m0, %7\n\ts_nop 0\n\tbuffer_load_dwordx4 %3, %4, %5 offen " MIFWT_PYR_DMA_POLICY " lds\n\ts_mov_b32 m0, %0"
                 : "=&s"(keep) : "v"(voff[0]), "v"(voff[1]), "v"(voff[2]), "s"(rsrc), "s"(soff), "s"(lds0), "n"(STR) : "memory", "scc");
  }
}

template <bool PROF>
__device__ __forceinline__ void pyr_barrier(unsigned long long& waited) {
  if constexpr (PROF) {
    const unsigned long long t0 = __builtin_readcyclecounter();
    __syncthreads();
    waited += __builtin_readcyclecounter() - t0;
  } else {
    __syncthreads();
  }
}
template <int N>
__device__ __forceinline__ void pyr_wait_vm() {
  asm volatile("s_waitcnt vmcnt(%0)" ::"n"(N) : "memory");
}

__device__ __forceinline__ void vfma_lo(f2& acc, const f2 tap, const f2 pair) { pkfma_lo(acc, tap, pair); }
__device__ __forceinline__ void vfma_hi(f2& acc, const f2 tap, const f2 pair) { pkfma_hi(acc, tap, pair); }
__device__ __forceinline__ f2 vmul_lo(const f2 tap, const f2 pair) { return pkmul_lo(tap, pair); }
__device__ __forceinline__ f2 vmul_hi(const f2 tap, const f2 pair) { return pkmul_hi(tap, pair); }

__device__ __forceinline__ void vfma_lo(d2& acc, const d2 tap, const d2 pair) { afma_lo(acc, tap, pair); }
__device__ __forceinline__ void vfma_hi(d2& acc, const d2 tap, const d2 pair) { afma_hi(acc, tap, pair); }
__device__ __forceinline__ d2 vmul_lo(const d2 tap, const d2 pair) { return amul_lo(tap, pair); }
__device__ __forceinline__ d2 vmul_hi(const d2 tap, const d2 pair) { return amul_hi(tap, pair); }

template <int L, int NC, typename V = f2>
struct PyrAcc {
  static constexpr int HP = L / 2;
  V lo[HP][NC], hi[HP][NC];
  __device__ __forceinline__ void clear() {
#pragma unroll
    for (int q = 0; q < HP; ++q)
#pragma unroll
      for (int c = 0; c < NC; ++c) lo[q][c] = hi[q][c] = V{};
  }
  template <int PH, int R>
  __device__ __forceinline__ void feed(const V (&tap)[L], const V (&hv)[NC]) {
#pragma unroll
    for (int q = 0; q < HP; ++q) {
      const int sl = (R - q + HP) % HP;
      const int m = L - 1 - 2 * q - PH;
#pragma unroll
      for (int c = 0; c < NC; ++c) {
        if (q == 0 && PH == 0) {
          lo[sl][c] = vmul_lo(tap[m], hv[c]);
          hi[sl][c] = vmul_hi(tap[m], hv[c]);
        } else {
          vfma_lo(lo[sl][c], tap[m], hv[c]);
          vfma_hi(hi[sl][c], tap[m], hv[c]);
        }
      }
    }
  }
  static constexpr int done(int R) { return (R + 1) % HP; }
};

template <int N, int I = 0, typename F>
__device__ __forceinline__ void pyr_static_for(F&& f) {
  if constexpr (I < N) {
    f(std::integral_constant<int, I>{});
    pyr_static_for<N, I + 1>(f);
  }
}

template <int N, typename F>
__device__ __forceinline__ void pyr_dispatch(int r, F&& f) {
  if constexpr (N == 1) {
    f(std::integral_constant<int, 0>{});
  } else if constexpr (N == 2) {
    if (r == 0) f(std::integral_constant<int, 0>{});
    else f(std::integral_constant<int, 1>{});
  } else if constexpr (N == 3) {
    if (r == 0) f(std::integral_constant<int, 0>{});
    else if (r == 1) f(std::integral_constant<int, 1>{});
    else f(std::integral_constant<int, 2>{});
  } else if constexpr (N == 4) {
    if (r < 2) {
      if (r == 0) f(std::integral_constant<int, 0>{});
      else f(std::integral_constant<int, 1>{});
    } else {
      if (r == 2) f(std::integral_constant<int, 2>{});
      else f(std::integral_constant<int, 3>{});
    }
  } else {
    static_assert(N == 5, "filter lengths up to 10");
    if (r < 2) {
      if (r == 0) f(std::integral_constant<int, 0>{});
      else f(std::integral_constant<int, 1>{});
    } else if (r == 2) {
      f(std::integral_constant<int, 2>{});
    } else {
      if (r == 3) f(std::integral_constant<int, 3>{});
      else f(std::integral_constant<int, 4>{});
    }
  }
}

}
```

Measured before the change: 701,400 Msamples/s.

## Skip halo-only detail FMAs and burst level-3 tail in pyramid units

Moves per-unit planning into a shared host/device PyrUnitPlan. Rows in the halo prefix (rA..oA) feed only the low-pass accumulators and skip high-pass FMAs and detail stores ("lean" steps). The level-3 pass no longer stretches the shared barrier cadence, so leftover level-3 pairs run after the main loop with fewer barriers. The price is more template variants, extra branches and more complex barrier counting, which must match across roles or the kernel deadlocks.

```diff
diff --git a/__graft_entry__.py b/__graft_entry__.py
--- a/__graft_entry__.py
+++ b/__graft_entry__.py
@@ -107,7 +107,7 @@
     from ptwt_amd import _engine
 
     lib = _engine.load_library()
-    for sym in ("mifwt_dwt_fwd", "mifwt_dwt_inv", "mifwt_dwt_fwd_adjoint", "mifwt_dwt_inv_adjoint", "mifwt_swt_fwd", "mifwt_swt_inv", "mifwt_tap_correlate", "mifwt_tap_correlate_dilated", "mifwt_dwt2_fwd_pair", "mifwt_dwt2_fwd_pair_supported", "mifwt_dwt2_inv_pair", "mifwt_dwt2_inv_pair_supported", "mifwt_dwt2_fwd_pyramid", "mifwt_dwt2_fwd_pyramid_supported", "mifwt_dwt2_fwd_pyramid_schedule", "mifwt_dwt3_fwd_slab_plan", "mifwt_dwt_fwd_dtaps", "mifwt_dwt_inv_dtaps", "mifwt_dwt_fwd_adjoint_dtaps", "mifwt_dwt_inv_adjoint_dtaps", "mifwt_workspace_bytes_dtaps", "mifwt_kernel_id_dtaps", "mifwt_dwt2_inv_pyramid", "mifwt_dwt2_inv_pyramid_supported", "mifwt_dwt1_fwd_long", "mifwt_dwt1_fwd_long_levels", "mifwt_dwt1_inv_long", "mifwt_dwt1_inv_long_supported", "mifwt_dwt1_long_plan", "mifwt_dwt1_fwd_tail", "mifwt_dwt1_fwd_tail_max_n", "mifwt_dwt1_inv_tail", "mifwt_workspace_bytes", "mifwt_kernel_id", "mifwt_set_option",
+    for sym in ("mifwt_dwt_fwd", "mifwt_dwt_inv", "mifwt_dwt_fwd_adjoint", "mifwt_dwt_inv_adjoint", "mifwt_swt_fwd", "mifwt_swt_inv", "mifwt_tap_correlate", "mifwt_tap_correlate_dilated", "mifwt_dwt2_fwd_pair", "mifwt_dwt2_fwd_pair_supported", "mifwt_dwt2_inv_pair", "mifwt_dwt2_inv_pair_supported", "mifwt_dwt2_fwd_pyramid", "mifwt_dwt2_fwd_pyramid_supported", "mifwt_dwt2_fwd_pyramid_schedule", "mifwt_dwt2_fwd_pyramid_unit_plan", "mifwt_dwt3_fwd_slab_plan", "mifwt_dwt_fwd_dtaps", "mifwt_dwt_inv_dtaps", "mifwt_dwt_fwd_adjoint_dtaps", "mifwt_dwt_inv_adjoint_dtaps", "mifwt_workspace_bytes_dtaps", "mifwt_kernel_id_dtaps", "mifwt_dwt2_inv_pyramid", "mifwt_dwt2_inv_pyramid_supported", "mifwt_dwt1_fwd_long", "mifwt_dwt1_fwd_long_levels", "mifwt_dwt1_inv_long", "mifwt_dwt1_inv_long_supported", "mifwt_dwt1_long_plan", "mifwt_dwt1_fwd_tail", "mifwt_dwt1_fwd_tail_max_n", "mifwt_dwt1_inv_tail", "mifwt_workspace_bytes", "mifwt_kernel_id", "mifwt_set_option",
                 "mifwt_launch_count", "mifwt_strerror", "mifwt_abi_version", "mifwt_bwt_fwd", "mifwt_bwt_inv", "mifwt_bwt_supported", "mifwt_bwt_kernel_id",
                 "mifwt_bwt_axis_fwd", "mifwt_bwt_axis_inv", "mifwt_bwt3_fwd", "mifwt_bwt3_inv", "mifwt_bwt3_supported", "mifwt_bwt3_kernel_id",
                 "mifwt_bwt_tree_levels", "mifwt_bwt_tree_fwd", "mifwt_bwt_tree_inv"):
diff --git a/include/mifwt.h b/include/mifwt.h
--- a/include/mifwt.h
+++ b/include/mifwt.h
@@ -81,6 +81,7 @@
 int mifwt_dwt2_fwd_pyramid(int nlevels, const mifwt_level_desc* const* descs, const void* x, void* const* const* details, void* approx,
                            const double* dec_lo, const double* dec_hi, void* stream);
 int mifwt_dwt2_fwd_pyramid_schedule(int nlevels, const mifwt_level_desc* const* descs, unsigned int* wg_start, int capacity);
+int mifwt_dwt2_fwd_pyramid_unit_plan(int filt_len, int nlevels, int rows, int unit_lo, int unit_rows, int* out, int capacity);
 
 int mifwt_dwt3_fwd_slab_plan(const mifwt_level_desc* desc, int* out, int capacity);
 
diff --git a/pytorch-wavelet-toolbox_amd/_engine.py b/pytorch-wavelet-toolbox_amd/_engine.py
--- a/pytorch-wavelet-toolbox_amd/_engine.py
+++ b/pytorch-wavelet-toolbox_amd/_engine.py
@@ -155,6 +155,8 @@
                                              ctypes.c_int64, ctypes.c_int, ctypes.c_int, dbl_p, dbl_p, vp, vp, vp]
     lib.mifwt_set_option.restype = ctypes.c_int
     lib.mifwt_set_option.argtypes = [ctypes.c_int, ctypes.c_int]
+    lib.mifwt_dwt2_fwd_pyramid_unit_plan.restype = ctypes.c_int
+    lib.mifwt_dwt2_fwd_pyramid_unit_plan.argtypes = [ctypes.c_int] * 5 + [ctypes.POINTER(ctypes.c_int), ctypes.c_int]
     _lib = lib
     return lib
 
@@ -209,6 +211,21 @@
 
 def launch_count(variant: int) -> int:
     return int(load_library().mifwt_launch_count(variant))
+
+
+DEBUG_PYR_OLD_UNITS = 1 << 22
+
+PYR_UNIT_PLAN_FIELDS = ("nsteps1", "nsteps", "lean1", "lean2", "pre3", "burst3", "barriers", "D2", "D3", "npair1", "npair2", "npair3",
+                        "rA1", "rA2", "rA3", "oA1", "oA2", "oA3", "barriers_l1", "barriers_l2", "barriers_l3", "barriers_loader",
+                        "barriers_tail", "flags")
+
+
+def pyramid_unit_plan(filt_len: int, nlevels: int, rows: int, unit_lo: int, unit_rows: int) -> dict:
+    out = (ctypes.c_int * len(PYR_UNIT_PLAN_FIELDS))()
+    n = load_library().mifwt_dwt2_fwd_pyramid_unit_plan(filt_len, nlevels, rows, unit_lo, unit_rows, out, len(out))
+    if n != len(out):
+        _check(n)
+    return dict(zip(PYR_UNIT_PLAN_FIELDS, out))
 
 
 def set_option(key: int, value: int) -> None:
diff --git a/pytorch-wavelet-toolbox_amd/csrc/mifwt_api.hip b/pytorch-wavelet-toolbox_amd/csrc/mifwt_api.hip
--- a/pytorch-wavelet-toolbox_amd/csrc/mifwt_api.hip
+++ b/pytorch-wavelet-toolbox_amd/csrc/mifwt_api.hip
@@ -636,6 +636,10 @@
   if (pyramid_route(nlevels, descs) != 1) return MIFWT_ERR_UNSUPPORTED;
   return dwt2_fwd_pyr_schedule(nlevels, descs, wg_start, capacity);
 }
+int mifwt_dwt2_fwd_pyramid_unit_plan(int filt_len, int nlevels, int rows, int unit_lo, int unit_rows, int* out, int capacity) {
+  if (!out) return MIFWT_ERR_BADARG;
+  return dwt2_fwd_pyr_unit_plan(filt_len, nlevels, rows, unit_lo, unit_rows, out, capacity);
+}
 int mifwt_dwt3_fwd_slab_plan(const mifwt_level_desc* desc, int* out, int capacity) {
   if (!desc || !out) return MIFWT_ERR_BADARG;
   const int rc = validate(desc, 0);
diff --git a/pytorch-wavelet-toolbox_amd/csrc/mifwt_common.h b/pytorch-wavelet-toolbox_amd/csrc/mifwt_common.h
--- a/pytorch-wavelet-toolbox_amd/csrc/mifwt_common.h
+++ b/pytorch-wavelet-toolbox_amd/csrc/mifwt_common.h
@@ -22,7 +22,7 @@
 #define MIFWT_EXPW(a) 0
 #define MIFWT_PROFP(a) (static_cast<unsigned long long*>(nullptr))
 #endif
-constexpr int kRouteBits = 8 | 64 | 512 | 1024 | 4096 | 8192 | 524288 | 1048576 | 2097152;
+constexpr int kRouteBits = 8 | 64 | 512 | 1024 | 4096 | 8192 | 524288 | 1048576 | 2097152 | 4194304;
 inline int exp_word() { return kDiag ? g_options[MIFWT_OPT_EXP] : 0; }
 extern unsigned long long g_launch_counts[16];
 inline void count_launch(int variant) { __atomic_fetch_add(&g_launch_counts[variant], 1ull, __ATOMIC_RELAXED); }
@@ -214,6 +214,7 @@
 int dwt2_fwd_pyr(int nlev, const mifwt_level_desc* const* d, const void* x, void* const* const* details, void* approx,
                  LevelTaps dec, hipStream_t stream);
 int dwt2_fwd_pyr_schedule(int nlev, const mifwt_level_desc* const* d, uint32_t* wg_start, int capacity);
+int dwt2_fwd_pyr_unit_plan(int L, int nlev, int H0, int u_lo, int u_rows, int* out, int capacity);
 
 bool dwt2_inv_pair_supported(const mifwt_level_desc* d2, const mifwt_level_desc* d1);
 int dwt2_inv_pair(const mifwt_level_desc* d2, const mifwt_level_desc* d1, const void* approx2, const void* const* details2,
diff --git a/pytorch-wavelet-toolbox_amd/csrc/mifwt_dwt2_fwd_pyr.hip b/pytorch-wavelet-toolbox_amd/csrc/mifwt_dwt2_fwd_pyr.hip
--- a/pytorch-wavelet-toolbox_amd/csrc/mifwt_dwt2_fwd_pyr.hip
+++ b/pytorch-wavelet-toolbox_amd/csrc/mifwt_dwt2_fwd_pyr.hip
@@ -39,6 +39,7 @@
   int mode;
   int exp;
   int l2split;
+  int uflags;
   unsigned long long* prof;
   int dbg;
   DevTapArg dt;
@@ -176,31 +177,14 @@
     const int u_rows = min(a.H[NLEV] - u_lo, (int)(g_hi - g));
     g += (uint32_t)u_rows;
 
+    const PyrUnitPlan up = pyr_unit_plan(L, NLEV, a.H, u_lo, u_rows, a.uflags);
     int rA[NLEV + 1], rB[NLEV + 1], oA[NLEV + 1], oB[NLEV + 1];
-    oA[NLEV] = rA[NLEV] = u_lo;
-    oB[NLEV] = rB[NLEV] = u_lo + u_rows;
-#pragma unroll
-    for (int l = NLEV - 1; l >= 1; --l) {
-      oA[l] = 2 * oA[l + 1];
-      oB[l] = oB[l + 1] == a.H[l + 1] ? a.H[l] : min(a.H[l], 2 * oB[l + 1]);
-      rA[l] = max(0, 2 * rA[l + 1] - HL);
-      rB[l] = min(a.H[l], 2 * rB[l + 1]);
-    }
-    const bool top = u_lo == 0;
-    const int D2 = top ? pyr_lag2(L) : pyr_lag2_inner(L);
-    const int D3 = top ? pyr_lag3(L) : pyr_lag3_inner(L);
+#pragma unroll
+    for (int l = 1; l <= NLEV; ++l) rA[l] = up.rA[l], rB[l] = up.rB[l], oA[l] = up.oA[l], oB[l] = up.oB[l];
+    const int D2 = up.D2, D3 = up.D3;
     const int E0 = 2 * rA[1] - HL, e0_end = 2 * rB[1];
-    const int npair1 = rB[1] - rA[1] + HP - 1;
-    const int nsteps1 = (npair1 + 3) / 4;
-    int nsteps = nsteps1, npair2 = 0, npair3 = 0;
-    if constexpr (NLEV >= 2) {
-      npair2 = rB[2] - rA[2] + HP - 1;
-      nsteps = max(nsteps, D2 + (npair2 + 1) / 2);
-    }
-    if constexpr (NLEV >= 3) {
-      npair3 = rB[3] - rA[3] + HP - 1;
-      nsteps = max(nsteps, D3 + npair3);
-    }
+    const int nsteps1 = up.nsteps1, nsteps = up.nsteps, npair2 = up.npair2, npair3 = up.npair3;
+    const bool burst = up.burst3 > 0;
     const int nsub = 2 * nsteps, nsub1 = 2 * nsteps1;
 
     if (role == kRoleLoad) {
@@ -247,6 +231,7 @@
           __syncthreads();
           if (t + ahead < nsub1) issue(t + ahead);
         }
+        if (burst) __syncthreads();
       };
       pyr_dispatch<3>(mych - 1, [&](auto k) { run(std::integral_constant<int, decltype(k)::value + 1>{}); });
     } else if (role == kRoleL1) {
@@ -317,8 +302,9 @@
         }
       };
 
-      auto step1 = [&](auto sm_tag, int s) {
+      auto step1 = [&](auto sm_tag, auto lean_tag, int s) {
         constexpr int SM = decltype(sm_tag)::value;
+        constexpr bool LEAN = decltype(lean_tag)::value;
         pyr_static_for<2>([&](auto half_tag) {
           constexpr int half = decltype(half_tag)::value;
           pyr_barrier<PROF>(waited);
@@ -344,8 +330,8 @@
               constexpr int R = (4 * SM + j) % HP;
               f2 ha[NC1], hb[NC1];
               h_pair(w[2 * jj], w[2 * jj + 1], ha, hb);
-              acc.template feed<0, R>(tap, ha);
-              acc.template feed<1, R>(tap, hb);
+              acc.template feed<0, R, LEAN>(tap, ha);
+              acc.template feed<1, R, LEAN>(tap, hb);
               const int i = rA[1] + 4 * s + j - (HP - 1);
               const f2 (&lo)[NC1] = acc.lo[PyrAcc<L, NC1>::done(R)];
               const f2 (&hi)[NC1] = acc.hi[PyrAcc<L, NC1>::done(R)];
@@ -354,6 +340,7 @@
 #pragma unroll
                 for (int k = 0; k < NC1; ++k) *reinterpret_cast<float*>(rr + (i < rB[1] ? rw[k] : 0u)) = lo[k].x;
               }
+              if constexpr (LEAN) return;
               const bool own = i >= oA[1] && i < oB[1];
               const uint32_t v2 = own ? sv2 : kPyrOob;
               const uint32_t so = own ? (uint32_t)i * (uint32_t)a.ds_h[0] * 4u : 0u;
@@ -376,15 +363,26 @@
         });
       };
       int sm = 0;
+      const int nlean1 = up.lean1 / 4;
+      auto run1 = [&](auto t, int s) {
+        if constexpr (NLEV >= 2) {
+          if (s < nlean1) {
+            step1(t, std::true_type{}, s);
+            return;
+          }
+        }
+        step1(t, std::false_type{}, s);
+      };
 #pragma unroll 1
       for (int s = 0; s < nsteps; ++s) {
         if constexpr (HP == 3 || HP == 5) {
-          pyr_dispatch<HP>(sm, [&](auto t) { step1(t, s); });
+          pyr_dispatch<HP>(sm, [&](auto t) { run1(t, s); });
           sm = sm == HP - 1 ? 0 : sm + 1;
         } else {
-          step1(std::integral_constant<int, 0>{}, s);
-        }
-      }
+          run1(std::integral_constant<int, 0>{}, s);
+        }
+      }
+      if (burst) pyr_barrier<PROF>(waited);
     } else if (NLEV >= 2 && role == kRoleL2) {
       if constexpr (NLEV >= 2) {
         const int gmax = (cB[2] - cA[2] + 1) / 2 - 1;
@@ -450,8 +448,9 @@
         if ((MIFWT_EXPW(a) & 3) == 2) __builtin_amdgcn_s_setprio(2);
         if ((MIFWT_EXPW(a) & 3) == 3) __builtin_amdgcn_s_setprio(3);
         unsigned long long tsec[4] = {0, 0, 0, 0};
-        auto do_pair = [&](auto r_tag, auto jj_tag, int s, const uint32_t (&so_r)[4]) {
+        auto do_pair = [&](auto r_tag, auto jj_tag, auto lean_tag, int s, const uint32_t (&so_r)[4]) {
           constexpr int R = decltype(r_tag)::value, jj = decltype(jj_tag)::value;
+          constexpr bool LEAN = decltype(lean_tag)::value;
           unsigned long long t0 = 0;
           if constexpr (PROF) t0 = __builtin_readcyclecounter();
           f2 wa[NW2], wb[NW2];
@@ -465,8 +464,8 @@
           }
           f2 ha[2], hb[2];
           h_pair(wa, wb, ha, hb);
-          acc.template feed<0, R>(tap, ha);
-          acc.template feed<1, R>(tap, hb);
+          acc.template feed<0, R, LEAN>(tap, ha);
+          acc.template feed<1, R, LEAN>(tap, hb);
           if constexpr (PROF) {
             asm volatile("" ::: "memory");
             const unsigned long long t1 = __builtin_readcyclecounter();
@@ -482,6 +481,10 @@
             const bool mine = i < rB[2];
             *reinterpret_cast<float*>(rr + (mine ? rw[0] : 0u)) = lo[0].x;
             *reinterpret_cast<float*>(rr + (mine ? rw[1] : 0u)) = lo[1].x;
+          }
+          if constexpr (LEAN) {
+            if constexpr (PROF) tsec[2] += __builtin_readcyclecounter() - t0;
+            return;
           }
           const bool own = i >= oA[2] && i < oB[2];
           const uint32_t v2 = own ? sv2 : kPyrOob;
@@ -505,7 +508,7 @@
             tsec[2] += __builtin_readcyclecounter() - t0;
           }
         };
-        auto half = [&](auto r_tag, auto jj_tag, int s, const uint32_t (&so_r)[4]) {
+        auto half = [&](auto r_tag, auto jj_tag, auto lean_tag, int s, const uint32_t (&so_r)[4]) {
           constexpr int jj = decltype(jj_tag)::value;
           unsigned long long tp = 0;
           if constexpr (PROF) tp = __builtin_readcyclecounter();
@@ -517,9 +520,9 @@
             wave_lds_fence();
           }
           if constexpr (PROF) tsec[3] += __builtin_readcyclecounter() - tp;
-          do_pair(r_tag, jj_tag, s, so_r);
+          do_pair(r_tag, jj_tag, lean_tag, s, so_r);
         };
-        auto step2 = [&](auto r0_tag, int s) {
+        auto step2 = [&](auto r0_tag, auto lean_tag, int s) {
           constexpr int R0 = decltype(r0_tag)::value;
           using RA = std::integral_constant<int, R0 % HP>;
           using RB = std::integral_constant<int, (R0 + 1) % HP>;
@@ -547,12 +550,12 @@
             }
             if (NW == 12 && widx == 0 && a.twave >= 0 && lane == 0) *reinterpret_cast<u4*>(smem) = (u4){so_r[0], so_r[1], so_r[2], so_r[3]};
             early = a.l2split && qmax0 <= 4 * s - 1;
-            if (early) half(RA{}, std::integral_constant<int, 0>{}, s, so_r);
+            if (early) half(RA{}, std::integral_constant<int, 0>{}, lean_tag, s, so_r);
           }
           pyr_barrier<PROF>(waited);
           if (act) {
-            if (!early) half(RA{}, std::integral_constant<int, 0>{}, s, so_r);
-            half(RB{}, std::integral_constant<int, 1>{}, s, so_r);
+            if (!early) half(RA{}, std::integral_constant<int, 0>{}, lean_tag, s, so_r);
+            half(RB{}, std::integral_constant<int, 1>{}, lean_tag, s, so_r);
           }
         };
         {
@@ -563,13 +566,23 @@
             pyr_barrier<PROF>(waited);
           }
           constexpr int PERIOD = (HP % 2 == 0) ? (HP / 2 > 0 ? HP / 2 : 1) : HP;
+          const int lean_end2 = D2 + up.lean2 / 2;
 #pragma unroll 1
           for (; s < nsteps; s += PERIOD) {
             pyr_static_for<PERIOD>([&](auto k_tag) {
               constexpr int k = decltype(k_tag)::value;
-              if (k == 0 || s + k < nsteps) step2(std::integral_constant<int, (2 * k) % HP>{}, s + k);
+              if (k == 0 || s + k < nsteps) {
+                if constexpr (NLEV >= 3) {
+                  if (s + k < lean_end2) {
+                    step2(std::integral_constant<int, (2 * k) % HP>{}, std::true_type{}, s + k);
+                    return;
+                  }
+                }
+                step2(std::integral_constant<int, (2 * k) % HP>{}, std::false_type{}, s + k);
+              }
             });
           }
+          if (burst) pyr_barrier<PROF>(waited);
         }
         if (PROF && widx == 0 && lane == 0) {
           unsigned long long* o = MIFWT_PROFP(a) + ((size_t)blockIdx.x * kPyrWaves + 14) * 2;
@@ -626,9 +639,11 @@
             vfma_hi(hb[0], tap[L - 2 - 2 * k], wb[k]);
           }
         };
+        const int ncad3 = max(nsteps - D3, 0);
         auto step3 = [&](auto r_tag, int s) {
           constexpr int R = decltype(r_tag)::value;
-          pyr_barrier<PROF>(waited);
+          const bool cad = s - D3 < ncad3;
+          if (cad || (burst && s - D3 == ncad3)) pyr_barrier<PROF>(waited);
           if (s - D3 < npair3 && !(MIFWT_DBG(a) & 4)) {
             uint32_t so_r[2];
             const int e0 = E2 + 2 * (s - D3);
@@ -668,20 +683,20 @@
             pyr_store1(hi.y, rd, v, so + o2);
             pyr_store1(lo.x, ra, v, own ? (uint32_t)i * (uint32_t)a.as_h * 4u : 0u);
           }
-          pyr_barrier<PROF>(waited);
+          if (cad) pyr_barrier<PROF>(waited);
         };
         {
-          int s = 0;
 #pragma unroll 1
-          for (; s < D3 && s < nsteps; ++s) {
+          for (int s = 0; s < D3 && s < nsteps; ++s) {
             pyr_barrier<PROF>(waited);
             pyr_barrier<PROF>(waited);
           }
+          const int s_end = D3 + max(ncad3, npair3);
 #pragma unroll 1
-          for (; s < nsteps; s += HP) {
+          for (int s = D3; s < s_end; s += HP) {
             pyr_static_for<HP>([&](auto k_tag) {
               constexpr int k = decltype(k_tag)::value;
-              if (k == 0 || s + k < nsteps) step3(k_tag, s + k);
+              if (s + k < s_end) step3(k_tag, s + k);
             });
           }
         }
@@ -810,21 +825,36 @@
           }
         }
       };
+      const int ro2 = NLEV >= 3 ? HP - 1 - rA[I3] : 0, E2 = NLEV >= 3 ? 2 * rA[NLEV] - HL : 0;
+      const int nt_steps = nsteps + ((MIFWT_DBG(a) & 4) ? (burst ? 1 : 0) : up.burst3);
 #pragma unroll 1
-      for (int s = 0; s < nsteps; ++s) {
-        const bool act1 = s < nsteps1;
-        const bool act2 = NLEV >= 2 && s >= D2 && 2 * (s - D2) < npair2 && !(MIFWT_DBG(a) & 4);
+      for (int t = 0; t < nt_steps; ++t) {
+        const bool cad = t < nsteps;
+        const int s = cad ? t : D3 + up.pre3 + (t - nsteps);
+        const bool act1 = cad && s < nsteps1;
+        const bool act2 = cad && NLEV >= 2 && s >= D2 && 2 * (s - D2) < npair2 && !(MIFWT_DBG(a) & 4);
         const bool act3 = NLEV >= 3 && s >= D3 && s - D3 < npair3 && !(MIFWT_DBG(a) & 4);
-        pyr_barrier<PROF>(waited);
+        if (cad || t == nsteps) pyr_barrier<PROF>(waited);
         uint32_t rb1 = (uint32_t)(stage - smem) + (uint32_t)bi * (uint32_t)(kPyrSub * a.pitch0);
-        if (act1) bi = bi + 1 == a.nbuf ? 0 : bi + 1;
-        run_half(s, 0, act1, false, false, rb1, (u4){0u, 0u, 0u, 0u}, (u2){0u, 0u});
-        pyr_barrier<PROF>(waited);
+        if (cad) {
+          if (act1) bi = bi + 1 == a.nbuf ? 0 : bi + 1;
+          run_half(s, 0, act1, false, false, rb1, (u4){0u, 0u, 0u, 0u}, (u2){0u, 0u});
+          pyr_barrier<PROF>(waited);
+        }
         const u4 v2 = *reinterpret_cast<const u4*>(smem);
-        const u2 v3 = *reinterpret_cast<const u2*>(smem + 16);
+        u2 v3 = *reinterpret_cast<const u2*>(smem + 16);
+        if constexpr (NLEV >= 3) {
+          if (!cad) {
+            const int e0 = E2 + 2 * (s - D3);
+            const bool dead0 = zero_mode && (unsigned)e0 >= (unsigned)a.H[I3], dead1 = zero_mode && (unsigned)(e0 + 1) >= (unsigned)a.H[I3];
+            v3.x = (uint32_t)((dead0 ? kPyrRing : ((fold(e0, a.H[I3]) + ro2) & (kPyrRing - 1))) * a.pitch2);
+            v3.y = (uint32_t)((dead1 ? kPyrRing : ((fold(e0 + 1, a.H[I3]) + ro2) & (kPyrRing - 1))) * a.pitch2);
+          }
+        }
         rb1 = (uint32_t)(stage - smem) + (uint32_t)bi * (uint32_t)(kPyrSub * a.pitch0);
         if (act1) bi = bi + 1 == a.nbuf ? 0 : bi + 1;
         run_half(s, 1, act1, act2, act3, rb1, v2, v3);
+        if (!cad) wave_lds_fence();
       }
       }
     }
@@ -1185,6 +1215,28 @@
   if (capacity < p.nwg + 1) return MIFWT_ERR_BADARG;
   std::copy(p.wg_start, p.wg_start + p.nwg + 1, wg_start);
   return p.nwg;
+}
+
+static int pyr_unit_flags() {
+  int f = (g_options[MIFWT_OPT_DEBUG] & 4194304) ? (kPyrPlanNoLean | kPyrPlanNoBurst) : 0;
+  if (kDiag) f |= (exp_word() >> 20) & 7;
+  return f;
+}
+
+int dwt2_fwd_pyr_unit_plan(int L, int nlev, int H0, int u_lo, int u_rows, int* out, int capacity) {
+  if (L < 2 || L > 10 || (L & 1) || nlev < 1 || nlev > 3 || (L == 10 && nlev != 1) || H0 < 1) return MIFWT_ERR_BADARG;
+  if (capacity < 24) return MIFWT_ERR_BADARG;
+  int H[4] = {H0, 0, 0, 0};
+  for (int l = 1; l <= nlev; ++l) H[l] = (H[l - 1] + L - 1) / 2;
+  if (u_lo < 0 || u_rows < 1 || u_lo + u_rows > H[nlev]) return MIFWT_ERR_BADARG;
+  const int flags = pyr_unit_flags();
+  const PyrUnitPlan p = pyr_unit_plan(L, nlev, H, u_lo, u_rows, flags);
+  const int v[24] = {p.nsteps1, p.nsteps, p.lean1, p.lean2, p.pre3, p.burst3, p.barriers, p.D2, p.D3, p.npair1, p.npair2, p.npair3,
+                     p.rA[1], p.rA[2], p.rA[3], p.oA[1], p.oA[2], p.oA[3],
+                     pyr_role_barriers(p, L, nlev, kRoleL1), pyr_role_barriers(p, L, nlev, kRoleL2), pyr_role_barriers(p, L, nlev, kRoleL3),
+                     pyr_role_barriers(p, L, nlev, kRoleLoad), pyr_role_barriers(p, L, nlev, kRoleTail), flags};
+  std::copy(v, v + 24, out);
+  return 24;
 }
 
 template <int L, int NLEV>
@@ -1237,6 +1289,7 @@
   if ((MIFWT_DBG(a) & 262144) && a.nl3 > 1) --a.nl3;
   a.prof = g_pyr_prof;
   a.l2split = (g_options[MIFWT_OPT_DEBUG] & 8192) ? 0 : 1;
+  a.uflags = pyr_unit_flags();
   a.exp = exp_word();
   a.hn_div = make_fastdiv((uint32_t)a.H[NLEV]);
   std::copy(p.wg_start, p.wg_start + p.nwg + 1, a.wg_start);
diff --git a/pytorch-wavelet-toolbox_amd/csrc/mifwt_pyr.h b/pytorch-wavelet-toolbox_amd/csrc/mifwt_pyr.h
--- a/pytorch-wavelet-toolbox_amd/csrc/mifwt_pyr.h
+++ b/pytorch-wavelet-toolbox_amd/csrc/mifwt_pyr.h
@@ -16,6 +16,98 @@
 constexpr int pyr_lag2(int L) { const int b = pyr_cdiv(L - 2 + L / 2 - 2, 4); return b > pyr_lag2_inner(L) ? b : pyr_lag2_inner(L); }
 constexpr int pyr_lag3_inner(int L) { return pyr_lag2_inner(L) + 1 + pyr_cdiv(L / 2 - 1, 2); }
 constexpr int pyr_lag3(int L) { const int a = L / 2 - 1, b = L - 2 + L / 2 - 2; return pyr_lag2(L) + 1 + pyr_cdiv(a > b ? a : b, 2); }
+
+struct PyrUnitPlan {
+  int rA[4], rB[4], oA[4], oB[4];
+  int D2, D3;
+  int npair1, npair2, npair3;
+  int nsteps1, nsteps;
+  int lean1, lean2;
+  int pre3, burst3;
+  int barriers;
+};
+constexpr int kPyrPlanNoLean = 1, kPyrPlanNoBurst = 2, kPyrPlanNoLean2 = 4;
+__host__ __device__ __forceinline__ PyrUnitPlan pyr_unit_plan(int L, int nlev, const int* H, int u_lo, int u_rows, int flags) {
+  const int HL = L - 2, HP = L / 2;
+  PyrUnitPlan p{};
+  p.oA[nlev] = p.rA[nlev] = u_lo;
+  p.oB[nlev] = p.rB[nlev] = u_lo + u_rows;
+#pragma unroll
+  for (int l = nlev - 1; l >= 1; --l) {
+    p.oA[l] = 2 * p.oA[l + 1];
+    p.oB[l] = p.oB[l + 1] == H[l + 1] ? H[l] : (H[l] < 2 * p.oB[l + 1] ? H[l] : 2 * p.oB[l + 1]);
+    p.rA[l] = 2 * p.rA[l + 1] - HL > 0 ? 2 * p.rA[l + 1] - HL : 0;
+    p.rB[l] = H[l] < 2 * p.rB[l + 1] ? H[l] : 2 * p.rB[l + 1];
+  }
+  const bool top = u_lo == 0;
+  p.D2 = top ? pyr_lag2(L) : pyr_lag2_inner(L);
+  p.D3 = top ? pyr_lag3(L) : pyr_lag3_inner(L);
+  p.npair1 = p.rB[1] - p.rA[1] + HP - 1;
+  p.nsteps1 = (p.npair1 + 3) / 4;
+  p.nsteps = p.nsteps1;
+  if (nlev >= 2) {
+    p.npair2 = p.rB[2] - p.rA[2] + HP - 1;
+    const int e2 = p.D2 + (p.npair2 + 1) / 2;
+    p.nsteps = p.nsteps > e2 ? p.nsteps : e2;
+  }
+  if (nlev >= 3) {
+    p.npair3 = p.rB[3] - p.rA[3] + HP - 1;
+    if (flags & kPyrPlanNoBurst) {
+      const int e3 = p.D3 + p.npair3;
+      p.nsteps = p.nsteps > e3 ? p.nsteps : e3;
+    }
+    const int in = p.nsteps - p.D3;
+    p.pre3 = in < 0 ? 0 : (in < p.npair3 ? in : p.npair3);
+    p.burst3 = p.npair3 - p.pre3;
+  }
+  if (!(flags & kPyrPlanNoLean)) {
+    p.lean1 = (p.oA[1] - p.rA[1]) & ~3;
+    if (nlev >= 2 && !(flags & kPyrPlanNoLean2)) p.lean2 = (p.oA[2] - p.rA[2]) & ~1;
+  }
+  p.barriers = 2 * p.nsteps + (p.burst3 > 0 ? 1 : 0) + 1;
+  return p;
+}
+
+inline int pyr_role_barriers(const PyrUnitPlan& p, int L, int nlev, int role) {
+  const int HP = L / 2;
+  const bool burst = p.burst3 > 0;
+  int n = 0;
+  if (role == kRoleLoad) {
+    for (int t = 0; t < 2 * p.nsteps; ++t) ++n;
+    if (burst) ++n;
+  } else if (role == kRoleL1) {
+    for (int s = 0; s < p.nsteps; ++s) n += 2;
+    if (burst) ++n;
+  } else if (role == kRoleTail) {
+    for (int t = 0; t < p.nsteps + p.burst3; ++t) {
+      const bool cad = t < p.nsteps;
+      if (cad || t == p.nsteps) ++n;
+      if (cad) ++n;
+    }
+  } else if (role == kRoleL2) {
+    if (nlev < 2) return -1;
+    int s = 0;
+    for (; s < p.D2 && s < p.nsteps; ++s) n += 2;
+    const int period = (HP % 2 == 0) ? (HP / 2 > 0 ? HP / 2 : 1) : HP;
+    for (; s < p.nsteps; s += period)
+      for (int k = 0; k < period; ++k)
+        if (k == 0 || s + k < p.nsteps) n += 2;
+    if (burst) ++n;
+  } else if (role == kRoleL3) {
+    if (nlev < 3) return -1;
+    for (int s = 0; s < p.D3 && s < p.nsteps; ++s) n += 2;
+    const int ncad3 = p.nsteps - p.D3 > 0 ? p.nsteps - p.D3 : 0;
+    const int s_end = p.D3 + (ncad3 > p.npair3 ? ncad3 : p.npair3);
+    for (int s = p.D3; s < s_end; s += HP)
+      for (int k = 0; k < HP; ++k)
+        if (s + k < s_end) {
+          const bool cad = s + k - p.D3 < ncad3;
+          if (cad || (burst && s + k - p.D3 == ncad3)) ++n;
+          if (cad) ++n;
+        }
+  }
+  return n + 1;
+}
 
 #ifndef MIFWT_ST_AUX
 #define MIFWT_ST_AUX 0
@@ -129,7 +221,7 @@
 #pragma unroll
       for (int c = 0; c < NC; ++c) lo[q][c] = hi[q][c] = V{};
   }
-  template <int PH, int R>
+  template <int PH, int R, bool LEAN = false>
   __device__ __forceinline__ void feed(const V (&tap)[L], const V (&hv)[NC]) {
 #pragma unroll
     for (int q = 0; q < HP; ++q) {
@@ -139,10 +231,10 @@
       for (int c = 0; c < NC; ++c) {
         if (q == 0 && PH == 0) {
           lo[sl][c] = vmul_lo(tap[m], hv[c]);
-          hi[sl][c] = vmul_hi(tap[m], hv[c]);
+          if constexpr (!LEAN) hi[sl][c] = vmul_hi(tap[m], hv[c]);
         } else {
           vfma_lo(lo[sl][c], tap[m], hv[c]);
-          vfma_hi(hi[sl][c], tap[m], hv[c]);
+          if constexpr (!LEAN) vfma_hi(hi[sl][c], tap[m], hv[c]);
         }
       }
     }
```

After: 703,800 Msamples/s (median of 2 runs). About the same (+0.3%).
